# kai422/DAS3R

Hardware: AMD Instinct MI355X
Metric: render fwd+bwd Msplats/s at 1080p (higher is better)
Workload: dtype f32; 1 GPU; 1M random splats, 1920x1080, SH degree 3, forward+backward (BASELINE.json configs[3], constant P); splats_per_gpu=1000000, splats_per_gpu_final=1000000, init_steps=30, sh_degree=3, num_rendered=2614506, api=GaussianRasterizer.forward + autograd backward (drop-in surface), parallelism=1 independent scenes, one per GPU

## Files before the change

### das3r_amd/_lib.py

```python
import ctypes as C
import os

_HERE = os.path.dirname(os.path.abspath(__file__))
LIB_PATH = os.path.join(_HERE, "libdas3r_hip.so")
ABI_VERSION = 16
NO_BACKWARD_IN_FLAG = 8
ANTIALIAS_FLAG = 16
AUX_MAX_CHANNELS = 8

ALLOC_FN = C.CFUNCTYPE(C.c_void_p, C.c_void_p, C.c_size_t)


class RasterArgs(C.Structure):
    _fields_ = [("P", C.c_int32), ("sh_degree", C.c_int32), ("M", C.c_int32), ("image_width", C.c_int32),
                ("image_height", C.c_int32), ("tanfovx", C.c_float), ("tanfovy", C.c_float), ("scale_modifier", C.c_float),
                ("bg", C.c_void_p), ("viewmatrix", C.c_void_p), ("projmatrix", C.c_void_p), ("campos", C.c_void_p),
                ("prefiltered", C.c_int32), ("debug", C.c_int32), ("capacity_hint", C.c_int64)]


class PreTransform(C.Structure):
    _fields_ = [("xyz", C.c_void_p), ("rot", C.c_void_p), ("scaling", C.c_void_p), ("opacity_raw", C.c_void_p), ("conf_flat", C.c_void_p),
                ("mask_index", C.c_void_p), ("R", C.c_void_p), ("t", C.c_void_p), ("Lq", C.c_void_p)]


class RasterIn(C.Structure):
    _fields_ = [("means3D", C.c_void_p), ("opacities", C.c_void_p), ("shs", C.c_void_p), ("colors_precomp", C.c_void_p),
                ("scales", C.c_void_p), ("rotations", C.c_void_p), ("cov3D_precomp", C.c_void_p), ("pre", C.POINTER(PreTransform))]


class RasterOut(C.Structure):
    _fields_ = [("out_color", C.c_void_p), ("radii", C.c_void_p), ("out_invdepth", C.c_void_p)]


class RasterSaved(C.Structure):
    _fields_ = [("geom", C.c_void_p), ("binning", C.c_void_p), ("img", C.c_void_p), ("num_rendered", C.c_int64), ("capacity", C.c_int64),
                ("check_word", C.c_void_p), ("check_tag", C.c_uint32), ("flags", C.c_uint32)]


class AdamSlot(C.Structure):
    _fields_ = [("param", C.c_void_p), ("exp_avg", C.c_void_p), ("exp_avg_sq", C.c_void_p), ("step_size", C.c_float), ("bc2_sqrt", C.c_float)]


class Chain(C.Structure):
    _fields_ = [("g_conf_flat", C.c_void_p), ("g_small", C.c_void_p), ("slots", C.POINTER(AdamSlot)), ("beta1", C.c_float), ("beta2", C.c_float),
                ("eps", C.c_float)]


class RasterGrads(C.Structure):
    _fields_ = [("dL_dmeans2D", C.c_void_p), ("dL_dopacities", C.c_void_p), ("dL_dmeans3D", C.c_void_p),
                ("dL_dshs", C.c_void_p), ("dL_dcolors_precomp", C.c_void_p), ("dL_dscales", C.c_void_p),
                ("dL_drotations", C.c_void_p), ("dL_dcov3D", C.c_void_p), ("scratch", C.c_void_p), ("chain", C.POINTER(Chain))]


class PruneTensor(C.Structure):
    _fields_ = [("src", C.c_void_p), ("dst", C.c_void_p), ("row_bytes", C.c_int64)]


class PathPolicyState(C.Structure):
    _fields_ = [("P", C.c_int32), ("W", C.c_int32), ("H", C.c_int32), ("last_I", C.c_int64), ("peak_I", C.c_int64), ("radix_left", C.c_int32),
                ("backoff", C.c_int32), ("gen", C.c_uint32), ("seg_extra", C.c_int32), ("last_seg", C.c_int32), ("fine", C.c_int32),
                ("forwards", C.c_uint32), ("clean", C.c_uint32), ("longest", C.c_uint32), ("resume_valid", C.c_int32), ("resume_fine", C.c_int32),
                ("resume_forwards", C.c_uint32)]


class PathPolicyInputs(C.Structure):
    _fields_ = [("P", C.c_int32), ("W", C.c_int32), ("H", C.c_int32), ("ntiles", C.c_int32), ("tbits", C.c_int32), ("tile_passes", C.c_int32),
                ("too_long", C.c_uint32), ("want_bits", C.c_uint32), ("forced", C.c_int32), ("onesweep", C.c_int32), ("capacity_hint", C.c_int64),
                ("capacity_exact", C.c_int32)]


class PathPolicyPlan(C.Structure):
    _fields_ = [("local", C.c_int32), ("seg", C.c_int32), ("seg_bits", C.c_int32), ("seg_passes", C.c_int32), ("speculate", C.c_int32),
                ("decide_fine", C.c_int32), ("gen", C.c_uint32), ("cap", C.c_int64)]


class Switches(C.Structure):
    _fields_ = [(n, C.c_int32) for n in
                ("sort_ipl", "sort_classic", "rect_upstream", "verbose", "binning", "capacity_exact", "fused_emit_off", "no_sh_stage", "render_fwd",
                 "render_bwd", "render_bwd_mb", "render_bwd_atomic", "render_bwd_pix", "render_bwd_occ", "render_bwd_strips", "tile_chunk",
                 "scan_items", "deterministic", "tile_lpt_off", "bwd_reduce_set", "bwd_reduce_shfl", "ablate_set", "ablate", "tickets",
                 "bwd_pad_lds", "fwd_pad_lds", "bwd_buckets", "fwd_no_prefetch", "split_colour", "tile_strip")]


class BwdChoice(C.Structure):
    _fields_ = [(n, C.c_int32) for n in ("kernel", "mb", "slices", "pix", "occ", "strips", "atomic_flush")]


class FwdChoice(C.Structure):
    _fields_ = [(n, C.c_int32) for n in ("kernel", "quad_lanes", "row_private", "tile_lpt")]


class PreprocessBackwardInputs(C.Structure):
    _fields_ = [(n, C.c_int32) for n in ("has_sh", "has_cov", "M", "sh_degree", "shs_aligned16", "dL_dshs_aligned16", "no_sh_stage", "jac_saved",
                                         "chained", "quad_rows", "depth", "aa")]


class PreprocessForm(C.Structure):
    _fields_ = [(n, C.c_int32) for n in ("has_sh", "has_cov", "stage_in", "stage_out", "deg0", "chain", "depth", "jac", "aa", "base_index",
                                         "sh_rows_staged")]


PRUNE_GROUP_ROWS = 1024


def prune_count_words(P):
    return 1 + (int(P) + PRUNE_GROUP_ROWS - 1) // PRUNE_GROUP_ROWS


class RasterLayout(C.Structure):
    _fields_ = [(n, C.c_size_t) for n in
                ("geom_bytes", "binning_bytes", "img_bytes", "depth_key", "xy", "conic_opacity", "rgbd", "splat_stride", "clamped",
                 "tiles_touched", "sorted_idx", "offsets", "point_list", "final_T", "n_contrib", "ranges")]


EXPORTS = ("das3r_raster_forward", "das3r_raster_backward", "das3r_raster_backward_depth", "das3r_raster_backward_depth_scratch_bytes", "das3r_raster_check", "das3r_raster_backward_scratch_bytes", "das3r_mark_visible", "das3r_knn3_workspace_bytes",
           "das3r_knn3_mean_dist2", "das3r_raster_get_layout", "das3r_abi_version", "das3r_last_error", "das3r_reload_switches", "das3r_get_stats",
           "das3r_raster_forget_shapes", "das3r_raster_learning",
           "das3r_profile_enable", "das3r_profile_report", "das3r_pretransform_forward", "das3r_pretransform_backward", "das3r_pose_matrices", "das3r_pose_chain",
           "das3r_adam_step", "das3r_adam_step_gated", "das3r_photometric_blocks", "das3r_photometric_forward", "das3r_photometric_backward",
           "das3r_has_experiments", "das3r_pair_counters", "das3r_debug_poison_lds", "das3r_debug_inject_fault", "das3r_debug_mutate",
           "das3r_pose_matrices_qt", "das3r_pose_chain_qt", "das3r_photometric_finish", "das3r_pretransform_backward_adam", "das3r_pretransform_pose_sums",
           "das3r_raster_count_live_pairs", "das3r_photometric_backward_finish", "das3r_pose_chain_qt_rearm", "das3r_ssim_map_forward", "das3r_ssim_map_backward",
           "das3r_split_colour_rule", "das3r_split_colour_switch", "das3r_depth_l1_blocks", "das3r_depth_l1", "das3r_prune_select", "das3r_prune_compact",
           "das3r_photometric_forward_exposure", "das3r_photometric_backward_finish_exposure", "das3r_exposure_grad_finish",
           "das3r_raster_aux_forward", "das3r_raster_aux_scratch_bytes", "das3r_raster_aux_adjoint",
           "das3r_raster_aux_backward_scratch_bytes", "das3r_raster_aux_backward",
           "das3r_raster_distortion_forward", "das3r_raster_distortion_backward_scratch_bytes", "das3r_raster_distortion_backward",
           "das3r_thin_workspace_bytes", "das3r_thin_voxels", "das3r_raster_focal_workspace_bytes", "das3r_raster_backward_focal",
           "das3r_debug_path_policy_fresh", "das3r_debug_path_policy_plan", "das3r_debug_path_policy_count", "das3r_debug_path_policy_skew",
           "das3r_debug_path_policy_hint", "das3r_debug_path_policy_forget", "das3r_debug_path_policy_resume", "das3r_debug_seg_dbits",
           "das3r_debug_parse_switches", "das3r_debug_choose_backward", "das3r_debug_choose_forward", "das3r_debug_has_invdepth_form",
           "das3r_debug_kernel_name", "das3r_debug_choose_preprocess_backward", "das3r_debug_preprocess_backward_name")

_lib = None


def load():
    global _lib
    if _lib is not None:
        return _lib
    if not os.path.exists(LIB_PATH):
        raise RuntimeError(
            f"das3r_amd: HIP library not found at {LIB_PATH}. Build it with `python -c 'import __graft_entry__ as g; "
            f"g.build()'` or `make -C das3r_amd/csrc`. There is no CPU fallback.")
    L = C.CDLL(LIB_PATH)
    for name in EXPORTS:
        if not hasattr(L, name):
            raise RuntimeError(f"das3r_amd: {LIB_PATH} does not export {name}; rebuild it")
    L.das3r_abi_version.restype = C.c_int
    if L.das3r_abi_version() != ABI_VERSION:
        raise RuntimeError("das3r_amd: ABI version mismatch between the Python host layer and libdas3r_hip.so; rebuild")
    L.das3r_last_error.restype = C.c_char_p
    L.das3r_raster_forward.restype = C.c_int64
    L.das3r_raster_forward.argtypes = [C.POINTER(RasterArgs), C.POINTER(RasterIn), C.POINTER(RasterOut), ALLOC_FN, ALLOC_FN,
                                       ALLOC_FN, C.c_void_p, C.POINTER(RasterSaved), C.c_void_p]
    L.das3r_raster_backward.restype = C.c_int
    L.das3r_raster_backward.argtypes = [C.POINTER(RasterArgs), C.POINTER(RasterIn), C.POINTER(RasterSaved), C.c_void_p,
                                        C.POINTER(RasterGrads), C.c_void_p]
    L.das3r_raster_backward_scratch_bytes.restype = C.c_size_t
    L.das3r_raster_backward_depth.restype = C.c_int
    L.das3r_raster_backward_depth.argtypes = [C.POINTER(RasterArgs), C.POINTER(RasterIn), C.POINTER(RasterSaved), C.c_void_p, C.c_void_p,
                                              C.POINTER(RasterGrads), C.c_void_p]
    L.das3r_raster_backward_depth_scratch_bytes.restype = C.c_size_t
    L.das3r_raster_backward_depth_scratch_bytes.argtypes = [C.c_int64]
    L.das3r_raster_backward_scratch_bytes.argtypes = [C.c_int64]
    L.das3r_raster_check.restype = C.c_int
    L.das3r_raster_check.argtypes = [C.POINTER(RasterSaved), C.c_void_p]
    L.das3r_raster_count_live_pairs.restype = C.c_int
    L.das3r_raster_count_live_pairs.argtypes = [C.POINTER(RasterArgs), C.POINTER(RasterSaved), C.POINTER(C.c_uint64), C.c_void_p]
    L.das3r_mark_visible.restype = C.c_int
    L.das3r_mark_visible.argtypes = [C.c_int32, C.c_void_p, C.c_void_p, C.c_void_p, C.c_void_p, C.c_void_p]
    L.das3r_knn3_workspace_bytes.restype = C.c_size_t
    L.das3r_knn3_workspace_bytes.argtypes = [C.c_int32]
    L.das3r_knn3_mean_dist2.restype = C.c_int
    L.das3r_knn3_mean_dist2.argtypes = [C.c_int32, C.c_void_p, C.c_void_p, C.c_void_p, C.c_void_p]
    L.das3r_pose_matrices.restype = C.c_int
    L.das3r_pose_matrices.argtypes = [C.c_void_p, C.c_void_p, C.c_void_p]
    L.das3r_pose_chain.restype = C.c_int
    L.das3r_pose_chain.argtypes = [C.c_void_p, C.c_void_p, C.c_void_p, C.c_void_p]
    L.das3r_pretransform_forward.restype = C.c_int
    L.das3r_pretransform_forward.argtypes = [C.c_int32] + [C.c_void_p] * 13 + [C.c_void_p]
    L.das3r_pretransform_backward.restype = C.c_int
    L.das3r_pretransform_backward.argtypes = [C.c_int32] + [C.c_void_p] * 18 + [C.c_void_p]
    L.das3r_pretransform_backward_adam.restype = C.c_int
    L.das3r_pretransform_backward_adam.argtypes = [C.c_int32] + [C.c_void_p] * 10 + [C.POINTER(AdamSlot), C.c_float, C.c_float, C.c_float, C.c_void_p]
    L.das3r_pretransform_pose_sums.restype = C.c_int
    L.das3r_pretransform_pose_sums.argtypes = [C.c_int32] + [C.c_void_p] * 7 + [C.c_void_p]
    L.das3r_photometric_blocks.restype = C.c_int64
    L.das3r_photometric_blocks.argtypes = [C.c_int32, C.c_int32]
    L.das3r_photometric_forward.restype = C.c_int
    L.das3r_photometric_forward.argtypes = [C.c_int32, C.c_int32, C.c_void_p, C.c_void_p, C.c_void_p, C.c_float, C.c_void_p, C.c_void_p, C.c_void_p]
    L.das3r_photometric_backward.restype = C.c_int
    L.das3r_photometric_backward.argtypes = [C.c_int32, C.c_int32, C.c_void_p, C.c_void_p, C.c_void_p, C.c_float, C.c_void_p, C.c_void_p,
                                             C.c_void_p, C.c_void_p, C.c_void_p]
    L.das3r_pose_matrices_qt.restype = C.c_int
    L.das3r_pose_matrices_qt.argtypes = [C.c_void_p, C.c_void_p, C.c_void_p, C.c_void_p]
    L.das3r_pose_chain_qt.restype = C.c_int
    L.das3r_pose_chain_qt.argtypes = [C.c_void_p, C.c_void_p, C.c_void_p, C.c_void_p, C.c_void_p]
    L.das3r_pose_chain_qt_rearm.restype = C.c_int
    L.das3r_pose_chain_qt_rearm.argtypes = [C.c_void_p, C.c_void_p, C.c_void_p, C.c_void_p, C.c_void_p, C.c_void_p, C.c_void_p]
    L.das3r_ssim_map_forward.restype = C.c_int
    L.das3r_ssim_map_forward.argtypes = [C.c_int32, C.c_int32, C.c_void_p, C.c_void_p, C.c_void_p, C.c_void_p, C.c_void_p, C.c_void_p]
    L.das3r_ssim_map_backward.restype = C.c_int
    L.das3r_ssim_map_backward.argtypes = [C.c_int32, C.c_int32, C.c_void_p, C.c_void_p, C.c_void_p, C.c_void_p, C.c_void_p, C.c_void_p, C.c_void_p]
    L.das3r_photometric_backward_finish.restype = C.c_int
    L.das3r_photometric_backward_finish.argtypes = [C.c_int32, C.c_int32, C.c_void_p, C.c_void_p, C.c_void_p, C.c_float, C.c_void_p, C.c_void_p,
                                                    C.c_void_p, C.c_void_p, C.c_void_p, C.c_void_p, C.c_void_p]
    L.das3r_photometric_forward_exposure.restype = C.c_int
    L.das3r_photometric_forward_exposure.argtypes = [C.c_int32, C.c_int32, C.c_void_p, C.c_void_p, C.c_void_p, C.c_float, C.c_void_p, C.c_void_p,
                                                     C.c_void_p, C.c_void_p]
    L.das3r_photometric_backward_finish_exposure.restype = C.c_int
    L.das3r_photometric_backward_finish_exposure.argtypes = [C.c_int32, C.c_int32, C.c_void_p, C.c_void_p, C.c_void_p, C.c_float] + [C.c_void_p] * 9
    L.das3r_exposure_grad_finish.restype = C.c_int
    L.das3r_exposure_grad_finish.argtypes = [C.c_int32, C.c_int32, C.c_void_p, C.c_void_p, C.c_void_p, C.c_void_p]
    L.das3r_depth_l1_blocks.restype = C.c_int64
    L.das3r_depth_l1_blocks.argtypes = [C.c_int32, C.c_int32]
    L.das3r_depth_l1.restype = C.c_int
    L.das3r_depth_l1.argtypes = [C.c_int32, C.c_int32, C.c_void_p, C.c_void_p, C.c_void_p, C.c_void_p, C.c_float, C.c_void_p, C.c_void_p, C.c_void_p,
                                 C.c_void_p, C.c_void_p]
    L.das3r_prune_select.restype = C.c_int
    L.das3r_prune_select.argtypes = [C.c_int32, C.c_void_p, C.c_void_p, C.c_void_p, C.c_float, C.c_void_p, C.c_float, C.c_void_p, C.c_void_p, C.c_void_p,
                                     C.c_void_p]
    L.das3r_prune_compact.restype = C.c_int
    L.das3r_prune_compact.argtypes = [C.c_int32, C.c_int32, C.c_void_p, C.c_int32, C.POINTER(PruneTensor), C.c_void_p]
    L.das3r_thin_workspace_bytes.restype = C.c_size_t
    L.das3r_thin_workspace_bytes.argtypes = [C.c_int32]
    L.das3r_thin_voxels.restype = C.c_int
    L.das3r_thin_voxels.argtypes = [C.c_int32, C.c_void_p, C.c_void_p, C.c_float, C.c_void_p, C.c_void_p, C.c_void_p, C.c_void_p, C.c_void_p]
    L.das3r_raster_focal_workspace_bytes.restype = C.c_size_t
    L.das3r_raster_focal_workspace_bytes.argtypes = [C.c_int32]
    L.das3r_raster_backward_focal.restype = C.c_int
    L.das3r_raster_backward_focal.argtypes = [C.POINTER(RasterArgs), C.POINTER(RasterIn), C.POINTER(RasterSaved), C.c_void_p, C.c_void_p,
                                              C.POINTER(RasterGrads), C.c_void_p, C.c_void_p, C.c_void_p, C.c_void_p]
    L.das3r_raster_aux_forward.restype = C.c_int
    L.das3r_raster_aux_forward.argtypes = [C.POINTER(RasterArgs), C.POINTER(RasterSaved), C.c_int32, C.c_void_p, C.c_void_p, C.c_void_p]
    L.das3r_raster_aux_scratch_bytes.restype = C.c_size_t
    L.das3r_raster_aux_scratch_bytes.argtypes = [C.c_int64, C.c_int32]
    L.das3r_raster_aux_adjoint.restype = C.c_int
    L.das3r_raster_aux_adjoint.argtypes = [C.POINTER(RasterArgs), C.POINTER(RasterSaved), C.c_int32, C.c_void_p, C.c_void_p, C.c_int32, C.c_void_p,
                                           C.c_void_p]
    L.das3r_raster_aux_backward_scratch_bytes.restype = C.c_size_t
    L.das3r_raster_aux_backward_scratch_bytes.argtypes = [C.c_int64, C.c_int32]
    L.das3r_raster_aux_backward.restype = C.c_int
    L.das3r_raster_aux_backward.argtypes = [C.POINTER(RasterArgs), C.POINTER(RasterIn), C.POINTER(RasterSaved), C.c_int32, C.c_void_p, C.c_void_p,
                                            C.c_void_p, C.c_void_p, C.POINTER(RasterGrads), C.c_void_p]
    L.das3r_raster_distortion_forward.restype = C.c_int
    L.das3r_raster_distortion_forward.argtypes = [C.POINTER(RasterArgs), C.POINTER(RasterSaved), C.c_void_p, C.c_void_p, C.c_void_p]
    L.das3r_raster_distortion_backward_scratch_bytes.restype = C.c_size_t
    L.das3r_raster_distortion_backward_scratch_bytes.argtypes = [C.c_int64, C.c_int32]
    L.das3r_raster_distortion_backward.restype = C.c_int
    L.das3r_raster_distortion_backward.argtypes = [C.POINTER(RasterArgs), C.POINTER(RasterIn), C.POINTER(RasterSaved), C.c_void_p, C.c_void_p,
                                                   C.POINTER(RasterGrads), C.c_void_p]
    L.das3r_photometric_finish.restype = C.c_int
    L.das3r_photometric_finish.argtypes = [C.c_int32, C.c_int32, C.c_void_p, C.c_float, C.c_void_p, C.c_void_p]
    L.das3r_adam_step_gated.restype = C.c_int
    L.das3r_adam_step_gated.argtypes = [C.c_int32, C.c_void_p, C.c_float, C.c_float, C.c_float, C.c_void_p, C.c_float, C.c_void_p, C.c_void_p]
    L.das3r_adam_step.restype = C.c_int
    L.das3r_adam_step.argtypes = [C.c_int32, C.c_void_p, C.c_float, C.c_float, C.c_float, C.c_void_p]
    ps = C.POINTER(PathPolicyState)
    L.das3r_debug_path_policy_fresh.restype = None
    L.das3r_debug_path_policy_fresh.argtypes = [ps, C.c_uint32]
    L.das3r_debug_path_policy_plan.restype = None
    L.das3r_debug_path_policy_plan.argtypes = [ps, C.POINTER(PathPolicyInputs), C.POINTER(PathPolicyPlan)]
    L.das3r_debug_path_policy_count.restype = C.c_int
    L.das3r_debug_path_policy_count.argtypes = [ps, C.POINTER(PathPolicyInputs), C.POINTER(PathPolicyPlan), C.c_int64]
    L.das3r_debug_path_policy_skew.restype = C.c_int
    L.das3r_debug_path_policy_skew.argtypes = [ps, C.c_uint32, C.c_uint32, C.c_int64, C.c_int32]
    L.das3r_debug_path_policy_hint.restype = C.c_uint32
    L.das3r_debug_path_policy_hint.argtypes = [ps]
    L.das3r_debug_path_policy_forget.restype = None
    L.das3r_debug_path_policy_forget.argtypes = [ps]
    L.das3r_debug_path_policy_resume.restype = None
    L.das3r_debug_path_policy_resume.argtypes = [ps, C.c_uint32, C.c_uint32]
    L.das3r_debug_seg_dbits.restype = C.c_int
    L.das3r_debug_seg_dbits.argtypes = [C.c_int32, C.c_int32]
    sw = C.POINTER(Switches)
    L.das3r_debug_parse_switches.restype = None
    L.das3r_debug_parse_switches.argtypes = [C.POINTER(C.c_char_p), C.POINTER(C.c_char_p), C.c_int32, C.c_int32, sw]
    L.das3r_debug_choose_backward.restype = None
    L.das3r_debug_choose_backward.argtypes = [sw, C.c_int64, C.c_int32, C.c_uint32, C.POINTER(BwdChoice)]
    L.das3r_debug_choose_forward.restype = None
    L.das3r_debug_choose_forward.argtypes = [sw, C.c_int32, C.c_int64, C.c_int32, C.c_int32, C.POINTER(FwdChoice)]
    L.das3r_debug_has_invdepth_form.restype = C.c_int
    L.das3r_debug_has_invdepth_form.argtypes = [C.c_int32, C.c_int32]
    L.das3r_debug_kernel_name.restype = C.c_char_p
    L.das3r_debug_kernel_name.argtypes = [C.c_int32, C.c_int32]
    L.das3r_debug_choose_preprocess_backward.restype = C.c_int
    L.das3r_debug_choose_preprocess_backward.argtypes = [C.POINTER(PreprocessBackwardInputs), C.POINTER(PreprocessForm)]
    L.das3r_debug_preprocess_backward_name.restype = C.c_char_p
    L.das3r_debug_preprocess_backward_name.argtypes = [C.POINTER(PreprocessForm)]
    L.das3r_raster_get_layout.restype = C.c_int
    L.das3r_raster_get_layout.argtypes = [C.c_int32, C.c_int64, C.c_int32, C.c_int32, C.POINTER(RasterLayout)]
    _lib = L
    return L


def reload_switches():
    L = load()
    L.das3r_reload_switches.restype = None
    L.das3r_reload_switches.argtypes = []
    L.das3r_reload_switches()


def split_colour_rule(has_sh, sh_degree, P, binning_path, forced=None, no_backward=False):
    L = load()
    L.das3r_split_colour_rule.restype = C.c_int
    L.das3r_split_colour_rule.argtypes = [C.c_int32] * 6
    L.das3r_split_colour_switch.restype = C.c_int
    L.das3r_split_colour_switch.argtypes = []
    if forced is None:
        forced = L.das3r_split_colour_switch()
    return bool(L.das3r_split_colour_rule(int(bool(has_sh)), int(sh_degree), int(P), int(binning_path), int(bool(no_backward)), int(forced)))


def split_colour_switch():
    L = load()
    L.das3r_split_colour_switch.restype = C.c_int
    L.das3r_split_colour_switch.argtypes = []
    return int(L.das3r_split_colour_switch())


def has_experiments():
    L = load()
    L.das3r_has_experiments.restype = C.c_int
    L.das3r_has_experiments.argtypes = []
    return bool(L.das3r_has_experiments())


def inject_fault(bits):
    L = load()
    L.das3r_debug_inject_fault.restype = None
    L.das3r_debug_inject_fault.argtypes = [C.c_uint32]
    L.das3r_debug_inject_fault(int(bits))


def forget_shapes():
    L = load()
    L.das3r_raster_forget_shapes.restype = C.c_int
    L.das3r_raster_forget_shapes.argtypes = []
    check(L.das3r_raster_forget_shapes(), "das3r_raster_forget_shapes")


def learning(state=None):
    L = load()
    L.das3r_raster_learning.restype = C.c_int
    L.das3r_raster_learning.argtypes = [C.c_int32, C.POINTER(C.c_uint32)]
    buf = (C.c_uint32 * 2)(*(state if state is not None else (0, 0)))
    check(L.das3r_raster_learning(0 if state is None else 1, buf), "das3r_raster_learning")
    return int(buf[0]), int(buf[1])


def mutate(what):
    L = load()
    L.das3r_debug_mutate.restype = None
    L.das3r_debug_mutate.argtypes = [C.c_uint32]
    L.das3r_debug_mutate(int(what))


def poison_lds(pattern=0x7FC00000):
    import torch
    L = load()
    L.das3r_debug_poison_lds.restype = C.c_int
    L.das3r_debug_poison_lds.argtypes = [C.c_uint32, C.c_void_p]
    check(L.das3r_debug_poison_lds(int(pattern), C.c_void_p(torch.cuda.current_stream().cuda_stream)), "das3r_debug_poison_lds")


def pair_counters(enable):
    L = load()
    L.das3r_pair_counters.restype = C.c_int
    L.das3r_pair_counters.argtypes = [C.c_int, C.POINTER(C.c_uint64)]
    if enable:
        check(L.das3r_pair_counters(1, None), "das3r_pair_counters")
        return None
    out = (C.c_uint64 * 4)()
    check(L.das3r_pair_counters(0, out), "das3r_pair_counters")
    return dict(fwd_pairs=int(out[0]), bwd_pairs=int(out[1]), fwd_wave_iterations=int(out[2]), bwd_wave_iterations=int(out[3]))
# ... 57 lines not shown
```

### das3r_amd/csrc/api.hip

```cpp
#include <stdarg.h>
#include <string.h>

#include <vector>

#include "host_state.h"
#include "preprocess_choice.h"
#include <algorithm>

namespace das3r {

static thread_local char g_err[512] = "";

void set_error(const char *fmt, ...) {
    va_list ap;
    va_start(ap, fmt);
    vsnprintf(g_err, sizeof(g_err), fmt, ap);
    va_end(ap);
}

struct ProfRec {
    const char *name;
    hipEvent_t start, stop;
};
static bool g_prof_on = false;
static std::vector<ProfRec> g_prof;
bool profile_enabled() { return g_prof_on; }
static std::vector<hipEvent_t> g_event_pool;
static hipEvent_t pooled_event() {
    if (!g_event_pool.empty()) { hipEvent_t e = g_event_pool.back(); g_event_pool.pop_back(); return e; }
    hipEvent_t e = nullptr;
    return hipEventCreate(&e) == hipSuccess ? e : nullptr;
}
void profile_begin(const char *name, hipStream_t s) {
    ProfRec r;
    r.name = name;
    r.start = pooled_event();
    r.stop = pooled_event();
    if (!r.start || !r.stop) return;
    (void)hipEventRecord(r.start, s);
    g_prof.push_back(r);
}
void profile_end(hipStream_t s) {
    if (!g_prof.empty()) (void)hipEventRecord(g_prof.back().stop, s);
}

static Switches g_sw;
static bool g_sw_loaded = false;
static int g_inject_fault = 0;
static int g_mutate = 0;
static void load_switches() {
#ifdef DAS3R_EXPERIMENTS
    const bool experiments = true;
#else
    const bool experiments = false;
#endif
    Switches w = parse_switches(getenv, experiments);
    w.inject_fault = g_inject_fault;
    w.mutate = g_mutate;
    g_sw = w;
    __atomic_store_n(&g_sw_loaded, true, __ATOMIC_RELEASE);
}
const Switches &switches() {
    if (!__atomic_load_n(&g_sw_loaded, __ATOMIC_ACQUIRE)) load_switches();
    return g_sw;
}

static int g_threads_on_device[MAX_DEVICES] = {};
struct ThreadRegistrar {
    bool on[MAX_DEVICES] = {};
    void add(int dev) {
        if (!on[dev]) { on[dev] = true; __atomic_fetch_add(&g_threads_on_device[dev], 1, __ATOMIC_RELAXED); }
    }
    ~ThreadRegistrar() {
        for (int d = 0; d < MAX_DEVICES; d++)
            if (on[d]) __atomic_fetch_sub(&g_threads_on_device[d], 1, __ATOMIC_RELAXED);
    }
};
static thread_local ThreadRegistrar g_registrar;
void register_rendering_thread(int dev) { g_registrar.add(dev); }
bool grid_is_resident(int nblocks) {
    const int forced = switches().tickets;
    int dev = 0;
    if (hipGetDevice(&dev) != hipSuccess || dev < 0 || dev >= MAX_DEVICES) return false;
    const bool shared = __atomic_load_n(&g_threads_on_device[dev], __ATOMIC_RELAXED) > 1;
    if (forced >= 0) {
        static bool warned = false;
        if (shared && forced > 0 && !__atomic_exchange_n(&warned, true, __ATOMIC_RELAXED))
            fprintf(stderr, "[das3r] DAS3R_TICKETS is set to a bound while several host threads render on device %d: ticket-free chained "
                            "kernels are only safe when a grid has the device to itself\n", dev);
        return nblocks <= forced;
    }
    if (shared) return false;
    static thread_local int cached_dev = -1, cached_limit = 0;
    if (dev != cached_dev) {
        int cus = 0;
        if (hipDeviceGetAttribute(&cus, hipDeviceAttributeMultiprocessorCount, dev) != hipSuccess) return false;
        cached_dev = dev;
        cached_limit = cus * 2;
    }
    return nblocks <= cached_limit;
}

int sort_ipl_override() { return switches().sort_ipl; }
#ifdef DAS3R_EXPERIMENTS
bool use_onesweep() { return !switches().sort_classic; }
#else
bool use_onesweep() { return true; }
#endif
bool use_tight_rect() { return !switches().rect_upstream; }

void compute_layout(int P, int64_t I, int W, int H, Layout *L, bool shjac) {
    memset(L, 0, sizeof(*L));
    const size_t Pn = P > 0 ? (size_t)P : 1, In = I > 0 ? (size_t)I : 1;
    L->capacity = I;
    L->tiles_x = (W + TILE_X - 1) / TILE_X;
    L->tiles_y = (H + TILE_Y - 1) / TILE_Y;
    L->ntiles = L->tiles_x * L->tiles_y;
    L->tbits = tile_bits(L->ntiles);
    L->tile_passes = (L->tbits + 7) / 8;
    L->dbits = 0;
    L->kbits = L->tbits;
    L->kshift = 0;
    L->part_passes = L->tile_passes;
    L->chunksP = sort_num_chunks(P);
    L->chunksI = sort_num_chunks(I);
    size_t o = 0;
    auto take = [&](size_t b) { size_t r = o; o += align_up(b); return r; };
    L->g_keyA = take(4 * Pn);
    L->g_keyB = take(4 * Pn);
    L->g_valA = take(4 * Pn);
    L->g_valB = take(4 * Pn);
    L->pub.sorted_idx = L->g_valA;
    L->pub.depth_key = L->g_keyA;
    L->pub.xy = take(16 * SPLAT_REC * Pn);
    L->pub.conic_opacity = L->pub.xy + 16;
    L->pub.rgbd = L->pub.xy + 32;
    L->pub.splat_stride = 16 * SPLAT_REC;
    L->pub.clamped = take(Pn);
    L->pub.tiles_touched = take(4 * Pn);
    L->pub.offsets = take(4 * Pn);
    L->g_hist = take(4 * (size_t)RADIX_SIZE * (size_t)(L->chunksP > 0 ? L->chunksP : 1));
    L->g_totals = take(4 * RADIX_SIZE);
    L->g_blocksums = take(4 * (size_t)div_up((int64_t)Pn, 4096));
    L->g_count = take(256);
    L->g_off_by_gid = take(4 * Pn);
    L->g_rect = take(4 * Pn);
    L->g_dhist = take(4 * 256);
    L->g_ghist = take(4 * 4 * RADIX_SIZE);
    L->g_ticket = take(256);
    L->g_status = take(onesweep_status_bytes((int64_t)Pn, 4));
    L->g_scan_status = take(scan_status_bytes((int)Pn));
    L->g_ctrl_bytes = o - L->g_ghist;
    if (shjac) L->g_shjac = take(4 * 9 * Pn);
    L->pub.geom_bytes = o;
    o = 0;
    L->b_keyA = take(4 * In);
    L->b_keyB = take(4 * In);
    L->b_valA = take(4 * In);
    L->b_valB = take(4 * In);
    L->b_hist = take(4 * (size_t)RADIX_SIZE * (size_t)(L->chunksI > 0 ? L->chunksI : 1));
    L->b_totals = take(4 * RADIX_SIZE);
    L->b_gid_of = take(4 * In);
    L->b_slot = take(4 * In);
    L->b_e2 = take(4 * In);
    L->b_ghist = take(4 * 4 * RADIX_SIZE);
    L->b_ticket = take(256);
    L->b_status = take(onesweep_status_bytes((int64_t)In, L->tile_passes + 1));
    L->b_ctrl_bytes = o - L->b_ghist;
    L->b_ckpt = take(((size_t)In / BUCKET + (size_t)(L->ntiles > 0 ? L->ntiles : 1) + 2) * 256 * 16);
    L->pub.binning_bytes = o;
    const size_t npix_d = (size_t)W * (size_t)H;
    L->d_ckpt = take(((size_t)In / BUCKET + (size_t)(L->ntiles > 0 ? L->ntiles : 1) + 2) * 256 * 16);
    L->d_recs = take(16 * SPLAT_REC * Pn);
    L->d_dpix = take(4 * 3 * (npix_d > 0 ? npix_d : 1));
    L->d_bg = take(16);
    L->d_dz = take(4 * Pn);
    L->d_bytes = o;
    L->pub.point_list = (L->tile_passes & 1) ? L->b_valB : L->b_valA;
    o = 0;
    const size_t npix = (size_t)W * (size_t)H;
    L->pub.final_T = take(4 * (npix > 0 ? npix : 1));
    L->pub.n_contrib = take(4 * (npix > 0 ? npix : 1));
    L->pub.ranges = take(8 * (size_t)(L->ntiles > 0 ? L->ntiles : 1));
    L->i_order = take(4 * (size_t)(L->ntiles > 0 ? L->ntiles : 1));
    L->pub.img_bytes = o;
}

}

using namespace das3r;

extern "C" int das3r_abi_version(void) { return DAS3R_ABI_VERSION; }
extern "C" void das3r_reload_switches(void) { load_switches(); }
extern "C" void das3r_debug_inject_fault(uint32_t bits) {
    g_inject_fault = (int)bits;
    load_switches();
}
extern "C" void das3r_debug_mutate(uint32_t what) {
    g_mutate = (int)what;
    load_switches();
}
extern "C" const char *das3r_last_error(void) { return g_err; }
extern "C" int das3r_split_colour_switch(void) { return switches().split_colour; }
extern "C" int das3r_split_colour_rule(int32_t has_sh, int32_t sh_degree, int32_t P, int32_t binning_path, int32_t no_backward, int32_t forced) {
    return split_colour_rule(has_sh != 0, sh_degree, P, binning_path, no_backward != 0, forced) ? 1 : 0;
}

namespace {
struct PolicyOnState {
    Verdict v;
    Resume r;
    das3r_path_policy_state *s;
    explicit PolicyOnState(das3r_path_policy_state *state) : s(state) { policy_state_from(*s, &v, &r); }
    ~PolicyOnState() { policy_state_to(v, r, s); }
    PolicyInputs inputs(const das3r_path_policy_inputs *in) {
        return PolicyInputs{in->P, in->W, in->H, in->ntiles, in->tbits, in->tile_passes, in->too_long, in->want_bits, in->forced, in->onesweep != 0,
                            in->capacity_hint, in->capacity_exact != 0, &r};
    }
};
ForwardPlan plan_of(const das3r_path_policy_plan *p) {
    return ForwardPlan{p->local != 0, p->seg != 0, p->seg == 2, p->seg_bits, p->seg_passes, p->speculate != 0, p->cap, p->decide_fine != 0, p->gen};
}
}
extern "C" void das3r_debug_path_policy_fresh(das3r_path_policy_state *state, uint32_t gen) { policy_state_to(Verdict::fresh(gen), Resume(), state); }
extern "C" void das3r_debug_path_policy_plan(das3r_path_policy_state *state, const das3r_path_policy_inputs *in, das3r_path_policy_plan *out) {
    PolicyOnState on(state);
    const ForwardPlan p = plan_forward(on.v, on.inputs(in));
    *out = das3r_path_policy_plan{p.local, p.bucket_local ? 2 : (p.seg ? 1 : 0), p.seg_bits, p.seg_passes, p.speculate, p.decide_fine, p.gen, p.cap};
}
extern "C" int das3r_debug_path_policy_count(das3r_path_policy_state *state, const das3r_path_policy_inputs *in, const das3r_path_policy_plan *plan, int64_t I) {
    PolicyOnState on(state);
    return learn_count(on.v, I, on.inputs(in), plan_of(plan)) ? 1 : 0;
}
extern "C" int das3r_debug_path_policy_skew(das3r_path_policy_state *state, uint32_t longest, uint32_t crowd16, int64_t cap, int32_t ntiles) {
    PolicyOnState on(state);
    return learn_skew(on.v, longest, crowd16, cap, ntiles) ? 1 : 0;
}
extern "C" uint32_t das3r_debug_path_policy_hint(const das3r_path_policy_state *state) {
    Verdict v;
    Resume r;
    policy_state_from(*state, &v, &r);
    return backward_hint(v, (uint32_t)BUCKET);
}
extern "C" void das3r_debug_path_policy_forget(das3r_path_policy_state *state) {
    PolicyOnState on(state);
    forget(on.v);
}
extern "C" void das3r_debug_path_policy_resume(das3r_path_policy_state *state, uint32_t fine, uint32_t forwards) {
    PolicyOnState on(state);
    resume(on.v, on.r, fine != 0u, forwards);
}
extern "C" int das3r_debug_seg_dbits(int32_t tbits, int32_t passes) { return seg_dbits((int)tbits, (int)passes); }

extern "C" void das3r_debug_parse_switches(const char *const *names, const char *const *values, int32_t n, int32_t experiments, das3r_switches *out) {
    auto lookup = [&](const char *name) -> const char * {
        for (int32_t i = 0; i < n; i++)
            if (strcmp(names[i], name) == 0) return values[i];
        return nullptr;
    };
    switches_to(parse_switches(lookup, experiments != 0), out);
}
extern "C" void das3r_debug_choose_backward(const das3r_switches *sw, int64_t num_rendered, int32_t ntiles, uint32_t fwd_flags, das3r_bwd_choice *out) {
    const BwdChoice c = choose_backward(switches_from(*sw), num_rendered, ntiles, fwd_flags);
    *out = das3r_bwd_choice{c.kernel, c.mb, c.slices, c.pix, c.occ, c.strips, c.atomic_flush};
}
extern "C" void das3r_debug_choose_forward(const das3r_switches *sw, int32_t ntiles, int64_t capacity, int32_t local_lists, int32_t prefer_regions,
                                           das3r_fwd_choice *out) {
    const Switches w = switches_from(*sw);
    const bool local = local_lists != 0, regions = prefer_regions != 0;
    *out = das3r_fwd_choice{choose_forward(w, ntiles, capacity, local, regions), quad_lanes(w, ntiles, capacity, local), row_private(w, capacity, ntiles),
                            tile_lpt_wanted(w, ntiles, capacity, local, regions)};
}
extern "C" int das3r_debug_has_invdepth_form(int32_t backward, int32_t kernel) {
    return (backward ? bwd_has_invdepth_form((BwdKernel)kernel) : fwd_has_invdepth_form((FwdKernel)kernel)) ? 1 : 0;
}
extern "C" const char *das3r_debug_kernel_name(int32_t backward, int32_t kernel) {
    return backward ? bwd_kernel_name((BwdKernel)kernel) : fwd_kernel_name((FwdKernel)kernel);
}

static PreprocessForm form_from(const das3r_preprocess_form *f) {
    return PreprocessForm{f->has_sh != 0, f->has_cov != 0, f->stage_in != 0, f->stage_out != 0, f->deg0 != 0, f->chain != 0, f->depth != 0, f->jac != 0, f->aa != 0};
}
extern "C" int das3r_debug_choose_preprocess_backward(const das3r_preprocess_backward_inputs *in, das3r_preprocess_form *out) {
    const PreprocessBackwardInputs ci = {in->has_sh != 0, in->has_cov != 0, in->M, in->sh_degree, in->shs_aligned16 != 0, in->dL_dshs_aligned16 != 0,
                                         in->no_sh_stage != 0, in->jac_saved != 0, in->chained != 0, in->quad_rows != 0, in->depth != 0, in->aa != 0};
    const PreprocessForm f = choose_preprocess_backward(ci);
    *out = das3r_preprocess_form{f.has_sh, f.has_cov, f.stage_in, f.stage_out, f.deg0, f.chain, f.depth, f.jac, f.aa, preprocess_backward_base_index(f),
                                 sh_rows_staged(ci.has_sh, ci.M, ci.sh_degree, ci.shs_aligned16, ci.no_sh_stage)};
    return chain_refusal(ci);
}
extern "C" const char *das3r_debug_preprocess_backward_name(const das3r_preprocess_form *form) { return preprocess_backward_name(form_from(form)); }

extern "C" int das3r_raster_get_layout(int32_t P, int64_t num_rendered, int32_t W, int32_t H, das3r_raster_layout *out) {
    if (!out || P < 0 || num_rendered < 0 || W <= 0 || H <= 0) { set_error("das3r_raster_get_layout: invalid argument"); return DAS3R_ERR_INVALID_ARG; }
    Layout L;
    compute_layout(P, num_rendered, W, H, &L);
    *out = L.pub;
    return DAS3R_OK;
}

extern "C" int das3r_raster_forget_shapes(void) {
    PerDevice *T = nullptr;
    int r = per_device(&T);
    if (r) return r;
    forget(T->verdict);
    return DAS3R_OK;
}

extern "C" int das3r_raster_learning(int32_t set, uint32_t state[2]) {
    if (!state) { set_error("das3r_raster_learning: invalid argument"); return DAS3R_ERR_INVALID_ARG; }
    PerDevice *T = nullptr;
    int r = per_device(&T);
    if (r) return r;
    if (!set) {
        state[0] = prefers_regions(T->verdict) ? 1u : 0u;
        state[1] = forwards_seen(T->verdict);
        return DAS3R_OK;
    }
    resume(T->verdict, T->resume, state[0] != 0u, state[1]);
    return DAS3R_OK;
}

static Layout saved_layout(const das3r_raster_args *a, const das3r_raster_saved *saved, bool shjac = false) {
    Layout L;
    compute_layout(a->P, saved->capacity > 0 ? saved->capacity : saved->num_rendered, a->image_width, a->image_height, &L, shjac);
    return L;
}

static bool shjac_saved(const das3r_raster_args *a, const das3r_raster_in *in, const das3r_raster_saved *saved) {
    return (saved->flags & SHJAC_SAVED_FLAG) != 0 && in->shs != nullptr && a->sh_degree >= 2;
}

static int backward_validate(const char *who, const das3r_raster_in *in, const das3r_raster_saved *saved, const float *dL_dpix, bool depth_pass,
                             const float *dL_dinvdepth, const das3r_raster_grads *g) {
    const bool chained = g && g->chain;
    if (!saved || !saved->geom || !saved->img || !dL_dpix || (depth_pass && !dL_dinvdepth) || !g || !g->dL_dmeans2D ||
        (!chained && (!g->dL_dopacities || !g->dL_dmeans3D)) || (saved->num_rendered > 0 && !g->scratch)) {
        set_error("%s: null saved state / %sgradient buffer", who, depth_pass ? "upstream gradient / " : "");
        return DAS3R_ERR_INVALID_ARG;
    }
    if (depth_pass && !(saved->flags & DEPTH_SAVED_FLAG)) {
        set_error("%s: the saved state is not that of a forward with out_invdepth (das3r_raster_saved.flags bit 1 is clear)", who);
        return DAS3R_ERR_INVALID_ARG;
    }
    const bool has_sh = in->shs != nullptr, has_cov = in->cov3D_precomp != nullptr;
    if ((has_sh && !g->dL_dshs) || (!has_sh && !g->dL_dcolors_precomp) || (has_cov && !g->dL_dcov3D) ||
        (!has_cov && !chained && (!g->dL_dscales || !g->dL_drotations))) {
        set_error("%s: gradient buffer missing for a provided input", who);
        return DAS3R_ERR_INVALID_ARG;
    }
    return DAS3R_OK;
}

struct FocalOut {
    float *sums, *per_splat, *workspace;
};

static int refuse_bwd_without_invdepth(const char *who) {
    const BwdKernel k = switches().render_bwd;
    if (bwd_has_invdepth_form(k)) return DAS3R_OK;
    set_error("%s: DAS3R_RENDER_BWD=%s has no inverse-depth form", who, bwd_kernel_name(k));
    return DAS3R_ERR_INVALID_ARG;
}

static int backward_body(const char *who, const das3r_raster_args *a, const das3r_raster_in *in, const das3r_raster_saved *saved, const float *dL_dpix,
                         bool depth_pass, const float *dL_dinvdepth, const das3r_raster_grads *g, const FocalOut *focal, das3r_stream_t stream) {
    hipStream_t s = (hipStream_t)stream;
    int rc = validate(a, in);
    if (rc) return rc;
    const int P = a->P;
    if (P == 0) {
        if (focal) HIP_TRY(hipMemsetAsync(focal->sums, 0, 2 * sizeof(float), s));
        return DAS3R_OK;
    }
    if ((rc = backward_validate(who, in, saved, dL_dpix, depth_pass, dL_dinvdepth, g))) return rc;
    if (depth_pass && (rc = refuse_bwd_without_invdepth(who))) return rc;
    if ((rc = das3r_raster_check(saved, stream))) return rc;
    const Layout L = saved_layout(a, saved, shjac_saved(a, in, saved));
    float *partial = g->scratch;
    const float *dz = nullptr;
    bool quad_rows = false;
    if (saved->num_rendered > 0) {
        if (!saved->binning) { set_error("%s: binning buffer missing", who); return DAS3R_ERR_INVALID_ARG; }
        if ((rc = launch_render_backward(a, dL_dpix, saved->geom, saved->binning, saved->img, L, partial, s, &quad_rows, saved->num_rendered, saved->flags))) return rc;
        if (depth_pass) {
            const size_t c = L.capacity > 0 ? (size_t)L.capacity : 1;
            float *partial_depth = (float *)((char *)g->scratch + align_up(c * 9 * sizeof(float) + 16));
            if ((rc = launch_depth_pass_inputs(P, a->image_width * a->image_height, saved->geom, L, saved->binning, dL_dinvdepth, s, a->debug != 0))) return rc;
            Layout Ld = L;
            Ld.pub.xy = L.d_recs;
            Ld.pub.conic_opacity = L.d_recs + 16;
            Ld.pub.rgbd = L.d_recs + 32;
            Ld.b_ckpt = L.d_ckpt;
            das3r_raster_args ad = *a;
            ad.bg = (const float *)(saved->binning + L.d_bg);
            bool quad_rows_d = false;
            if ((rc = launch_render_backward(&ad, (const float *)(saved->binning + L.d_dpix), saved->binning, saved->binning, saved->img, Ld, partial_depth, s,
                                             &quad_rows_d, saved->num_rendered, saved->flags))) return rc;
            float *dzw = (float *)(saved->binning + L.d_dz);
            if ((rc = launch_depth_fold(P, saved->geom, L, partial, partial_depth, dzw, s, a->debug != 0))) return rc;
            dz = dzw;
        }
    }
    const bool aa = (saved->flags & ANTIALIAS_FLAG) != 0;
    if (focal && (rc = launch_focal_grad(a, in, saved->geom, L, partial, quad_rows, aa, focal->sums, focal->per_splat, focal->workspace, s))) return rc;
    return launch_preprocess_backward(a, in, saved->geom, saved->binning, L, g, partial, s, quad_rows, dz, aa);
}

extern "C" int das3r_raster_backward(const das3r_raster_args *a, const das3r_raster_in *in, const das3r_raster_saved *saved,
                                     const float *dL_dpix, const das3r_raster_grads *g, das3r_stream_t stream) {
    return backward_body("das3r_raster_backward", a, in, saved, dL_dpix, false, nullptr, g, nullptr, stream);
}

extern "C" int das3r_raster_backward_depth(const das3r_raster_args *a, const das3r_raster_in *in, const das3r_raster_saved *saved,
                                           const float *dL_dpix, const float *dL_dinvdepth, const das3r_raster_grads *g, das3r_stream_t stream) {
    return backward_body("das3r_raster_backward_depth", a, in, saved, dL_dpix, true, dL_dinvdepth, g, nullptr, stream);
}

extern "C" size_t das3r_raster_focal_workspace_bytes(int32_t P) { return focal_workspace_bytes(P); }
extern "C" int das3r_raster_backward_focal(const das3r_raster_args *a, const das3r_raster_in *in, const das3r_raster_saved *saved, const float *dL_dpix,
                                           const float *dL_dinvdepth, const das3r_raster_grads *g, float *sums, float *per_splat, float *workspace,
                                           das3r_stream_t stream) {
    if (!sums || !workspace) {
        set_error("das3r_raster_backward_focal: null sums / workspace");
        return DAS3R_ERR_INVALID_ARG;
    }
    const bool depth_pass = dL_dinvdepth != nullptr;
    if (depth_pass) {
        const int rc = refuse_bwd_without_invdepth("das3r_raster_backward_focal");
        if (rc) return rc;
    }
    const FocalOut focal = {sums, per_splat, workspace};
    return backward_body("das3r_raster_backward_focal", a, in, saved, dL_dpix, depth_pass, dL_dinvdepth, g, &focal, stream);
}

extern "C" size_t das3r_raster_backward_depth_scratch_bytes(int64_t capacity) {
    const size_t c = capacity > 0 ? (size_t)capacity : 1;
    return align_up(c * 9 * sizeof(float) + 16) + c * 9 * sizeof(float) + 16;
}

extern "C" size_t das3r_raster_backward_scratch_bytes(int64_t capacity) {
    const size_t c = capacity > 0 ? (size_t)capacity : 1;
#ifdef DAS3R_EXPERIMENTS
    if (switches().render_bwd == BWD_STREAM) return std::max(c * 9 * sizeof(float) + 16, stream_scratch_bytes(capacity));
#endif
    return c * 9 * sizeof(float) + 16;
}

static int aux_validate(const char *who, const das3r_raster_args *a, const das3r_raster_saved *saved, int32_t C, const void *p0, const void *p1) {
    if (!a || !saved) { set_error("%s: null args / saved state", who); return DAS3R_ERR_INVALID_ARG; }
    if (C < 1 || C > DAS3R_AUX_MAX_CHANNELS) { set_error("%s: C = %d channels (1 .. %d per call)", who, C, DAS3R_AUX_MAX_CHANNELS); return DAS3R_ERR_INVALID_ARG; }
    if (a->P < 0 || a->image_width <= 0 || a->image_height <= 0) { set_error("%s: bad extents P=%d W=%d H=%d", who, a->P, a->image_width, a->image_height); return DAS3R_ERR_INVALID_ARG; }
    if (!p1 || (a->P > 0 && !p0)) { set_error("%s: null feature / image / gradient pointer", who); return DAS3R_ERR_INVALID_ARG; }
    if (a->P > 0 && saved->num_rendered > 0 && (!saved->geom || !saved->binning || !saved->img)) { set_error("%s: saved buffers missing", who); return DAS3R_ERR_INVALID_ARG; }
    return DAS3R_OK;
}

extern "C" int das3r_raster_aux_forward(const das3r_raster_args *a, const das3r_raster_saved *saved, int32_t C, const float *features, float *out,
                                        das3r_stream_t stream) {
    hipStream_t s = (hipStream_t)stream;
    int rc = aux_validate("das3r_raster_aux_forward", a, saved, C, features, out);
    if (rc) return rc;
    const int P = a->P, W = a->image_width, H = a->image_height;
    if (P == 0 || saved->num_rendered <= 0) {
        HIP_TRY(hipMemsetAsync(out, 0, sizeof(float) * (size_t)C * (size_t)W * (size_t)H, s));
        return DAS3R_OK;
    }
    if ((rc = das3r_raster_check(saved, stream))) return rc;
    const Layout L = saved_layout(a, saved);
    return launch_render_aux_forward(P, W, H, C, features, out, saved->geom, saved->binning, saved->img, L, saved->num_rendered, a->debug != 0, s);
}

extern "C" size_t das3r_raster_aux_scratch_bytes(int64_t capacity, int32_t C) {
    const size_t c = capacity > 0 ? (size_t)capacity : 1, ch = C > 0 ? (size_t)C : 1;
    return c * ch * sizeof(float) + 16;
}

extern "C" int das3r_raster_aux_adjoint(const das3r_raster_args *a, const das3r_raster_saved *saved, int32_t C, const float *dL_dout, float *dL_dfeat,
                                        int32_t accumulate, float *scratch, das3r_stream_t stream) {
    hipStream_t s = (hipStream_t)stream;
    int rc = aux_validate("das3r_raster_aux_adjoint", a, saved, C, dL_dfeat, dL_dout);
    if (rc) return rc;
    const int P = a->P, W = a->image_width, H = a->image_height;
    if (P == 0) return DAS3R_OK;
    if (saved->num_rendered <= 0) {
        if (!accumulate) HIP_TRY(hipMemsetAsync(dL_dfeat, 0, sizeof(float) * (size_t)P * (size_t)C, s));
        return DAS3R_OK;
    }
    if (!scratch) { set_error("das3r_raster_aux_adjoint: null scratch (das3r_raster_aux_scratch_bytes)"); return DAS3R_ERR_INVALID_ARG; }
    if ((rc = das3r_raster_check(saved, stream))) return rc;
    const Layout L = saved_layout(a, saved);
    return launch_render_aux_adjoint(P, W, H, C, dL_dout, dL_dfeat, accumulate != 0, scratch, saved->geom, saved->binning, saved->img, L, saved->num_rendered, a->debug != 0, s);
}

extern "C" size_t das3r_raster_aux_backward_scratch_bytes(int64_t capacity, int32_t C) {
    const size_t c = capacity > 0 ? (size_t)capacity : 1, ch = C > 0 ? (size_t)C : 0;
    return align_up(c * 9 * sizeof(float) + 16) + c * ch * sizeof(float) + 16;
}

extern "C" int das3r_raster_aux_backward(const das3r_raster_args *a, const das3r_raster_in *in, const das3r_raster_saved *saved, int32_t C,
                                         const float *features, const float *dL_dout, const float *dL_dalpha, float *dL_dfeatures,
                                         const das3r_raster_grads *g, das3r_stream_t stream) {
    static const char who[] = "das3r_raster_aux_backward";
    hipStream_t s = (hipStream_t)stream;
    if (!a || !in || !saved || !g) { set_error("%s: null args / inputs / saved state / grads", who); return DAS3R_ERR_INVALID_ARG; }
    if (C < 0 || C > DAS3R_AUX_MAX_CHANNELS) { set_error("%s: C = %d channels (0 .. %d per call)", who, C, DAS3R_AUX_MAX_CHANNELS); return DAS3R_ERR_INVALID_ARG; }
    if (C == 0 && !dL_dalpha) { set_error("%s: C = 0 channels and null dL_dalpha: no loss term", who); return DAS3R_ERR_INVALID_ARG; }
    if (C == 0 && dL_dfeatures) { set_error("%s: dL_dfeatures with C = 0 channels", who); return DAS3R_ERR_INVALID_ARG; }
    if (C > 0 && (!dL_dout || (a->P > 0 && !features))) { set_error("%s: null features / dL_dout with C = %d channels", who, C); return DAS3R_ERR_INVALID_ARG; }
    if (g->chain) { set_error("%s: grads->chain is not supported here (the chained backward belongs to the colour loss)", who); return DAS3R_ERR_INVALID_ARG; }
    if (!g->scratch) { set_error("%s: null scratch (das3r_raster_aux_backward_scratch_bytes)", who); return DAS3R_ERR_INVALID_ARG; }
    int rc = validate(a, in);
    if (rc) return rc;
    const int P = a->P, W = a->image_width, H = a->image_height;
    if (P == 0) return DAS3R_OK;
    if ((rc = backward_validate(who, in, saved,  reinterpret_cast<const float *>(g->scratch), false, nullptr, g))) return rc;
    if (saved->num_rendered > 0 && !saved->binning) { set_error("%s: binning buffer missing", who); return DAS3R_ERR_INVALID_ARG; }
    if ((rc = das3r_raster_check(saved, stream))) return rc;
    const Layout L = saved_layout(a, saved, shjac_saved(a, in, saved));
    float *partial = g->scratch;
    if (saved->num_rendered > 0) {
        const size_t c = L.capacity > 0 ? (size_t)L.capacity : 1;
        float *partial_f = dL_dfeatures ? (float *)((char *)g->scratch + align_up(c * 9 * sizeof(float) + 16)) : nullptr;
        if ((rc = launch_render_aux_backward(P, W, H, C, features, dL_dout, dL_dalpha, partial, partial_f, saved->geom, saved->binning, saved->img, L,
                                             a->debug != 0, s))) return rc;
        if (dL_dfeatures && (rc = launch_aux_gather(P, C, partial_f, dL_dfeatures, saved->geom, L, a->debug != 0, s))) return rc;
    } else if (dL_dfeatures) {
        HIP_TRY(hipMemsetAsync(dL_dfeatures, 0, sizeof(float) * (size_t)P * (size_t)C, s));
    }
    return launch_preprocess_backward(a, in, saved->geom, saved->binning, L, g, partial, s, false, nullptr, (saved->flags & ANTIALIAS_FLAG) != 0);
}
// ... 198 lines not shown
```

### das3r_amd/csrc/common.h

```cpp
#pragma once
#include <hip/hip_runtime.h>
#include <stdint.h>
#include <stdio.h>

#include "../../include/das3r_raster.h"
#include "kernel_choice.h"
#include "path_policy.h"
#include "pretransform_math.h"

#define TILE_X 16
#define TILE_Y 16
#define TILE_PIX 256
#define WAVE 64
#define NEAR_PLANE 0.001f

namespace das3r {

void set_error(const char *fmt, ...);

const Switches &switches();

#define HIP_TRY(expr)                                                                          \
    do {                                                                                       \
        hipError_t _e = (expr);                                                                \
        if (_e != hipSuccess) {                                                                \
            das3r::set_error("%s failed: %s (%s:%d)", #expr, hipGetErrorString(_e), __FILE__, __LINE__); \
            return DAS3R_ERR_HIP;                                                              \
        }                                                                                      \
    } while (0)

#define KERNEL_CHECK(stream, debug, name)                                                      \
    do {                                                                                       \
        hipError_t _e = hipGetLastError();                                                     \
        if (_e == hipSuccess && (debug)) _e = hipStreamSynchronize(stream);                    \
        if (_e != hipSuccess) {                                                                \
            das3r::set_error("kernel %s failed: %s", name, hipGetErrorString(_e));             \
            return DAS3R_ERR_HIP;                                                              \
        }                                                                                      \
    } while (0)

bool profile_enabled();
void profile_begin(const char *name, hipStream_t s);
void profile_end(hipStream_t s);
struct ProfTimer {
    hipStream_t s;
    bool on;
    ProfTimer(const char *name, hipStream_t stream) : s(stream), on(profile_enabled()) {
        if (on) profile_begin(name, s);
    }
    ~ProfTimer() {
        if (on) profile_end(s);
    }
};

unsigned long long *pair_counters();
constexpr int PHASE_WORDS = 16, PHASE_COPIES = 64;
#ifdef DAS3R_EXPERIMENTS
#define PHASE_BEGIN()                                                                      \
    __shared__ unsigned long long phase_w_[8];                                             \
    unsigned long long phase_t_ = 0ull;                                                    \
    if (pairs != nullptr && threadIdx.x == 0) {                                            \
        for (int k_ = 0; k_ < 8; k_++) phase_w_[k_] = 0ull;                                \
        phase_t_ = clock64();                                                              \
    }
#define PHASE_MARK(k)                                                                      \
    if (pairs != nullptr && threadIdx.x == 0) {                                            \
        const unsigned long long now_ = clock64();                                         \
        phase_w_[(k) & 7] += now_ - phase_t_;                                              \
        phase_t_ = now_;                                                                   \
    }
#define PHASE_END(base)                                                                    \
    if (pairs != nullptr && threadIdx.x == 0)                                              \
        for (int k_ = 0; k_ < 8; k_++) atomicAdd(pairs + 4 + (blockIdx.x % PHASE_COPIES) * PHASE_WORDS + (base) + k_, phase_w_[k_]);
constexpr int TRACE_WGS = 16384, TRACE_PASSES = 8, TRACE_STAMPS = 8;
unsigned long long *wg_trace();
static inline unsigned long long *pairs_or_trace() {
    unsigned long long *p = pair_counters();
    if (p == nullptr && wg_trace() != nullptr) p = reinterpret_cast<unsigned long long *>(reinterpret_cast<uintptr_t>(wg_trace()) | 1u);
    return p;
}
#define DECODE_PAIRS_OR_TRACE(arg)                                                                                         \
    unsigned long long *const trace = (reinterpret_cast<uintptr_t>(arg) & 1u)                                              \
                                          ? reinterpret_cast<unsigned long long *>(reinterpret_cast<uintptr_t>(arg) & ~(uintptr_t)1) \
                                          : nullptr;                                                                       \
    unsigned long long *const pairs = trace ? nullptr : (arg);
#define WG_STAMP(k)                                                                                   \
    if (trace != nullptr && threadIdx.x == 0 && s_block < (uint32_t)TRACE_WGS)                        \
        trace[((size_t)(shift >> 3) * TRACE_WGS + s_block) * TRACE_STAMPS + (k)] = wall_clock64();
#define SCAN_STAMP(k)                                                                                 \
    if (wg_trace_ptr != nullptr && threadIdx.x == 0 && s_block < (uint32_t)TRACE_WGS)                 \
        wg_trace_ptr[((size_t)(TRACE_PASSES - 1) * TRACE_WGS + s_block) * TRACE_STAMPS + (k)] = wall_clock64();
#define BLK_STAMP(ptr, r, k)                                                                          \
    if ((ptr) != nullptr && threadIdx.x == 0 && blockIdx.x < (uint32_t)TRACE_WGS)                      \
        (ptr)[((size_t)(r) * TRACE_WGS + blockIdx.x) * TRACE_STAMPS + (k)] = wall_clock64();
#define PAIRS_ARG pairs_or_trace()
#else
#define PAIRS_ARG pair_counters()
#define PHASE_MARK(k)
#define PHASE_BEGIN()
#define PHASE_END(base)
#define WG_STAMP(k)
#define SCAN_STAMP(k)
#define BLK_STAMP(ptr, r, k)
#endif

#define DAS3R_LAUNCH(kernel, grid, block, shmem, stream, ...)                \
    do {                                                                     \
        das3r::ProfTimer _pt(#kernel, stream);                               \
        hipLaunchKernelGGL(kernel, grid, block, shmem, stream, __VA_ARGS__); \
    } while (0)

static inline size_t align_up(size_t x, size_t a = 256) { return (x + a - 1) / a * a; }
static inline int div_up(int64_t a, int64_t b) { return (int)((a + b - 1) / b); }

constexpr int RADIX_BITS = 8;
constexpr int RADIX_SIZE = 1 << RADIX_BITS;
constexpr int SORT_WAVES_PER_BLOCK = 4;
int sort_ipl_override();
static inline int sort_items_per_lane(int64_t n) {
    const int o = sort_ipl_override();
    return o ? o : (n >= (int64_t)(1 << 21) ? 16 : (n >= (1 << 17) ? 8 : 4));
}
static inline int sort_num_chunks(int64_t n) { return n == 0 ? 0 : div_up(n, (int64_t)WAVE * sort_items_per_lane(n)); }
__host__ __device__ static inline int tile_digit_width(int tbits) {
    const int passes = (tbits + 7) / 8;
    return passes > 0 ? (tbits + passes - 1) / passes : 8;
}
static inline int tile_bits(int ntiles) {
    int b = 0;
    while ((1 << b) < ntiles) b++;
    return b < 1 ? 1 : b;
}

constexpr int SPLAT_REC = 4;

constexpr uint32_t DEPTH_SAVED_FLAG = 2u;
constexpr uint32_t SHJAC_SAVED_FLAG = 4u;
constexpr uint32_t NO_BACKWARD_IN_FLAG = 8u;
constexpr uint32_t ANTIALIAS_FLAG = 16u;
struct Layout {
    das3r_raster_layout pub;
    size_t g_keyA, g_keyB, g_valA, g_valB, g_hist, g_totals, g_blocksums, g_count, g_off_by_gid, g_rect;
    size_t b_keyA, b_keyB, b_valA, b_valB, b_hist, b_totals, b_gid_of, b_slot;
    size_t b_e2;
    size_t b_ckpt;
    size_t d_ckpt, d_recs, d_dpix, d_bg, d_dz, d_bytes;
    size_t g_ghist, g_ticket, g_status, g_scan_status, g_ctrl_bytes;
    int64_t capacity;
    size_t b_ghist, b_ticket, b_status, b_ctrl_bytes;
    int tiles_x, tiles_y, ntiles, tbits, tile_passes;
    int chunksP, chunksI;
    int dbits, kbits, kshift;
    int part_passes;
    size_t g_dhist;
    size_t g_shjac;
    const uint32_t *dhist_ptr;
    size_t i_order;
};
static inline int seg_dbits(const Layout &L, int passes) { return seg_dbits(L.tbits, passes); }

struct LocalBin {
    float4 *ckpt;
    uint32_t *point_list, *slot_list;
    uint32_t *keys;
    uint32_t *host_flag;
    uint32_t flag_value;
    uint32_t last_g, cap;
    bool prefer_regions;
    const uint32_t *tile_order;
    int dbits, fbits;
};
void compute_layout(int P, int64_t I, int W, int H, Layout *L, bool shjac = false);

struct EmitArgs {
    unsigned long long *status;
    uint32_t tag;
    uint32_t *ghist;
    uint32_t *err;
    uint32_t *tile_keys, *gids, *off_by_gid;
    uint32_t cap;
    int tbits;
    uint32_t *count;
    uint32_t *count_out;
};
constexpr int EMIT_SLOT_WORDS = 64 + 4 * 256;
constexpr int EMIT_STATUS_GRANULES = 1024;

constexpr int COLOUR_WGS_PER_CU = 4;
struct SideStream {
    hipStream_t stream;
    hipEvent_t fork, join;
    int colour_blocks;
};
int launch_preprocess(const das3r_raster_args *a, const das3r_raster_in *in, int32_t *radii, char *geom, char *img, char *binning_ctrl,
                      size_t binning_ctrl_bytes, const Layout &L, unsigned long long *arrive, uint32_t *host_out, uint32_t tag,
                      hipStream_t s, const EmitArgs *emit, uint32_t *dhist, uint32_t *dhist_next, bool aa ,
                      const SideStream *side = nullptr);
int launch_sh_colour(const das3r_raster_args *a, const das3r_raster_in *in, char *geom, const Layout &L, const SideStream *side);
int launch_mark_visible(int P, const float *means3D, const float *viewmatrix, uint8_t *present, hipStream_t s);
int launch_depth_sort(int P, char *geom, const Layout &L, int part, char *binning_ctrl, size_t binning_ctrl_bytes, bool debug, hipStream_t s);
int launch_scan(int P, char *geom, const Layout &L, uint32_t *host_out, uint32_t tag, bool debug, hipStream_t s, bool index_order = false);
int launch_scan_emit(int P, int64_t cap, const int32_t *radii, char *geom, char *binning, const Layout &L, uint32_t *host_out, uint32_t tag,
                     bool debug, hipStream_t s, bool index_order = false);
size_t scan_status_bytes(int P);
int launch_binning_scan_emit(int P, int64_t I, const int32_t *radii, char *geom, char *binning, const Layout &L, bool ctrl_zeroed,
                             uint32_t *host_out, uint32_t tag, bool debug, hipStream_t s, bool index_order = false);
size_t onesweep_status_bytes(int64_t n, int passes);
int launch_onesweep_depth_sort(int P, char *geom, const Layout &L, int part, uint32_t *zero_ptr, uint32_t zero_words, bool debug,
                               hipStream_t s);
int launch_onesweep_partition(int64_t cap, char *geom, char *binning, const Layout &L, uint32_t **keys_final, bool debug, hipStream_t s,
                              uint32_t *ghist_override = nullptr, uint32_t *err_override = nullptr);
inline PreXform pre_xform(const das3r_raster_in *in) {
    PreXform x = {nullptr, nullptr, nullptr, nullptr, nullptr, nullptr, nullptr, nullptr, nullptr};
    if (in && in->pre) {
        const das3r_pretransform *p = in->pre;
        x = PreXform{p->xyz, p->rot, p->scaling, p->opacity_raw, p->conf_flat, p->mask_index, p->R, p->t, p->Lq};
    }
    return x;
}
int launch_render_forward_regions(const das3r_raster_args *a, float *out_color, char *geom, char *binning, char *img, const Layout &L, const LocalBin &lb,
                                  hipStream_t s, float *out_invdepth, float4 *dckpt);
int launch_tile_lpt(char *img, const Layout &L, uint32_t cap, bool debug, hipStream_t s);
int launch_list_skew(const char *img, const char *binning, const char *geom, const Layout &L, uint32_t cap, uint32_t last_g, uint32_t *mailbox_words, uint32_t tag,
                     bool debug, hipStream_t s);
int launch_render_forward_slices(const das3r_raster_args *a, float *out_color, char *geom, char *binning, char *img, const Layout &L, const LocalBin &lb,
                                 hipStream_t s);
int launch_render_forward_lanes(const das3r_raster_args *a, float *out_color, char *geom, char *binning, char *img, const Layout &L,
                                const LocalBin &lb, hipStream_t s, float *out_invdepth, float4 *dckpt);
int launch_render_forward_rows(const das3r_raster_args *a, float *out_color, char *geom, char *binning, char *img, const Layout &L,
                               const LocalBin &lb, hipStream_t s, float *out_invdepth, float4 *dckpt);
int launch_render_backward_mfma(const das3r_raster_args *a, const float *dL_dpix, char *geom, char *binning, char *img, const Layout &L,
                                float *partial, hipStream_t s);
size_t stream_scratch_bytes(int64_t capacity);
int launch_render_backward_stream(const das3r_raster_args *a, const float *dL_dpix, char *geom, char *binning, char *img, const Layout &L,
                                  float *scratch, hipStream_t s);
int launch_render_backward_scan(const das3r_raster_args *a, const float *dL_dpix, char *geom, char *binning, char *img, const Layout &L,
                                float *partial, const BwdChoice &c, hipStream_t s);
int launch_render_backward_blk(const das3r_raster_args *a, const float *dL_dpix, char *geom, char *binning, char *img, const Layout &L,
                               float *partial, const BwdChoice &c, hipStream_t s);
int launch_render_backward_regions(const das3r_raster_args *a, const float *dL_dpix, char *geom, char *binning, char *img, const Layout &L,
                               float *partial, const BwdChoice &c, hipStream_t s);
constexpr int LOCAL_MAX = 1024;
bool grid_is_resident(int nblocks);
bool use_onesweep();
bool use_tight_rect();
int launch_binning(int P, int64_t I, int W, int H, const int32_t *radii, char *geom, char *binning, char *img, const Layout &L,
                   bool fused_scan, uint32_t *host_late, uint32_t tag, bool debug, hipStream_t s, uint32_t **dead_keys = nullptr,
                   uint32_t *emit_slot = nullptr ,
                   uint32_t *seg_host_flag = nullptr, uint32_t seg_flag_value = 0 ,
                   bool local_finish = false );
int launch_segment_sort(int64_t cap, const uint32_t *n_ptr, const uint32_t *keys_final, int fbits, uint32_t *point_list, uint32_t *slot_list,
                        const uint32_t *depth_key, uint32_t last_g, uint32_t *scratch_keys, uint32_t *host_flag, uint32_t flag_value, bool debug,
                        hipStream_t s, int dbits, uint2 *ranges, const uint32_t *err, uint32_t *host_late, uint32_t tag, uint32_t inject);
int launch_render_forward(const das3r_raster_args *a, const float *colors_precomp, float *out_color, char *geom, char *binning,
                          char *img, const Layout &L, const LocalBin &lb, hipStream_t s, float *out_invdepth ,
                          float4 *dckpt );
int launch_depth_pass_inputs(int P, int npix, const char *geom, const Layout &L, char *binning, const float *dL_dinvdepth, hipStream_t s, bool debug);
int launch_depth_fold(int P, const char *geom, const Layout &L, float *partial, const float *partial_depth, float *dz, hipStream_t s, bool debug);
size_t focal_workspace_bytes(int P);
int launch_focal_grad(const das3r_raster_args *a, const das3r_raster_in *in, const char *geom, const Layout &L, const float *partial, bool quad_rows,
                      bool aa , float *sums , float *per_splat , float *workspace, hipStream_t s);
static inline const uint8_t *quad_rows_exist(const float *partial, const Layout &L, bool quad_rows) {
    const size_t cap_rows = L.capacity > 0 ? (size_t)L.capacity : 1;
    return quad_rows ? reinterpret_cast<const uint8_t *>(partial) + align_up(cap_rows * 4 * 12 * sizeof(float)) : nullptr;
}
int launch_render_backward(const das3r_raster_args *a, const float *dL_dpix, char *geom, char *binning, char *img, const Layout &L,
                           float *partial, hipStream_t s, bool *quad_rows, int64_t num_rendered, uint32_t fwd_flags );
int launch_render_aux_forward(int P, int W, int H, int C, const float *feat, float *out, const char *geom, const char *binning, const char *img,
                              const Layout &L, int64_t num_rendered, bool debug, hipStream_t s);
int launch_render_aux_adjoint(int P, int W, int H, int C, const float *dL_dout, float *dL_dfeat, int accumulate, float *partial, const char *geom,
                              const char *binning, const char *img, const Layout &L, int64_t num_rendered, bool debug, hipStream_t s);
int launch_aux_gather(int P, int C, const float *partial, float *dL_dfeat, const char *geom, const Layout &L, bool debug, hipStream_t s);
int launch_render_aux_backward(int P, int W, int H, int C, const float *feat, const float *dL_dout, const float *dL_dalpha, float *partial,
                               float *partial_f, const char *geom, const char *binning, const char *img, const Layout &L, bool debug, hipStream_t s);
int launch_render_distortion_forward(int P, int W, int H, float *out, float *totals, const char *geom, const char *binning, const char *img,
                                     const Layout &L, bool debug, hipStream_t s);
int launch_render_distortion_backward(int P, int W, int H, const float *dL_ddist, const float *totals, float *partial, const char *geom,
                                      const char *binning, const char *img, const Layout &L, bool debug, hipStream_t s);
int launch_distortion_fold(int P, const char *geom, const Layout &L, float *partial, float *dz, bool debug, hipStream_t s);
int launch_count_live_pairs(const das3r_raster_args *a, char *geom, char *binning, char *img, const Layout &L, unsigned long long *out, hipStream_t s);
int launch_preprocess_backward(const das3r_raster_args *a, const das3r_raster_in *in, char *geom, char *binning, const Layout &L,
                               const das3r_raster_grads *g, const float *partial, hipStream_t s, bool quad_rows, const float *dz ,
                               bool aa );

#ifdef __HIPCC__
__device__ __forceinline__ int lane_id() { return __lane_id(); }

template <int CTRL, int ROW_MASK>
__device__ __forceinline__ float dpp_step(float v) {
    int moved = __builtin_amdgcn_update_dpp(0, __float_as_int(v), CTRL, ROW_MASK, 0xf, true);
    return v + __int_as_float(moved);
}
__device__ __forceinline__ float wave_sum_to_lane63(float v) {
    v = dpp_step<0x111, 0xf>(v);
    v = dpp_step<0x112, 0xf>(v);
    v = dpp_step<0x114, 0xf>(v);
    v = dpp_step<0x118, 0xf>(v);
    v = dpp_step<0x142, 0xa>(v);
    v = dpp_step<0x143, 0xc>(v);
    return v;
}
__device__ __forceinline__ float row_sum_to_lane15(float v) {
    v = dpp_step<0x111, 0xf>(v);
    v = dpp_step<0x112, 0xf>(v);
    v = dpp_step<0x114, 0xf>(v);
    v = dpp_step<0x118, 0xf>(v);
    return v;
}
__device__ __forceinline__ float wave_sum_shfl(float v) {
#pragma unroll
    for (int o = 32; o >= 1; o >>= 1) v += __shfl_xor(v, o, 64);
    return v;
}
#endif

}
```

### das3r_amd/csrc/forward.hip

```cpp
#include <string.h>

#include <algorithm>
#include <vector>

#include "host_state.h"

namespace das3r {

constexpr int SPLIT_MIN_P = 1 << 18;
bool split_colour_rule(bool has_sh, int sh_degree, int P, int binning_path, bool no_backward, int forced) {
    if (!has_sh || sh_degree < 1 || binning_path != 1 || forced < 0 || P <= 0) return false;
    if (forced > 0) return true;
    return sh_degree >= 2 && P >= SPLIT_MIN_P && !no_backward;
}

struct PerStream {
    int dev;
    hipStream_t caller;
    SideStream side = {nullptr, nullptr, nullptr, 0};
    uint32_t *dhist = nullptr;
    uint32_t turn = 0;
};
struct PerStreams {
    std::vector<PerStream> all;
// ... 73 lines not shown
    if ((in->shs != nullptr) == (in->colors_precomp != nullptr)) { set_error("Please provide excatly one of either SHs or precomputed colors!"); return DAS3R_ERR_INVALID_ARG; }
    const bool sr = in->pre != nullptr || (in->scales != nullptr && in->rotations != nullptr);
    if ((!in->pre && (in->scales != nullptr) != (in->rotations != nullptr)) || sr == (in->cov3D_precomp != nullptr)) {
        set_error("Please provide exactly one of either scale/rotation pair or precomputed 3D covariance!");
        return DAS3R_ERR_INVALID_ARG;
    }
    if (in->shs) {
        if (a->sh_degree < 0 || a->sh_degree > 3) { set_error("sh_degree must be 0..3 (got %d)", a->sh_degree); return DAS3R_ERR_INVALID_ARG; }
        if (a->M < (a->sh_degree + 1) * (a->sh_degree + 1) || a->M > 16) { set_error("M=%d incompatible with sh_degree=%d (need (D+1)^2 <= M <= 16)", a->M, a->sh_degree); return DAS3R_ERR_INVALID_ARG; }
    }
    if (a->tanfovx <= 0.f || a->tanfovy <= 0.f) { set_error("tanfov must be positive"); return DAS3R_ERR_INVALID_ARG; }
    return DAS3R_OK;
}

int per_device(PerDevice **out) {
    static thread_local PerDevice state[MAX_DEVICES];
    int dev = 0;
    HIP_TRY(hipGetDevice(&dev));
    if (dev < 0 || dev >= MAX_DEVICES) { set_error("device ordinal %d not supported", dev); return DAS3R_ERR_INVALID_ARG; }
    PerDevice &T = state[dev];
    register_rendering_thread(dev);
    if (!T.mb.host) {
        uint32_t *h = nullptr;
        HIP_TRY(hipHostMalloc((void **)&h, MAILBOX_BYTES, hipHostMallocMapped));
        memset(h, 0, MAILBOX_BYTES);
        HIP_TRY(hipHostGetDevicePointer((void **)&T.mb.dev, h, 0));
        T.mb.host = h;
    }
    *out = &T;
    return DAS3R_OK;
}
static int await_tag(volatile uint32_t *word, uint32_t tag, hipStream_t s, uint32_t *seen) {
    for (long spins = 0; spins < 200000000L; spins++) {
        if ((*seen = __atomic_load_n(word, __ATOMIC_ACQUIRE)) == tag) return DAS3R_OK;
        __builtin_ia32_pause();
        if ((spins & 0xFFFFF) == 0xFFFFF && hipStreamQuery(s) != hipErrorNotReady) break;
    }
    HIP_TRY(hipStreamSynchronize(s));
    *seen = __atomic_load_n(word, __ATOMIC_ACQUIRE);
    return DAS3R_OK;
}
static int mailbox_wait(Mailbox *mb, int idx, uint32_t tag, hipStream_t s) {
    uint32_t seen = 0;
    const int r = await_tag(&mb->host[idx], tag, s, &seen);
    if (r) return r;
    if (seen == tag) return DAS3R_OK;
    set_error("the device never delivered the result of this forward to the host mailbox");
    return DAS3R_ERR_HIP;
}

static unsigned long long g_stats[4] = {0, 0, 0, 0};
static void stat_add(int i) { __atomic_fetch_add(&g_stats[i], 1ull, __ATOMIC_RELAXED); }
int examine_check_slot(volatile uint32_t *slot, uint32_t tag, bool wait, hipStream_t s) {
    const CheckResult c = examine_check_word(slot, tag, wait, [s](volatile uint32_t *word, uint32_t t, uint32_t *seen) { return await_tag(word, t, s, seen); });
    if (c.error) return c.error;
    if (c.state == CHECK_NOT_THERE) return 1;
    for (int i = 1; i < 4; i++)
        if (c.stats >> i & 1u) stat_add(i);
    if (c.rescued && switches().verbose) fprintf(stderr, "das3r: a look-back poll needed the read-modify-write path\n");
    if (c.state != CHECK_FAILED) return DAS3R_OK;
    set_error("a forward's binning failed its self-check (flags 0x%x); its output is invalid", c.flags);
    return DAS3R_ERR_HIP;
}
struct SlotExaminer {
    Mailbox *mb;
    hipStream_t s;
    int operator()(uint32_t i, uint32_t tag, bool wait) const { return examine_check_slot(mb->host + check_word_index(i), tag, wait, s); }
};

constexpr uint32_t ARRIVE_SLOTS = 16, ARRIVE_WORDS = 8 + 64 * 8;
constexpr size_t EMIT_SLOT_BYTES = sizeof(uint32_t) * EMIT_SLOT_WORDS + sizeof(unsigned long long) * EMIT_STATUS_GRANULES;

struct Join {
    hipStream_t s;
    SideStream side = {nullptr, nullptr, nullptr, 0};
    bool forked = false, pending = false;
    ~Join() {
        if (pending) (void)hipStreamWaitEvent(s, side.join, 0);
    }
};

struct ForwardCall {
    const das3r_raster_args *a;
    const das3r_raster_in *in;
    const das3r_raster_out *out;
    das3r_alloc_fn alloc_geom, alloc_binning, alloc_img;
    void *user;
    das3r_raster_saved *saved;
    hipStream_t s;
    Join join;
    PerDevice *T = nullptr;
    Mailbox *mb = nullptr;
    Layout L;
    PolicyInputs policy_in;
    ForwardPlan plan;
    bool local = false;
    bool shjac = false, depth = false, no_backward = false, aa = false;
    uint32_t count_tag = 0, late_tag = 0;
    const uint32_t *seg_dhist = nullptr;
    unsigned long long *arrive = nullptr;

    int64_t run();
    int check_arguments();
    int empty_scene();
    int arrival_ring();
    int layout_and_alloc(int64_t cap);
    int preprocess(int binning_path, const EmitArgs *emit);
    int colour_launch();
    int colour_join();
    int claim_check_slot(uint32_t **host_late);
    int look_at_lists(LocalBin *lb);
    int bin_and_render(bool local_order, bool ctrl_zeroed, uint32_t *count_out = nullptr, uint32_t count_out_tag = 0, uint32_t *emit_slot = nullptr);
    int read_count(int64_t *I);
    int flow_fused_emit(int64_t *I);
    int flow_speculative(int64_t *I);
    int after_speculation(int64_t *I);
    int flow_exact(int64_t *I);
    int redo_exact(int64_t I);
};

int ForwardCall::check_arguments() {
    const int rc = validate(a, in);
    if (rc) return rc;
    if (!out || !out->out_color || (a->P > 0 && !out->radii) || !alloc_geom || !alloc_binning || !alloc_img || !saved) {
        set_error("das3r_raster_forward: null output/allocator");
        return DAS3R_ERR_INVALID_ARG;
    }
    if (out->out_invdepth && !fwd_has_invdepth_form(switches().render_fwd)) {
        set_error("das3r_raster_forward: DAS3R_RENDER=%s has no inverse-depth form (das3r_raster_out.out_invdepth)", fwd_kernel_name(switches().render_fwd));
        return DAS3R_ERR_INVALID_ARG;
    }
    return DAS3R_OK;
}

int64_t ForwardCall::run() {
    stat_add(0);
    int rc = check_arguments();
    if (rc) return rc;
    const int P = a->P, W = a->image_width, H = a->image_height;
    depth = out->out_invdepth != nullptr;
    shjac = in->shs != nullptr && a->sh_degree >= 2 && !(saved->flags & NO_BACKWARD_IN_FLAG);
    no_backward = (saved->flags & NO_BACKWARD_IN_FLAG) != 0;
    aa = (saved->flags & ANTIALIAS_FLAG) != 0;
    compute_layout(P, 0, W, H, &L, shjac);
    saved->geom = alloc_geom(user, L.pub.geom_bytes);
    saved->img = alloc_img(user, L.pub.img_bytes);
    saved->binning = nullptr;
    saved->num_rendered = 0;
    saved->capacity = 0;
    saved->check_word = nullptr;
    saved->check_tag = 0;
    saved->flags = aa ? ANTIALIAS_FLAG : 0u;
    if (!saved->geom || !saved->img) { set_error("scratch allocation failed (geom %zu B, img %zu B)", L.pub.geom_bytes, L.pub.img_bytes); return DAS3R_ERR_ALLOC; }
    if (P == 0) return empty_scene();
    if ((rc = per_device(&T))) return rc;
    mb = &T->mb;
    if ((rc = T->checks.settle_all(SlotExaminer{mb, s}))) return rc;
    if ((rc = arrival_ring())) return rc;
    const uint32_t too_long = mb->host[MB_TOO_LONG];
    if (too_long) mb->host[MB_TOO_LONG] = 0;
    const uint32_t want_bits = mb->host[MB_WANT_BITS];
    if (want_bits) mb->host[MB_WANT_BITS] = 0;
    policy_in = PolicyInputs{P, W, H, L.ntiles, L.tbits, L.tile_passes, too_long, want_bits, switches().binning , use_onesweep(),
                             a->capacity_hint, switches().capacity_exact, &T->resume};
    plan = plan_forward(T->verdict, policy_in);
    local = plan.local;
    count_tag = next_tag(mb);
    arrive = T->arrive_ring + (size_t)(count_tag % ARRIVE_SLOTS) * ARRIVE_WORDS;
    int64_t I = 0;
    if (plan.speculate) {
        if ((rc = layout_and_alloc(plan.cap))) return rc;
        const bool fused_emit = local && grid_is_resident(div_up(P, 256)) && !switches().fused_emit_off;
        rc = fused_emit ? flow_fused_emit(&I) : flow_speculative(&I);
    } else {
        rc = flow_exact(&I);
    }
    if (rc) return rc;
    if (a->debug && late_tag && (rc = T->checks.settle(check_slot_of(late_tag), true, SlotExaminer{mb, s}))) return rc;
    saved->num_rendered = I;
    saved->capacity = L.capacity;
    if (depth) saved->flags |= DEPTH_SAVED_FLAG;
    if (shjac) saved->flags |= SHJAC_SAVED_FLAG;
    return I;
}

int ForwardCall::empty_scene() {
    const int W = a->image_width, H = a->image_height;
    HIP_TRY(hipMemsetAsync(out->out_color, 0, sizeof(float) * 3 * (size_t)W * H, s));
    if (out->out_invdepth) HIP_TRY(hipMemsetAsync(out->out_invdepth, 0, sizeof(float) * (size_t)W * H, s));
    HIP_TRY(hipMemsetAsync(saved->img + L.pub.ranges, 0, 8 * (size_t)L.ntiles, s));
    saved->binning = alloc_binning(user, 256);
    return 0;
}

int ForwardCall::arrival_ring() {
    if (T->arrive_ring) return DAS3R_OK;
    HIP_TRY(hipMalloc((void **)&T->arrive_ring, ARRIVE_SLOTS * ARRIVE_WORDS * sizeof(unsigned long long)));
    HIP_TRY(hipMemsetAsync(T->arrive_ring, 0, ARRIVE_SLOTS * ARRIVE_WORDS * sizeof(unsigned long long), s));
    HIP_TRY(hipStreamSynchronize(s));
    return DAS3R_OK;
}

int ForwardCall::layout_and_alloc(int64_t cap) {
    compute_layout(a->P, cap, a->image_width, a->image_height, &L, shjac);
    L.dhist_ptr = seg_dhist;
    if (plan.seg) {
        L.dbits = plan.seg_bits;
        L.kbits = L.tbits + plan.seg_bits;
        L.kshift = std::min(16, 32 - L.kbits);
        L.part_passes = plan.seg_passes;
    }
    saved->binning = alloc_binning(user, depth ? L.d_bytes : L.pub.binning_bytes);
    if (saved->binning) return DAS3R_OK;
    set_error("scratch allocation failed (binning %zu B)", L.pub.binning_bytes);
    return DAS3R_ERR_ALLOC;
}

int ForwardCall::preprocess(int binning_path, const EmitArgs *emit) {
    int rc;
    uint32_t *dhist = nullptr, *dhist_next = nullptr;
    if (!emit && (rc = seg_dhist_for(plan.seg, s, saved->geom, L, &dhist, &dhist_next))) return rc;
    L.dhist_ptr = seg_dhist = dhist;
    const SideStream *side = nullptr;
    if (split_colour_rule(in->shs != nullptr, a->sh_degree, a->P, binning_path, no_backward, switches().split_colour)) {
        if ((rc = side_stream_for(s, &join.side))) return rc;
        side = &join.side;
    }
    char *ctrl = plan.speculate ? saved->binning + L.b_ghist : nullptr;
    if ((rc = launch_preprocess(a, in, out->radii, saved->geom, saved->img, ctrl, ctrl ? L.b_ctrl_bytes : 0, L, plan.speculate ? nullptr : arrive, mb->dev,
                                count_tag, s, emit, dhist, dhist_next, aa, side))) return rc;
    join.forked = side != nullptr;
    return DAS3R_OK;
}

int ForwardCall::colour_launch() {
    if (!join.forked) return DAS3R_OK;
    join.forked = false;
    join.pending = true;
    return launch_sh_colour(a, in, saved->geom, L, &join.side);
}
int ForwardCall::colour_join() {
    const int r = colour_launch();
    if (r) return r;
    if (!join.pending) return DAS3R_OK;
    join.pending = false;
    HIP_TRY(hipStreamWaitEvent(s, join.side.join, 0));
    return DAS3R_OK;
}

int ForwardCall::claim_check_slot(uint32_t **host_late) {
    late_tag = next_tag(mb);
    uint32_t slot = 0;
    const int r = T->checks.claim(late_tag, &slot, SlotExaminer{mb, s});
    if (r) return r;
    *host_late = mb->dev + check_word_index(slot);
    saved->check_word = (void *)(mb->host + check_word_index(slot));
    saved->check_tag = late_tag;
    return DAS3R_OK;
}

int ForwardCall::look_at_lists(LocalBin *lb) {
    int r;
    const int P = a->P;
    const int64_t cap = L.capacity;
    const bool by_shape = cap > 0 && quad_lanes(switches(), L.ntiles, L.capacity, false);
    if (plan.decide_fine && by_shape) {
        const uint32_t tag = next_tag(mb);
        if ((r = launch_list_skew(saved->img, saved->binning, saved->geom, L, (uint32_t)cap, (uint32_t)(P - 1), mb->dev + MB_LONGEST, tag, a->debug != 0, s))) return r;
        if ((r = mailbox_wait(mb, MB_SKEW_TAG, tag, s))) return r;
        const uint32_t longest = mb->host[MB_LONGEST], crowd16 = mb->host[MB_CROWD16];
        const int64_t mean = skew_mean(T->verdict, cap, L.ntiles);
        const bool now_fine = learn_skew(T->verdict, longest, crowd16, cap, L.ntiles);
        if (switches().verbose) fprintf(stderr, "[das3r] tile lists: longest %lld, mean %lld, %.1f of 64 consecutive entries in one quadrant -> %s kernels\n", (long long)longest,
                                        (long long)mean, crowd16 / 16.0, now_fine ? "2x2-region" : "block");
    }
    const bool fine = prefers_regions(T->verdict);
    lb->prefer_regions = fine;
    lb->tile_order = nullptr;
    if (tile_lpt_wanted(switches(), L.ntiles, L.capacity, false, fine)) {
        if ((r = launch_tile_lpt(saved->img, L, (uint32_t)cap, a->debug != 0, s))) return r;
        lb->tile_order = (const uint32_t *)(saved->img + L.i_order);
    }
    if (fine && by_shape) saved->flags |= backward_hint(T->verdict, (uint32_t)BUCKET);
    return DAS3R_OK;
}

int ForwardCall::bin_and_render(bool local_order, bool ctrl_zeroed, uint32_t *count_out, uint32_t count_out_tag, uint32_t *emit_slot) {
    int r;
    const int P = a->P;
    const int64_t cap = L.capacity;
    const bool fused_scan = use_onesweep();
    const bool seg = L.dbits > 0;
    const bool finish = seg && plan.bucket_local;
    if (!emit_slot) {
        if (fused_scan) {
            if ((r = launch_binning_scan_emit(P, cap, out->radii, saved->geom, saved->binning, L, ctrl_zeroed, count_out, count_out_tag, a->debug != 0,
                                              s, local_order || seg))) return r;
        } else if ((r = launch_scan(P, saved->geom, L, nullptr, 0, a->debug != 0, s))) return r;
    }
    uint32_t *host_late = nullptr;
    if (cap > 0 && (r = claim_check_slot(&host_late))) return r;
    uint32_t *dead_keys = nullptr;
    if ((r = launch_binning(P, cap, a->image_width, a->image_height, out->radii, saved->geom, saved->binning, saved->img, L, fused_scan, host_late, late_tag,
                            a->debug != 0, s, &dead_keys, emit_slot, mb->dev + MB_TOO_LONG, plan.gen, finish))) return r;
    if ((r = colour_launch())) return r;
    LocalBin lb = {(float4 *)(saved->binning + L.b_ckpt), nullptr, nullptr, nullptr, nullptr, plan.gen, (uint32_t)(P - 1), (uint32_t)cap};
    if ((r = look_at_lists(&lb))) return r;
    if ((local_order || finish) && cap > 0) {
        lb.point_list = (uint32_t *)(saved->binning + L.pub.point_list);
        lb.slot_list = (uint32_t *)(saved->binning + L.b_slot);
        lb.keys = dead_keys;
        lb.host_flag = mb->dev + MB_TOO_LONG;
        if (finish) lb.dbits = L.dbits, lb.fbits = L.kshift;
    }
    if ((r = colour_join())) return r;
    return launch_render_forward(a, in->colors_precomp, out->out_color, saved->geom, saved->binning, saved->img, L, lb, s, out->out_invdepth,
                                 depth ? (float4 *)(saved->binning + L.d_ckpt) : nullptr);
}

int ForwardCall::read_count(int64_t *I) {
    const int rc = mailbox_wait(mb, MB_COUNT_TAG, count_tag, s);
    if (rc) return rc;
    if (a->prefiltered && mb->host[MB_FILTERED] == count_tag) {
        set_error("Point is filtered although prefiltered is set. This shouldn't happen!");
        return DAS3R_ERR_INVALID_ARG;
    }
    *I = (int64_t)mb->host[MB_COUNT];
    if (*I > CAPACITY_MAX) { set_error("num_rendered %lld exceeds 2^31", (long long)*I); return DAS3R_ERR_OVERFLOW; }
    return DAS3R_OK;
}

int ForwardCall::flow_fused_emit(int64_t *I) {
    int rc;
    if (!T->emit_ring) HIP_TRY(hipMalloc((void **)&T->emit_ring, ARRIVE_SLOTS * EMIT_SLOT_BYTES));
    if (T->emit.wants_zeroing(count_tag)) {
        HIP_TRY(hipMemsetAsync(T->emit_ring, 0, ARRIVE_SLOTS * EMIT_SLOT_BYTES, s));
        T->emit.zeroed();
    }
    uint32_t *emit_slot = (uint32_t *)(T->emit_ring + (size_t)(count_tag % ARRIVE_SLOTS) * EMIT_SLOT_BYTES);
    const EmitArgs em = {(unsigned long long *)(emit_slot + EMIT_SLOT_WORDS), count_tag, emit_slot + 64, emit_slot,
                         (uint32_t *)(saved->binning + L.b_keyA), (uint32_t *)(saved->binning + L.b_gid_of),
                         (uint32_t *)(saved->geom + L.g_off_by_gid), (uint32_t)L.capacity, L.tbits, (uint32_t *)(saved->geom + L.g_count), mb->dev};
    T->emit.taken_by(count_tag);
    if ((rc = preprocess(2, &em))) return rc;
    if ((rc = bin_and_render(true, true, nullptr, 0, emit_slot))) return rc;
    T->emit.rearmed();
    return after_speculation(I);
}

int ForwardCall::flow_speculative(int64_t *I) {
    int rc;
    if ((rc = preprocess(1, nullptr))) return rc;
    if ((rc = bin_and_render(local, true, mb->dev, count_tag))) return rc;
    return after_speculation(I);
}

int ForwardCall::after_speculation(int64_t *I) {
    const int rc = read_count(I);
    if (rc) return rc;
    (void)learn_count(T->verdict, *I, policy_in, plan);
    return *I > L.capacity ? redo_exact(*I) : DAS3R_OK;
}

int ForwardCall::redo_exact(int64_t I) {
    const int rc = layout_and_alloc(I);
    if (rc) return rc;
    HIP_TRY(hipMemsetAsync(saved->geom + L.g_ghist, 0, L.g_ctrl_bytes, s));
    HIP_TRY(hipMemsetAsync(saved->img + L.pub.ranges, 0, 8 * (size_t)L.ntiles, s));
    return bin_and_render(local, false);
}

int ForwardCall::flow_exact(int64_t *I) {
    int rc;
    const int P = a->P;
    const bool seg = plan.seg, debug = a->debug != 0;
    if ((rc = preprocess((local || seg) ? 1 : 0, nullptr))) return rc;
    if (!local && !seg && (rc = launch_depth_sort(P, saved->geom, L, 0, nullptr, 0, debug, s))) return rc;
    if ((rc = read_count(I))) return rc;
    if (learn_count(T->verdict, *I, policy_in, plan)) {
        local = false;
        if ((rc = colour_join())) return rc;
        if ((rc = launch_depth_sort(P, saved->geom, L, 0, nullptr, 0, debug, s))) return rc;
    }
    if ((rc = layout_and_alloc(*I))) return rc;
    if (!local && !seg && (rc = launch_depth_sort(P, saved->geom, L, 1, saved->binning + L.b_ghist, L.b_ctrl_bytes, debug, s))) return rc;
    return bin_and_render(local, !local && !seg);
}

}

using namespace das3r;

extern "C" int das3r_raster_check(const das3r_raster_saved *saved, das3r_stream_t stream) {
    if (!saved) { set_error("das3r_raster_check: null saved state"); return DAS3R_ERR_INVALID_ARG; }
    if (!saved->check_word || !saved->check_tag) return DAS3R_OK;
    const int r = examine_check_slot((volatile uint32_t *)saved->check_word, saved->check_tag, true, (hipStream_t)stream);
    return r < 0 ? r : DAS3R_OK;
}

extern "C" void das3r_get_stats(uint64_t out[4]) {
    for (int i = 0; i < 4; i++) out[i] = (uint64_t)__atomic_load_n(&g_stats[i], __ATOMIC_RELAXED);
}

extern "C" int64_t das3r_raster_forward(const das3r_raster_args *a, const das3r_raster_in *in, const das3r_raster_out *out,
                                        das3r_alloc_fn alloc_geom, das3r_alloc_fn alloc_binning, das3r_alloc_fn alloc_img,
                                        void *user, das3r_raster_saved *saved, das3r_stream_t stream) {
    ForwardCall call = {a, in, out, alloc_geom, alloc_binning, alloc_img, user, saved, (hipStream_t)stream, Join{(hipStream_t)stream}};
    return call.run();
}
```

### das3r_amd/csrc/kernel_choice.h

```cpp
#pragma once
#include <stdint.h>
#include <stdlib.h>
#include <string.h>

#include <algorithm>

namespace das3r {

enum FwdKernel : int {
    FWD_AUTO = 0,
    FWD_QUAD = 1,
    FWD_ROWS = 2,
    FWD_LANES = 3,
    FWD_SLICES = 4,
    FWD_REGIONS = 5,
};
enum BwdKernel : int {
    BWD_AUTO = 0,
    BWD_DPP = 1,
    BWD_MFMA = 2,
    BWD_SCAN = 3,
    BWD_STREAM = 5,
    BWD_BLK = 6,
    BWD_REGIONS = 7,
};
enum RegionStrips : int {
    STRIPS_NONE = 0,
    STRIPS_QUADRANT = 1,
    STRIPS_INTERLEAVED = 2,
};

static inline const char *fwd_kernel_name(FwdKernel k) {
    switch (k) {
        case FWD_QUAD: return "quad";
        case FWD_ROWS: return "rows";
        case FWD_LANES: return "lanes";
        case FWD_SLICES: return "slices";
        case FWD_REGIONS: return "fine";
        default: return "auto";
    }
}
static inline const char *bwd_kernel_name(BwdKernel k) {
    switch (k) {
        case BWD_DPP: return "dpp";
        case BWD_MFMA: return "mfma";
        case BWD_SCAN: return "scan";
        case BWD_STREAM: return "stream";
        case BWD_BLK: return "blk";
        case BWD_REGIONS: return "fine";
        default: return "auto";
    }
}
static inline bool fwd_has_invdepth_form(FwdKernel k) { return k != FWD_SLICES; }
static inline bool bwd_has_invdepth_form(BwdKernel k) { return k != BWD_MFMA && k != BWD_SCAN && k != BWD_STREAM; }

struct Switches {
    int sort_ipl;
    bool sort_classic;
    bool rect_upstream;
    bool verbose;
    int binning;
    bool capacity_exact;
    bool fused_emit_off;
    bool no_sh_stage;
    FwdKernel render_fwd;
    BwdKernel render_bwd;
    int render_bwd_mb;
    bool render_bwd_atomic;
    int tile_chunk;
    int scan_items;
    bool deterministic;
    int render_bwd_occ;
    bool tile_lpt_off;
    int render_bwd_pix;
    RegionStrips render_bwd_strips;
    bool bwd_reduce_set, bwd_reduce_shfl;
    bool ablate_set;
    int ablate;
    int tickets;
    int bwd_pad_lds, fwd_pad_lds;
    int bwd_buckets;
    int inject_fault;
    int mutate;
    bool fwd_no_prefetch;
    int split_colour;
    int tile_strip;
};

template <class Lookup>
static inline Switches parse_switches(Lookup &&lookup, bool experiments) {
    Switches w;
    memset(&w, 0, sizeof(w));
    auto env = [&](const char *k) -> const char * { const char *e = lookup(k); return (e && e[0]) ? e : nullptr; };
    auto number_in = [](const char *e, int none) {
        while (*e && (*e < '0' || *e > '9')) e++;
        return *e ? atoi(e) : none;
    };
    const char *e;
    if (experiments) {
        if ((e = env("DAS3R_SORT_IPL"))) { const int v = atoi(e); w.sort_ipl = (v == 4 || v == 8 || v == 16) ? v : 0; }
        w.sort_classic = (e = env("DAS3R_SORT")) && e[0] == 'c';
        w.no_sh_stage = lookup("DAS3R_NO_SH_STAGE") != nullptr;
        if ((e = env("DAS3R_ABLATE"))) { w.ablate_set = true; w.ablate = atoi(e); }
        if ((e = env("DAS3R_BWD_PAD_LDS"))) w.bwd_pad_lds = atoi(e);
        if ((e = env("DAS3R_FWD_PAD_LDS"))) w.fwd_pad_lds = atoi(e);
        if ((e = env("DAS3R_SCAN_ITEMS"))) { const int v = atoi(e); w.scan_items = (v == 1 || v == 2 || v == 4 || v == 8 || v == 16) ? v : 0; }
        w.fwd_no_prefetch = (e = env("DAS3R_FWD_PREFETCH")) && e[0] == '0';
    }
    w.rect_upstream = (e = env("DAS3R_RECT")) && e[0] == 'u';
    w.verbose = env("DAS3R_VERBOSE") != nullptr;
    if ((e = env("DAS3R_BINNING"))) w.binning = e[0] == 'l' ? 1 : (e[0] == 'r' ? -1 : (e[0] == 's' ? (strchr(e, '3') ? 3 : 2) : (e[0] == 'b' ? 4 : 0)));
    w.capacity_exact = (e = env("DAS3R_CAPACITY")) && e[0] == 'e';
    w.fused_emit_off = (e = env("DAS3R_FUSED_EMIT")) && e[0] == '0';
    if ((e = env("DAS3R_SPLIT_COLOUR"))) w.split_colour = e[0] == '0' ? -1 : (e[0] == '1' ? 1 : 0);
    w.tile_lpt_off = (e = env("DAS3R_TILE_LPT")) && e[0] == '0';
    if ((e = env("DAS3R_RENDER")))
        w.render_fwd = e[0] == 'q' ? FWD_QUAD : (e[0] == 'r' ? FWD_ROWS : (e[0] == 'l' ? FWD_LANES : (e[0] == 's' ? FWD_SLICES : (e[0] == 'f' ? FWD_REGIONS : FWD_AUTO))));
    if ((e = env("DAS3R_RENDER_BWD"))) {
        w.render_bwd = e[0] == 'd' ? BWD_DPP
                     : e[0] == 'm' ? BWD_MFMA
                     : strncmp(e, "stream", 6) == 0 ? BWD_STREAM
                     : e[0] == 's' ? BWD_SCAN
                     : e[0] == 'b' ? BWD_BLK
                     : e[0] == 'f' ? BWD_REGIONS : BWD_AUTO;
        if (w.render_bwd == BWD_BLK) {
            w.render_bwd_mb = number_in(e, 128);
            const char *pp = strchr(e, 'p');
            w.render_bwd_pix = pp ? atoi(pp + 1) : 0;
            const char *po = strchr(e, 'o');
            w.render_bwd_occ = po ? atoi(po + 1) : 5;
        }
        if (w.render_bwd == BWD_REGIONS) {
            w.render_bwd_mb = number_in(e, 128);
            w.render_bwd_strips = strchr(e, 'q') ? STRIPS_QUADRANT : (strchr(e, 's') ? STRIPS_INTERLEAVED : STRIPS_NONE);
        }
        if (w.render_bwd == BWD_SCAN) {
            w.render_bwd_mb = number_in(e, 256);
            w.render_bwd_atomic = strncmp(e, "scana", 5) == 0 || w.render_bwd_mb >= 1000;
        }
    }
    if ((e = env("DAS3R_BWD_REDUCE"))) { w.bwd_reduce_set = true; w.bwd_reduce_shfl = e[0] == 's'; }
    w.tickets = -1;
    if ((e = env("DAS3R_TICKETS"))) w.tickets = e[0] == 'a' ? 0 : (e[0] == 'n' ? 1 << 30 : ((e[0] >= '1' && e[0] <= '9') ? atoi(e) : -1));
    w.deterministic = (e = env("DAS3R_DETERMINISTIC")) && e[0] != '0';
    w.bwd_buckets = -1;
    if ((e = env("DAS3R_BWD_BUCKETS"))) w.bwd_buckets = atoi(e);
    w.tile_strip = 8;
    w.tile_chunk = -1;
    if ((e = env("DAS3R_TILE_CHUNK"))) { const int v = atoi(e); w.tile_chunk = (v >= 0 && v <= 64 && (v & (v - 1)) == 0) ? v : -1; }
    if ((e = env("DAS3R_TILE_STRIP"))) w.tile_strip = std::max(0, std::min(63, atoi(e)));
    return w;
}

constexpr int64_t ROWS_MEAN_LIST = 128;
constexpr int64_t LANES_MEAN_LIST = 1024;
constexpr int FEW_TILES = 1024;

static inline bool quad_lanes(const Switches &sw, int ntiles, int64_t capacity, bool local_lists) {
    if (local_lists) return false;
    if (sw.render_fwd != FWD_AUTO) return sw.render_fwd >= FWD_LANES;
    return ntiles <= FEW_TILES && capacity >= LANES_MEAN_LIST * ntiles;
}
static inline bool row_private(const Switches &sw, int64_t instances, int ntiles) {
    if (sw.render_fwd == FWD_QUAD || sw.render_fwd == FWD_ROWS) return sw.render_fwd == FWD_ROWS;
    return instances >= ROWS_MEAN_LIST * ntiles;
}
static inline FwdKernel choose_forward(const Switches &sw, int ntiles, int64_t capacity, bool local_lists, bool prefer_regions) {
    if (quad_lanes(sw, ntiles, capacity, local_lists)) {
        if (sw.render_fwd == FWD_SLICES) return FWD_SLICES;
        if (sw.render_fwd == FWD_REGIONS || (sw.render_fwd == FWD_AUTO && prefer_regions)) return FWD_REGIONS;
        return FWD_LANES;
    }
    return row_private(sw, capacity, ntiles) ? FWD_ROWS : FWD_QUAD;
}
static inline bool tile_lpt_wanted(const Switches &sw, int ntiles, int64_t capacity, bool local_lists, bool prefer_regions) {
    return prefer_regions && capacity > 0 && quad_lanes(sw, ntiles, capacity, local_lists) && ntiles <= FEW_TILES && !sw.tile_lpt_off &&
           (sw.render_fwd == FWD_AUTO || sw.render_fwd == FWD_REGIONS);
}

constexpr int BUCKET = 1024;
constexpr int64_t BLK_MEAN_LIST = 96;
constexpr int64_t LONG_MEAN_LIST = 1024;
constexpr int MAX_SLICES = 32, MAX_HINT_SLICES = 64;
constexpr int MAX_BUCKET_MB = 256;

struct BwdChoice {
    BwdKernel kernel;
    int mb;
    int slices;
    int pix, occ;
    RegionStrips strips;
    bool atomic_flush;
};

static inline BwdChoice choose_backward(const Switches &sw, int64_t num_rendered, int ntiles, uint32_t fwd_flags) {
    BwdKernel kind = sw.render_bwd;
    int mb = sw.render_bwd_mb ? sw.render_bwd_mb : 256;
    const int64_t tiles = std::max(ntiles, 1);
    if (kind == BWD_AUTO) {
        const int64_t mean_list = num_rendered / tiles;
        const bool long_lists = mean_list >= BLK_MEAN_LIST;
        kind = (sw.bwd_reduce_set || sw.ablate_set || !long_lists) ? BWD_DPP : BWD_BLK;
        mb = mean_list >= LONG_MEAN_LIST ? 192 : 128;
        if (kind == BWD_BLK && mean_list >= LONG_MEAN_LIST && ntiles <= FEW_TILES && (fwd_flags & 1u) && !sw.ablate_set) {
            kind = BWD_REGIONS;
            mb = 128;
        }
        if (sw.deterministic && kind == BWD_DPP) {
            kind = BWD_BLK;
            mb = 64;
        }
    }
    BwdChoice c = {kind, mb, 1, 0, 5, STRIPS_NONE, false};
    if (kind == BWD_SCAN || kind == BWD_BLK || kind == BWD_REGIONS) {
        int slices = sw.bwd_buckets;
        if (slices < 0) slices = (int)std::min<int64_t>(MAX_SLICES, std::max<int64_t>(1, num_rendered / ((int64_t)BUCKET * tiles)));
        c.atomic_flush = kind == BWD_SCAN && sw.render_bwd_atomic;
        if (slices > 1 && (mb > MAX_BUCKET_MB || c.atomic_flush)) slices = 1;
        const int hint = (int)((fwd_flags >> 8) & 0xFFu);
        if (sw.bwd_buckets < 0 && kind == BWD_REGIONS && slices > 1 && hint > slices) slices = std::min(hint, MAX_HINT_SLICES);
        c.slices = slices;
    }
    c.pix = sw.render_bwd == BWD_BLK ? sw.render_bwd_pix : (mb == 128 ? 1 : 0);
    c.occ = sw.render_bwd_occ == 4 ? 4 : 5;
    if (sw.render_bwd == BWD_REGIONS) c.strips = sw.render_bwd_strips;
    return c;
}

#define DAS3R_SWITCH_FIELDS(X)                                                                                                              \
    X(sort_ipl) X(sort_classic) X(rect_upstream) X(verbose) X(binning) X(capacity_exact) X(fused_emit_off) X(no_sh_stage) X(render_bwd_mb) \
    X(render_bwd_atomic) X(tile_chunk) X(scan_items) X(deterministic) X(render_bwd_occ) X(tile_lpt_off) X(render_bwd_pix) X(bwd_reduce_set) \
    X(bwd_reduce_shfl) X(ablate_set) X(ablate) X(tickets) X(bwd_pad_lds) X(fwd_pad_lds) X(bwd_buckets) X(fwd_no_prefetch) X(split_colour)   \
    X(tile_strip)
template <class S>
static inline Switches switches_from(const S &s) {
    Switches w;
    memset(&w, 0, sizeof(w));
#define X(f) w.f = static_cast<decltype(w.f)>(s.f);
    DAS3R_SWITCH_FIELDS(X)
#undef X
    w.render_fwd = static_cast<FwdKernel>(s.render_fwd);
    w.render_bwd = static_cast<BwdKernel>(s.render_bwd);
    w.render_bwd_strips = static_cast<RegionStrips>(s.render_bwd_strips);
    return w;
}
template <class S>
static inline void switches_to(const Switches &w, S *s) {
#define X(f) s->f = static_cast<int32_t>(w.f);
    DAS3R_SWITCH_FIELDS(X)
#undef X
    s->render_fwd = w.render_fwd;
    s->render_bwd = w.render_bwd;
    s->render_bwd_strips = w.render_bwd_strips;
}
#undef DAS3R_SWITCH_FIELDS

}
```

### das3r_amd/csrc/path_policy.h

```cpp
#pragma once
#include <stdint.h>

#include <algorithm>

namespace das3r {

constexpr int64_t LOCAL_AVG = 384;
constexpr int64_t SEG_AVG = 384;
constexpr int64_t BUCKET_LOCAL_AVG = 256;
constexpr int BUCKET_LOCAL_TILES = 1024;
constexpr int BUCKET_LOCAL_DBITS = 2;
constexpr uint32_t CROWDED16 = 23u * 16u;
constexpr uint32_t FINE_PERIOD = 512;
constexpr int BACKOFF_MIN = 64, BACKOFF_MAX = 4096;
constexpr uint32_t CLEAN_RESET = 256;
constexpr int64_t CAPACITY_MAX = 0x7FFFFF00;

static inline int seg_dbits(int tbits, int passes) { return 8 * (passes < 3 ? passes : 3) - tbits; }

static inline uint32_t next_gen(uint32_t gen) { return gen + 1u ? gen + 1u : 1u; }

static inline bool bucket_local_rule(int forced, bool onesweep, int tbits, int tile_passes, int ntiles, int64_t last_I, int radix_left) {
    if (!onesweep || seg_dbits(tbits, tile_passes) < BUCKET_LOCAL_DBITS) return false;
    if (forced == 4) return true;
    return forced == 0 && radix_left == 0 && ntiles > BUCKET_LOCAL_TILES && last_I > BUCKET_LOCAL_AVG * ntiles && last_I <= LOCAL_AVG * ntiles;
}

struct Verdict {
    int P = 0, W = 0, H = 0;
    int64_t last_I = -1;
    int64_t peak_I = 0;
    int radix_left = 0;
    int backoff = BACKOFF_MIN;
    uint32_t gen = 0;
    int seg_extra = 0;
    bool last_seg = false;
    bool fine = false;
    uint32_t forwards = 0;
    uint32_t clean = 0;
    uint32_t longest = 0;
    static Verdict fresh(uint32_t gen) {
        Verdict v;
        v.gen = gen;
        return v;
    }
};

struct Resume {
    bool valid = false, fine = false;
    uint32_t forwards = 0;
};

struct PolicyInputs {
    int P, W, H;
    int ntiles, tbits, tile_passes;
    uint32_t too_long;
    uint32_t want_bits;
    int forced;
    bool onesweep;
    int64_t capacity_hint;
    bool capacity_exact;
    Resume *resume;
};

struct ForwardPlan {
    bool local, seg;
    bool bucket_local;
    int seg_bits, seg_passes;
    bool speculate;
    int64_t cap;
    bool decide_fine;
    uint32_t gen;
};

static inline ForwardPlan plan_forward(Verdict &v, const PolicyInputs &in) {
    if (v.P != in.P || v.W != in.W || v.H != in.H) {
        v = Verdict::fresh(next_gen(v.gen));
        v.P = in.P;
        v.W = in.W;
        v.H = in.H;
        if (in.resume && in.resume->valid) {
            v.fine = in.resume->fine;
            v.forwards = in.resume->forwards;
            in.resume->valid = false;
        }
    }
    ForwardPlan p;
    p.decide_fine = (v.forwards++ & (FINE_PERIOD - 1u)) == 0u;
    if (v.last_I < 0) {
    } else if (in.too_long == v.gen && !(v.last_seg && v.seg_extra == 0 && in.tile_passes < 3 && seg_dbits(in.tbits, in.tile_passes + 1) > 0)) {
        if (v.clean >= CLEAN_RESET) v.backoff = BACKOFF_MIN;
        v.radix_left = v.backoff;
        if (v.backoff < BACKOFF_MAX) v.backoff *= 2;
        v.clean = 0;
        v.gen = next_gen(v.gen);
    } else if (in.too_long == v.gen || in.want_bits == v.gen) {
        v.seg_extra = 1;
        v.gen = next_gen(v.gen);
    }
    const int forced = in.forced;
    p.bucket_local = bucket_local_rule(forced, in.onesweep, in.tbits, in.tile_passes, in.ntiles, v.last_I, v.radix_left);
    p.local = !p.bucket_local && in.onesweep && (forced == 1 || forced == 4 || (forced == 0 && v.radix_left == 0 && v.last_I <= LOCAL_AVG * in.ntiles));
    p.seg_passes = in.tile_passes + ((!p.bucket_local && (forced == 3 || (forced == 0 && v.seg_extra))) ? 1 : 0);
    p.seg_bits = (in.onesweep && p.seg_passes <= 3) ? seg_dbits(in.tbits, p.seg_passes) : 0;
    p.seg = p.bucket_local || (!p.local && p.seg_bits > 0 && (forced == 2 || forced == 3 || (forced == 0 && v.radix_left == 0 && v.last_I >= 0 &&
                                                                                              (v.last_I >> std::min(p.seg_bits, 20)) <= SEG_AVG * in.ntiles)));
    v.last_seg = p.seg && !p.bucket_local;
    if (p.local || p.seg) v.clean++;
    if (forced == 0 && v.radix_left > 0) v.radix_left--;
    p.speculate = (p.local || p.seg) && v.last_I >= 0 && in.capacity_hint != -1 && !in.capacity_exact;
    p.cap = p.speculate ? std::min(std::max(v.last_I + v.last_I / 4, v.peak_I + v.peak_I / 20) + 4096, CAPACITY_MAX) : 0;
    p.gen = v.gen;
    return p;
}

static inline bool learn_count(Verdict &v, int64_t I, const PolicyInputs &in, const ForwardPlan &p) {
    v.last_I = I;
    v.peak_I = std::max(I, v.peak_I - v.peak_I / 1024);
    return p.local && in.forced == 0 && I > LOCAL_AVG * in.ntiles;
}

static inline int64_t skew_mean(const Verdict &v, int64_t cap, int ntiles) { return (v.last_I > 0 ? v.last_I : cap) / std::max(ntiles, 1); }

static inline bool learn_skew(Verdict &v, uint32_t longest32, uint32_t crowd16, int64_t cap, int ntiles) {
    const int64_t longest = (int64_t)longest32, mean = skew_mean(v, cap, ntiles);
    v.longest = longest32;
    v.fine = (longest > mean + (mean * 4) / 5 && longest >= 4096) || crowd16 >= CROWDED16;
    return v.fine;
}

static inline uint32_t backward_hint(const Verdict &v, uint32_t bucket) { return 1u | (std::min<uint32_t>(63u, v.longest / bucket + 2u) << 8); }

static inline bool prefers_regions(const Verdict &v) { return v.fine; }
static inline uint32_t forwards_seen(const Verdict &v) { return v.forwards; }

static inline void forget(Verdict &v) { v = Verdict::fresh(v.gen); }

static inline void resume(Verdict &v, Resume &r, bool fine, uint32_t forwards) {
    forget(v);
    r.valid = true;
    r.fine = fine;
    r.forwards = forwards;
}

template <class S>
static inline void policy_state_from(const S &s, Verdict *v, Resume *r) {
    v->P = s.P, v->W = s.W, v->H = s.H;
    v->last_I = s.last_I, v->peak_I = s.peak_I;
    v->radix_left = s.radix_left, v->backoff = s.backoff;
    v->gen = s.gen;
    v->seg_extra = s.seg_extra;
    v->last_seg = s.last_seg != 0, v->fine = s.fine != 0;
    v->forwards = s.forwards, v->clean = s.clean, v->longest = s.longest;
    r->valid = s.resume_valid != 0, r->fine = s.resume_fine != 0, r->forwards = s.resume_forwards;
}
template <class S>
static inline void policy_state_to(const Verdict &v, const Resume &r, S *s) {
    s->P = v.P, s->W = v.W, s->H = v.H;
    s->last_I = v.last_I, s->peak_I = v.peak_I;
    s->radix_left = v.radix_left, s->backoff = v.backoff;
    s->gen = v.gen;
    s->seg_extra = v.seg_extra;
    s->last_seg = v.last_seg, s->fine = v.fine;
    s->forwards = v.forwards, s->clean = v.clean, s->longest = v.longest;
    s->resume_valid = r.valid, s->resume_fine = r.fine, s->resume_forwards = r.forwards;
}

}
```

### das3r_amd/csrc/render_common.h

```cpp
#pragma once
#include "common.h"

namespace das3r {

struct StagedSplat {
    float4 xyh;
    float4 co;
    float4 rgbd;
};

__device__ __forceinline__ float4 lds_read4(const float4 *p) {
    const float4 v = *p;
    asm volatile("" ::"v"(v.w));
    return v;
}

__device__ __forceinline__ StagedSplat null_splat() {
    StagedSplat z;
    z.xyh = make_float4(0.f, 0.f, -1e30f, -1e30f);
    z.co = make_float4(0.f, 0.f, 0.f, 0.f);
    z.rgbd = make_float4(0.f, 0.f, 0.f, 0.f);
    return z;
}

__device__ __forceinline__ void lds_barrier() {
    __builtin_amdgcn_fence(__ATOMIC_RELEASE, "workgroup", "local");
    __builtin_amdgcn_s_barrier();
    __builtin_amdgcn_fence(__ATOMIC_ACQUIRE, "workgroup", "local");
}

__device__ __forceinline__ int packed_ntiles(const int packed) { return packed & 0x3FFFFF; }
__device__ __forceinline__ int xcd_tile(const int block, const int packed, const int tiles_x) {
    const int ntiles = packed & 0x3FFFFF, code = (packed >> 22) & 7, SH = (int)((unsigned)packed >> 25);
    int k;
    if (code == 0) {
        const int per = (ntiles + 7) >> 3;
        k = (block & 7) * per + (block >> 3);
    } else {
        const int lg = code - 1, j = block >> 3;
        k = ((((j >> lg) << 3) + (block & 7)) << lg) + (j & ((1 << lg) - 1));
    }
    if (k >= ntiles) return -1;
    if (SH == 0) return k;
    const int tiles_y = ntiles / tiles_x;
    const int strip = k / (SH * tiles_x);
    const int rem = k - strip * SH * tiles_x;
    const int h = min(SH, tiles_y - SH * strip);
    const int bx = rem / h, by = SH * strip + (rem - bx * h);
    return by * tiles_x + bx;
}
static inline int tile_chunk_code(const int ntiles) {
    const int forced = switches().tile_chunk;
    if (forced == 0) return 0;
    int c = 64;
    if (forced > 0) c = forced;
    else while (c > 1 && ntiles / c < 64) c >>= 1;
    int lg = 0;
    while ((1 << lg) < c) lg++;
    return lg + 1;
}
static inline int pack_tiles(const Layout &L) {
    const uint32_t sh = (L.capacity >= (int64_t)128 * L.ntiles) ? (uint32_t)std::min(switches().tile_strip, 63) : 0u;
    return (int)(((uint32_t)L.ntiles & 0x3FFFFFu) | ((uint32_t)tile_chunk_code(L.ntiles) << 22) | (sh << 25));
}
static inline int xcd_grid(const Layout &L) {
    const int code = tile_chunk_code(L.ntiles);
    if (code == 0) return ((L.ntiles + 7) / 8) * 8;
    const int ch = 1 << (code - 1), nchunks = (L.ntiles + ch - 1) / ch;
    return ((nchunks + 7) / 8) * 8 * ch;
}

__device__ __forceinline__ void quadrant_pixel(const int bx, const int by, const int wave, const int lane, int &px, int &py) {
    px = bx * TILE_X + ((wave & 1) << 3) + (lane & 7);
    py = by * TILE_Y + ((wave >> 1) << 3) + (lane >> 3);
}

__device__ __forceinline__ bool pair_alpha(const float x, const float y, const float4 co, const float px, const float py, float &dx,
                                           float &dy, float &G, float &alpha) {
    dx = x - px;
    dy = y - py;
    const float q = __fmaf_rn(__fmul_rn(co.x, dx), dx, __fmul_rn(__fmul_rn(co.z, dy), dy));
    const float power = __fmaf_rn(-0.5f, q, -__fmul_rn(__fmul_rn(co.y, dx), dy));
    G = __expf(power);
    alpha = fminf(0.99f, __fmul_rn(co.w, G));
    return (!(power > 0.0f)) & (alpha >= (1.0f / 255.0f));
}


__device__ __forceinline__ float min_clamp01(const float a, const float b) {
    float r;
    asm("v_min_f32_e64 %0, %1, %2 clamp" : "=v"(r) : "v"(a), "v"(b));
    return r;
}
__device__ __forceinline__ float fma_clamp01(const float a, const float b, const float c) {
    float r;
    asm("v_fma_f32 %0, %1, %2, %3 clamp" : "=v"(r) : "v"(a), "v"(b), "v"(c));
    return r;
}
__device__ __forceinline__ float alpha_if_visible(const float a1, const float power) {
    const float m = fminf(a1 - (1.0f / 255.0f), -power);
    return min_clamp01(a1, __fmaf_rn(1e30f, m, a1));
}
struct PixelBlend {
    float T, C0, C1, C2, live, lastf;
    float D;
};
__device__ __forceinline__ float4 staged_invz(const float4 r) {
    return make_float4(r.x, r.y, r.z, 1.0f / r.w);
}
template <bool DEPTH = false>
__device__ __forceinline__ void blend_pair(PixelBlend &px, const float alpha, const float4 c, const float jf) {
    const float a = alpha * px.live;
    const float test_T = px.T * (1.0f - a);
    const float s = fma_clamp01(test_T, 0x1p100f, -__uint_as_float(0x6AD1B716u) );
    const float w = a * s;
    const float wT = w * px.T;
    px.C0 = __fmaf_rn(c.x, wT, px.C0);
    px.C1 = __fmaf_rn(c.y, wT, px.C1);
    px.C2 = __fmaf_rn(c.z, wT, px.C2);
    if constexpr (DEPTH) px.D = __fmaf_rn(c.w, wT, px.D);
    px.T = px.T * (1.0f - w);
    px.live *= s;
    px.lastf = fmaxf(px.lastf, fminf(jf, __fmaf_rn(w, 1e30f, -1.0f)));
}
__device__ __forceinline__ void blend_batch_begin(PixelBlend &px) { px.lastf = -1.0f; }
__device__ __forceinline__ uint32_t blend_batch_end(const PixelBlend &px, const uint32_t last_contributor, const uint32_t batch_first) {
    return px.lastf >= 0.0f ? batch_first + (uint32_t)px.lastf + 1u : last_contributor;
}

__device__ __forceinline__ uint2 safe_range(uint2 r, const uint32_t cap) {
    r.y = min(r.y, cap);
    r.x = min(r.x, r.y);
    return r;
}

__device__ __forceinline__ bool quadrant_hit(const float4 xyh, const float cx, const float cy) {
    return fabsf(xyh.x - cx) <= xyh.z + 3.5f && fabsf(xyh.y - cy) <= xyh.w + 3.5f;
}

__device__ __forceinline__ void diagonal_extents(const float4 xyh, const float4 co, float &hd1, float &hd2) {
    const float ex = (xyh.z - 0.02f) * (1.0f / 1.0005f), ey = (xyh.w - 0.02f) * (1.0f / 1.0005f);
    const float ex2 = ex * ex, ey2 = ey * ey, txy = -co.y * ex2 * __builtin_amdgcn_rcpf(co.z);
    const float half = 0.5f * (ex2 + ey2), slack = 2e-6f * (ex2 + ey2) + 1e-3f;
    hd1 = __builtin_amdgcn_sqrtf(fmaxf(half + txy, 0.f) + slack) * 1.0005f + 0.05f;
    hd2 = __builtin_amdgcn_sqrtf(fmaxf(half - txy, 0.f) + slack) * 1.0005f + 0.05f;
}
__device__ __forceinline__ bool block_hit_oct(const float x, const float y, const float hx, const float hy, const float hd1, const float hd2,
                                              const float cx, const float cy) {
    const float ddx = x - cx, ddy = y - cy;
    constexpr float RS2 = 0.70710678f, HALF_DIAG = 2.1213204f + 1e-3f;
    return (fabsf(ddx) <= hx + 1.5f) & (fabsf(ddy) <= hy + 1.5f) & (fabsf(ddx + ddy) * RS2 <= hd1 + HALF_DIAG) &
           (fabsf(ddx - ddy) * RS2 <= hd2 + HALF_DIAG);
}

__device__ __forceinline__ uint32_t region_mask(const float4 p, const float qcx0, const float qcy0) {
    uint32_t xb = 0, yb = 0;
    const float hx = p.z + 0.5f, hy = p.w + 0.5f;
#pragma unroll
    for (int k = 0; k < 4; k++) {
        xb |= (fabsf(p.x - (qcx0 + (float)(2 * k))) <= hx ? 1u : 0u) << k;
        yb |= (fabsf(p.y - (qcy0 + (float)(2 * k))) <= hy ? 1u : 0u) << k;
    }
    return ((yb & 1u) ? xb : 0u) | ((yb & 2u) ? xb << 4 : 0u) | ((yb & 4u) ? xb << 8 : 0u) | ((yb & 8u) ? xb << 12 : 0u);
}

__device__ __forceinline__ float4 *ckpt_slot(float4 *ckpt, const uint2 range, const int tile, const int s) {
    return ckpt + ((size_t)(range.x / BUCKET) + (size_t)tile + (size_t)s) * TILE_PIX;
}
__device__ __forceinline__ int ckpt_buckets(const uint2 range) { return (int)((range.y - range.x + BUCKET - 1) / BUCKET); }

__device__ __forceinline__ void ce64(double &lo, double &hi) {
    double a, b;
    asm("v_min_f64 %0, %2, %3\n\tv_max_f64 %1, %2, %3" : "=&v"(a), "=&v"(b) : "v"(lo), "v"(hi));
    lo = a;
    hi = b;
}
constexpr unsigned long long SORT_PAD = 0x7FEFFFFFFFFFFFFFull;

template <int g, int E>
__device__ __forceinline__ void butterfly_group(double *key, const int lane, const int R) {
    const int s = R - g;
#pragma unroll
    for (int c = 0; c < (E >> g); c++) {
        const int gid = c * 64 + lane;
        const int base = ((gid >> s) << R) | (gid & ((1 << s) - 1));
        double e[1 << g];
#pragma unroll
        for (int m = 0; m < (1 << g); m++) e[m] = key[base + (m << s)];
#pragma unroll
        for (int t = g - 1; t >= 0; t--)
#pragma unroll
            for (int m = 0; m < (1 << g); m++)
                if (!((m >> t) & 1)) ce64(e[m], e[m | (1 << t)]);
#pragma unroll
        for (int m = 0; m < (1 << g); m++) key[base + (m << s)] = e[m];
    }
}

template <int G>
__device__ __forceinline__ void wave_bitonic_sort(double *key, const int lane) {
    constexpr int E = 1 << G, H = E / 2, LOGN = 6 + G;
    {
        double v[E];
#pragma unroll
        for (int m = 0; m < E; m++) v[m] = key[lane * E + m];
#pragma unroll
        for (int lk = 1; lk <= G; lk++) {
#pragma unroll
            for (int i = 0; i < E; i++)
                if (!(i & (1 << (lk - 1)))) ce64(v[i], v[i ^ ((1 << lk) - 1)]);
#pragma unroll
            for (int lj = lk - 2; lj >= 0; lj--)
#pragma unroll
                for (int i = 0; i < E; i++)
                    if (!((i >> lj) & 1)) ce64(v[i], v[i | (1 << lj)]);
        }
#pragma unroll
        for (int m = 0; m < E; m++) key[lane * E + m] = v[m];
    }
    __builtin_amdgcn_fence(__ATOMIC_ACQ_REL, "wavefront");
    for (int lk = G + 1; lk <= LOGN; lk++) {
        {
            const int sh = lk - G;
            const int block = lane >> sh, hbase = lane & ((1 << sh) - 1);
            const int lo0 = (block << lk) + hbase, hi0 = (block << lk) + ((1 << lk) - 1) - hbase;
            double a[H], b[H];
#pragma unroll
            for (int m = 0; m < H; m++) {
                a[m] = key[lo0 + (m << sh)];
                b[m] = key[hi0 - (m << sh)];
            }
#pragma unroll
            for (int m = 0; m < H; m++) ce64(a[m], b[m]);
#pragma unroll
            for (int t = G - 2; t >= 0; t--)
#pragma unroll
                for (int m = 0; m < H; m++)
                    if (!((m >> t) & 1)) {
                        ce64(a[m], a[m | (1 << t)]);
                        ce64(b[m | (1 << t)], b[m]);
                    }
#pragma unroll
            for (int m = 0; m < H; m++) {
                key[lo0 + (m << sh)] = a[m];
                key[hi0 - (m << sh)] = b[m];
            }
        }
        __builtin_amdgcn_fence(__ATOMIC_ACQ_REL, "wavefront");
        for (int R = lk - G; R > 0;) {
            const int g = R < G ? R : G;
            if (g == 1) butterfly_group<1, E>(key, lane, R);
            else if (g == 2) butterfly_group<2, E>(key, lane, R);
            else if (g == 3) butterfly_group<3, E>(key, lane, R);
            __builtin_amdgcn_fence(__ATOMIC_ACQ_REL, "wavefront");
            R -= g;
        }
    }
}

__device__ __forceinline__ void rank_below(uint32_t &rank, const uint32_t kj, const uint32_t ki) {
    uint32_t tmp;
    asm("v_sub_co_u32 %1, vcc, %2, %3\n\tv_addc_co_u32 %0, vcc, 0, %0, vcc" : "+v"(rank), "=&v"(tmp) : "v"(kj), "v"(ki) : "vcc");
}
struct NoMark {
    __device__ __forceinline__ void operator()(int) const {}
};
template <bool DEPTH = false, class Mark = NoMark>
__device__ __forceinline__ bool local_order_tile(const LocalBin &lb, const uint2 range, const float4 *__restrict__ xyh,
                                                 const float4 *__restrict__ conic_opacity, const float4 *__restrict__ rgbd,
                                                 StagedSplat *stage , uint32_t *s_gid , const int tid,
                                                 const Mark mark = Mark()) {
    const int n = (int)(range.y - range.x);
    uint32_t *pl = lb.point_list + range.x, *sl = lb.slot_list + range.x;
    if (n <= TILE_PIX) {
        unsigned long long *s_key = reinterpret_cast<unsigned long long *>(s_gid);
        unsigned long long key = 0;
        uint32_t g = 0, slot = 0;
        float4 r0 = make_float4(0.f, 0.f, 0.f, 0.f), r1 = r0, r2 = r0;
        if (tid < n) {
            g = min(pl[tid], lb.last_g);
            slot = sl[tid];
            r0 = xyh[(size_t)g * SPLAT_REC];
            r1 = conic_opacity[(size_t)g * SPLAT_REC];
            r2 = rgbd[(size_t)g * SPLAT_REC];
            key = ((unsigned long long)__float_as_uint(r2.w) << 32) | (unsigned long long)g;
        }
        if (tid < ((n + 7) & ~7)) s_key[tid] = tid < n ? key : ~0ull;
        __syncthreads();
        if (tid < n) {
            int rank = 0;
            for (int j = 0; j < n; j += 8) {
                unsigned long long o[8];
#pragma unroll
                for (int u = 0; u < 8; u++) o[u] = s_key[j + u];
#pragma unroll
                for (int u = 0; u < 8; u++) rank += o[u] < key ? 1 : 0;
            }
            stage[rank].xyh = r0;
            stage[rank].co = r1;
            if constexpr (DEPTH) stage[rank].rgbd = staged_invz(r2);
            else stage[rank].rgbd = r2;
            pl[rank] = g;
            sl[rank] = slot;
        } else {
            stage[tid] = null_splat();
        }
        return true;
    }
    if (lb.dbits > 0 && n <= 2 * TILE_PIX) {
        uint32_t *s_word = reinterpret_cast<uint32_t *>(stage), *s_byrank = s_word + 2 * TILE_PIX + 8, *s_depth = s_byrank + 2 * TILE_PIX + 8;
        uint32_t *s_lo = s_depth + 2 * TILE_PIX, *s_hi = s_lo + 128;
        const uint32_t *kk = lb.keys + range.x;
        const int wsh = lb.fbits + 9;
        const uint32_t kmask = (1u << (lb.dbits + lb.fbits)) - 1u;
        uint32_t g[2], slot[2], w[2], rank[2];
#pragma unroll
        for (int u = 0; u < 2; u++) {
            const int i = u * TILE_PIX + tid;
            g[u] = slot[u] = 0u;
            rank[u] = 0xFFFFFFFFu;
            w[u] = 0xFFFFFFFFu;
            if (i < n) {
                g[u] = min(pl[i], lb.last_g);
                slot[u] = sl[i];
                w[u] = ((kk[i] & kmask) << 9) | (uint32_t)i;
            }
            s_word[i] = w[u];
        }
        if (tid < 8) s_word[2 * TILE_PIX + tid] = 0xFFFFFFFFu;
        __syncthreads();
#pragma unroll
        for (int u = 0; u < 2; u++) {
            const int i = u * TILE_PIX + tid;
            if (i < n) {
                const uint32_t b = w[u] >> wsh, before = i ? s_word[i - 1] >> wsh : 0xFFFFFFFFu;
                if (before != b) {
                    s_lo[b] = (uint32_t)i;
                    if (i) s_hi[before] = (uint32_t)i;
                }
                if (i == n - 1) s_hi[b] = (uint32_t)n;
            }
        }
        __syncthreads();
#pragma unroll
        for (int u = 0; u < 2; u++) {
            const int i = u * TILE_PIX + tid;
            if (i < n) {
                const uint32_t b = w[u] >> wsh, lo = min(s_lo[b], (uint32_t)n) & ~3u, hi = min(s_hi[b], (uint32_t)n);
                uint32_t r = lo;
                for (uint32_t j = lo; j < hi; j += 8u) {
                    const uint4 o = *reinterpret_cast<const uint4 *>(s_word + j), q = *reinterpret_cast<const uint4 *>(s_word + j + 4u);
                    rank_below(r, o.x, w[u]);
                    rank_below(r, o.y, w[u]);
                    rank_below(r, o.z, w[u]);
                    rank_below(r, o.w, w[u]);
                    rank_below(r, q.x, w[u]);
                    rank_below(r, q.y, w[u]);
                    rank_below(r, q.z, w[u]);
                    rank_below(r, q.w, w[u]);
                }
                rank[u] = min(r, (uint32_t)(n - 1));
                s_byrank[rank[u]] = w[u];
            }
        }
        __syncthreads();
        bool tied[2];
#pragma unroll
        for (int u = 0; u < 2; u++) {
            const uint32_t r = rank[u], f = w[u] >> 9;
            tied[u] = r != 0xFFFFFFFFu && ((r > 0u && (s_byrank[r - 1u] >> 9) == f) || (r + 1u < (uint32_t)n && (s_byrank[r + 1u] >> 9) == f));
            if (tied[u]) s_depth[r] = __float_as_uint(rgbd[(size_t)g[u] * SPLAT_REC].w);
        }
        __syncthreads();
#pragma unroll
        for (int u = 0; u < 2; u++)
            if (tied[u]) {
                const uint32_t r = rank[u], f = w[u] >> 9, mine = s_depth[r], at = w[u] & 0x1FFu;
                uint32_t a = r, b = r + 1u, below = 0u;
                while (a > 0u && (s_byrank[a - 1u] >> 9) == f) a--;
                while (b < (uint32_t)n && (s_byrank[b] >> 9) == f) b++;
                for (uint32_t k = a; k < b; k++) {
                    const uint32_t dk = s_depth[k], pk = s_byrank[k] & 0x1FFu;
                    below += (dk < mine || (dk == mine && pk < at)) ? 1u : 0u;
                }
                rank[u] = a + below;
            }
#pragma unroll
        for (int u = 0; u < 2; u++)
            if (rank[u] != 0xFFFFFFFFu) s_gid[rank[u]] = g[u];
        __syncthreads();
#pragma unroll
        for (int u = 0; u < 2; u++)
            if (rank[u] != 0xFFFFFFFFu) {
                pl[rank[u]] = g[u];
                sl[rank[u]] = slot[u];
            }
        return false;
    }
    if (n <= LOCAL_MAX) {
        unsigned long long *s_key = reinterpret_cast<unsigned long long *>(stage);
        uint32_t *s_slot = reinterpret_cast<uint32_t *>(stage) + 2 * LOCAL_MAX;
        const int N = n <= 2 * TILE_PIX ? 2 * TILE_PIX : LOCAL_MAX;
        for (int i = tid; i < N; i += TILE_PIX) {
            unsigned long long k = SORT_PAD;
            if (i < n) {
                const uint32_t g = min(pl[i], lb.last_g);
                s_gid[i] = g;
                s_slot[i] = sl[i];
                k = ((unsigned long long)__float_as_uint(rgbd[(size_t)g * SPLAT_REC].w) << 32) | (unsigned long long)i;
            }
            s_key[i] = k;
        }
        __syncthreads();
        mark(6);
        if (N == 2 * TILE_PIX) {
            if (tid < 64) wave_bitonic_sort<3>(reinterpret_cast<double *>(stage), tid);
        } else {
            bool wide_before = false;
            for (int lk = 1; (1 << (lk - 1)) < n; lk++)
                for (int lj = lk - 1; lj >= 0; lj--) {
                    const bool wide = lj > 6;
                    if (wide || wide_before) __syncthreads();
                    else __builtin_amdgcn_fence(__ATOMIC_ACQ_REL, "wavefront");
                    wide_before = wide;
                    for (int pr = tid; pr < (N >> 1); pr += TILE_PIX) {
                        const int i = ((pr >> lj) << (lj + 1)) | (pr & ((1 << lj) - 1));
                        const int q = (lj == lk - 1) ? (i ^ ((2 << lj) - 1)) : (i | (1 << lj));
                        if (q < n) {
                            const unsigned long long a = s_key[i], b = s_key[q];
                            if (a > b) {
                                s_key[i] = b;
                                s_key[q] = a;
                            }
                        }
                    }
                }
        }
        __syncthreads();
        mark(7);
        uint32_t g[LOCAL_MAX / TILE_PIX], slot[LOCAL_MAX / TILE_PIX];
#pragma unroll
        for (int u = 0; u < LOCAL_MAX / TILE_PIX; u++) {
            const int i = u * TILE_PIX + tid;
            const int from = i < n ? (int)((uint32_t)s_key[i] & (uint32_t)(LOCAL_MAX - 1)) : 0;
            g[u] = s_gid[from];
            slot[u] = s_slot[from];
        }
        __syncthreads();
#pragma unroll
        for (int u = 0; u < LOCAL_MAX / TILE_PIX; u++) {
            const int i = u * TILE_PIX + tid;
            if (i < n) {
                s_gid[i] = g[u];
                pl[i] = g[u];
                sl[i] = slot[u];
            }
        }
        __syncthreads();
        return false;
    }
    uint32_t *dk = lb.keys + range.x;
    if (tid == 0) __hip_atomic_store(lb.host_flag, lb.flag_value, __ATOMIC_RELAXED, __HIP_MEMORY_SCOPE_SYSTEM);
    for (int i = tid; i < n; i += TILE_PIX) dk[i] = __float_as_uint(rgbd[(size_t)min(pl[i], lb.last_g) * SPLAT_REC].w);
    __syncthreads();
    for (int k = 2; (k >> 1) < n; k <<= 1)
        for (int j = k >> 1; j > 0; j >>= 1) {
            const int flip = (j == (k >> 1)) ? k - 1 : j;
            for (int i = tid; i < n; i += TILE_PIX) {
                const int q = i ^ flip;
                if (q > i && q < n) {
                    const uint32_t da = dk[i], db = dk[q], ga = pl[i], gb = pl[q];
                    if (da > db || (da == db && ga > gb)) {
                        dk[i] = db; dk[q] = da;
                        pl[i] = gb; pl[q] = ga;
                        const uint32_t t = sl[i];
                        sl[i] = sl[q];
                        sl[q] = t;
                    }
                }
            }
            __syncthreads();
        }
    return false;
}

template <int CTRL>
__device__ __forceinline__ float dpp_add_full(float v) {
    return v + __int_as_float(__builtin_amdgcn_update_dpp(0, __float_as_int(v), CTRL, 0xf, 0xf, true));
}
__device__ __forceinline__ float swap32_add(const float a, const float b) {
    const auto r = __builtin_amdgcn_permlane32_swap(__float_as_uint(a), __float_as_uint(b), false, false);
    return __uint_as_float(r[0]) + __uint_as_float(r[1]);
}
__device__ __forceinline__ float swap16_add(const float a, const float b) {
    const auto r = __builtin_amdgcn_permlane16_swap(__float_as_uint(a), __float_as_uint(b), false, false);
    return __uint_as_float(r[0]) + __uint_as_float(r[1]);
}
__device__ __forceinline__ float wave_reduce8_transposed(const float v[8], const int lane) {
    const float r0 = swap32_add(v[0], v[4]), r1 = swap32_add(v[1], v[5]);
    const float r2 = swap32_add(v[2], v[6]), r3 = swap32_add(v[3], v[7]);
    const float s02 = swap16_add(r0, r2);
    const float s13 = swap16_add(r1, r3);
    const float t0 = dpp_add_full<0x128>(s02);
    const float t1 = dpp_add_full<0x128>(s13);
    float m = (lane & 8) ? t1 : t0;
    m = dpp_add_full<0x141>(m);
    m = dpp_add_full<0x1B>(m);
    m = dpp_add_full<0xB1>(m);
    return m;
}

struct ReplayState {
    float T, R;
};
__device__ __forceinline__ void replay_pair(const bool active, const float alpha, const float G, const float dx, const float dy,
                                            const float4 co, const float4 c, const float dLp0, const float dLp1, const float dLp2,
                                            const float tfbg, const float ddelx_dx, const float ddely_dy, ReplayState &st, float v[9]) {
    const float am = active ? alpha : 0.f, Gm = active ? G : 0.f;
    const float rinv = __builtin_amdgcn_rcpf(1.f - am);
    st.T = st.T * rinv;
    const float w = am * st.T;
    const float cd = c.x * dLp0 + c.y * dLp1 + c.z * dLp2;
    const float dL_dalpha = st.T * cd - (st.R + tfbg) * rinv;
    st.R = st.R + cd * w;
    const float gdl = Gm * dL_dalpha;
    const float hd = -0.5f * co.w * gdl;
    const float gx = hd * dx, gy = hd * dy;
    v[0] = w * dLp0;
    v[1] = w * dLp1;
    v[2] = w * dLp2;
    v[3] = (gx * co.x + gy * co.y) * (2.0f * ddelx_dx);
    v[4] = (gy * co.z + gx * co.y) * (2.0f * ddely_dy);
    v[5] = gx * dx;
    v[6] = gx * dy;
    v[7] = gy * dy;
    v[8] = gdl;
}

__device__ __forceinline__ void replay_pair_moments(const bool active, const float alpha, const float G, const float dx, const float dy,
                                                    const float4 c, const float dLp0, const float dLp1, const float dLp2, const float tfbg,
                                                    ReplayState &st, float v[9]) {
    const float am = active ? alpha : 0.f, Gm = active ? G : 0.f;
    const float rinv = __builtin_amdgcn_rcpf(1.f - am);
    st.T = st.T * rinv;
    const float w = am * st.T;
    const float cd = c.x * dLp0 + c.y * dLp1 + c.z * dLp2;
    const float dL_dalpha = st.T * cd - (st.R + tfbg) * rinv;
    st.R = st.R + cd * w;
    const float g = Gm * dL_dalpha;
    const float gx = g * dx, gy = g * dy;
    v[0] = w * dLp0;
    v[1] = w * dLp1;
    v[2] = w * dLp2;
    v[3] = gx;
    v[4] = gy;
    v[5] = gx * dx;
    v[6] = gx * dy;
    v[7] = gy * dy;
    v[8] = g;
}
__device__ __forceinline__ void moments_to_sums(float *a , const float4 co, const float ddelx_dx, const float ddely_dy) {
    const float hd = -0.5f * co.w;
    const float m1 = a[3], m2 = a[4];
    a[3] = hd * (co.x * m1 + co.y * m2) * (2.0f * ddelx_dx);
    a[4] = hd * (co.z * m2 + co.y * m1) * (2.0f * ddely_dy);
    a[5] = hd * a[5];
    a[6] = hd * a[6];
    a[7] = hd * a[7];
}

}
```

### das3r_amd/csrc/sort.hip

```cpp
#include "granule.h"
#include "segkey.h"
#include <algorithm>
#include "splat_math.h"

namespace das3r {

template <int IPL>
__global__ void __launch_bounds__(256) radix_hist_kernel(const uint32_t *__restrict__ keys, uint32_t cap, const uint32_t *__restrict__ n_ptr,
                                                         int shift, uint32_t mask, int nchunks, uint32_t *__restrict__ hist) {
    const uint32_t n = n_ptr ? min(*n_ptr, cap) : cap;
    __shared__ uint32_t cnt[SORT_WAVES_PER_BLOCK][RADIX_SIZE];
    const int lane = __lane_id(), wave = threadIdx.x >> 6;
    const int chunk = blockIdx.x * SORT_WAVES_PER_BLOCK + wave;
    const uint32_t base = (uint32_t)chunk * 64u * (uint32_t)IPL;
    uint32_t k[IPL];
#pragma unroll
    for (int s = 0; s < IPL; s++) {
        const uint32_t i = base + s * 64 + lane;
        k[s] = (chunk < nchunks && i < n) ? keys[i] : 0u;
    }
#pragma unroll
    for (int d = lane; d < RADIX_SIZE; d += 64) cnt[wave][d] = 0;
    __builtin_amdgcn_wave_barrier();
    if (chunk >= nchunks) return;
#pragma unroll
    for (int s = 0; s < IPL; s++) {
        const uint32_t i = base + s * 64 + lane;
        if (i < n) atomicAdd(&cnt[wave][(k[s] >> shift) & mask], 1u);
    }
    __builtin_amdgcn_wave_barrier();
#pragma unroll
    for (int d = lane; d < RADIX_SIZE; d += 64) hist[(size_t)d * nchunks + chunk] = cnt[wave][d];
}

__global__ void __launch_bounds__(256) radix_rowscan_kernel(uint32_t *__restrict__ hist, int nchunks, uint32_t *__restrict__ totals) {
    __shared__ uint32_t ws[4];
    uint32_t *row = hist + (size_t)blockIdx.x * nchunks;
    uint32_t carry = 0;
    for (int base = 0; base < nchunks; base += 256) {
        const int i = base + threadIdx.x;
        const uint32_t v = i < nchunks ? row[i] : 0;
        uint32_t tot;
        const uint32_t ex = block_exclusive_scan_256(v, ws, &tot);
        if (i < nchunks) row[i] = carry + ex;
        carry += tot;
    }
    if (threadIdx.x == 0) totals[blockIdx.x] = carry;
}

template <int IPL>
__global__ void __launch_bounds__(256) radix_scatter_kernel(const uint32_t *__restrict__ keys_in, const uint32_t *__restrict__ vals_in,
                                                            uint32_t *__restrict__ keys_out, uint32_t *__restrict__ vals_out,
                                                            uint32_t cap, const uint32_t *__restrict__ n_ptr, int shift, int bits,
                                                            int nchunks, const uint32_t *__restrict__ hist,
                                                            const uint32_t *__restrict__ totals, const uint32_t *__restrict__ gather_src,
                                                            uint32_t *__restrict__ inv_out) {
    const uint32_t n = n_ptr ? min(*n_ptr, cap) : cap;
    __shared__ uint32_t off_s[SORT_WAVES_PER_BLOCK][RADIX_SIZE];
    const int lane = __lane_id(), wave = threadIdx.x >> 6;
    const int chunk = blockIdx.x * SORT_WAVES_PER_BLOCK + wave;
    if (chunk >= nchunks) return;
    volatile uint32_t *off = off_s[wave];
    const uint32_t mask = (1u << bits) - 1u;
    const uint32_t base = (uint32_t)chunk * 64u * (uint32_t)IPL;

    uint32_t k[IPL], v[IPL], out[IPL];
#pragma unroll
    for (int s = 0; s < IPL; s++) {
        const uint32_t i = base + s * 64 + lane;
        k[s] = i < n ? keys_in[i] : 0u;
        v[s] = (vals_in && i < n) ? vals_in[i] : i;
    }
#pragma unroll
    for (int s = 0; s < IPL; s++) {
        const uint32_t i = base + s * 64 + lane;
        out[s] = (gather_src && i < n) ? gather_src[v[s]] : v[s];
    }
    {
        uint32_t t[4], h[4], sum = 0;
#pragma unroll
        for (int q = 0; q < 4; q++) {
            t[q] = totals[4 * lane + q];
            h[q] = hist[(size_t)(4 * lane + q) * nchunks + chunk];
            sum += t[q];
        }
        uint32_t ex = wave_incl_scan_u32(sum) - sum;
#pragma unroll
        for (int q = 0; q < 4; q++) {
            off[4 * lane + q] = ex + h[q];
            ex += t[q];
        }
    }
    __builtin_amdgcn_wave_barrier();

#pragma unroll
    for (int s = 0; s < IPL; s++) {
        const uint32_t i = base + s * 64 + lane;
        const bool valid = i < n;
        const uint32_t digit = (k[s] >> shift) & mask;
        uint64_t peers = __ballot(valid);
        for (int b = 0; b < bits; b++) {
            const bool bit = (digit >> b) & 1u;
            const uint64_t m = __ballot(valid && bit);
            peers &= bit ? m : ~m;
        }
        const uint64_t lt = (1ull << lane) - 1ull;
        const uint32_t rank = (uint32_t)__popcll(peers & lt);
        const uint32_t count = (uint32_t)__popcll(peers);
        uint32_t o = 0;
        if (valid) o = off[digit];
        __builtin_amdgcn_wave_barrier();
        if (valid && rank == 0) off[digit] = o + count;
        __builtin_amdgcn_wave_barrier();
        if (valid) {
            const uint32_t dst = o + rank;
            if (keys_out) keys_out[dst] = k[s];
            vals_out[dst] = out[s];
            if (inv_out) inv_out[dst] = v[s];
        }
    }
}

static int radix_pass(const uint32_t *kin, const uint32_t *vin, uint32_t *kout, uint32_t *vout, int64_t n, int shift, int bits,
                      uint32_t *hist, uint32_t *totals, bool debug, hipStream_t s, const uint32_t *gather_src = nullptr,
                      uint32_t *inv_out = nullptr, const uint32_t *n_ptr = nullptr) {
    const int ipl = sort_items_per_lane(n), nchunks = sort_num_chunks(n);
    const int nblocks = div_up(nchunks, SORT_WAVES_PER_BLOCK);
    const uint32_t mask = (1u << bits) - 1u;
#define HIST(IPL) DAS3R_LAUNCH((radix_hist_kernel<IPL>), dim3(nblocks), dim3(256), 0, s, kin, (uint32_t)n, n_ptr, shift, mask, nchunks, hist)
#define SCAT(IPL)                                                                                                             \
    DAS3R_LAUNCH((radix_scatter_kernel<IPL>), dim3(nblocks), dim3(256), 0, s, kin, vin, kout, vout, (uint32_t)n, n_ptr, shift, bits, \
                 nchunks, hist, totals, gather_src, inv_out)
    if (ipl == 4) HIST(4); else if (ipl == 8) HIST(8); else HIST(16);
    KERNEL_CHECK(s, debug, "radix_hist");
    DAS3R_LAUNCH(radix_rowscan_kernel, dim3(RADIX_SIZE), dim3(256), 0, s, hist, nchunks, totals);
    KERNEL_CHECK(s, debug, "radix_rowscan");
    if (ipl == 4) SCAT(4); else if (ipl == 8) SCAT(8); else SCAT(16);
    KERNEL_CHECK(s, debug, "radix_scatter");
#undef HIST
#undef SCAT
    return DAS3R_OK;
}

int radix_sort_u32_pairs(const uint32_t *keys_in, uint32_t *keyA, uint32_t *keyB, uint32_t *valA, uint32_t *valB, int64_t n,
                         int total_bits, uint32_t *hist, uint32_t *totals, uint32_t **vals_final, hipStream_t s) {
    (void)keys_in;
    const int passes = (total_bits + 7) / 8;
    uint32_t *kin = keyA, *kout = keyB, *vin = nullptr, *vout = valB;
    int shift = 0;
    for (int p = 0; p < passes; p++) {
        const int bits = (total_bits - shift) < 8 ? (total_bits - shift) : 8;
        const bool last = p == passes - 1;
        int rc = radix_pass(kin, vin, last ? nullptr : kout, vout, n, shift, bits, hist, totals, false, s);
        if (rc) return rc;
        shift += bits;
        uint32_t *t = kin; kin = kout; kout = t;
        vin = vout;
        vout = (vout == valB) ? valA : valB;
    }
    *vals_final = vin;
    return DAS3R_OK;
}

#ifdef DAS3R_EXPERIMENTS
__global__ void __launch_bounds__(256) emit_kernel(int P, int tiles_x, int tiles_y, const uint32_t *__restrict__ sorted_idx,
                                                   const uint32_t *__restrict__ tiles_touched, const uint32_t *__restrict__ offsets,
                                                   const float4 *__restrict__ xyh, const int32_t *__restrict__ radii,
                                                   uint32_t *__restrict__ tile_keys, uint32_t *__restrict__ gids, uint32_t cap,
                                                   uint32_t *__restrict__ ghist , int tbits, int tight_rect) {
    __shared__ uint32_t h[4][RADIX_SIZE];
    if (ghist) {
#pragma unroll
        for (int q = 0; q < 4; q++) h[q][threadIdx.x] = 0;
        __syncthreads();
    }
    for (int r = blockIdx.x * blockDim.x + threadIdx.x; r < P; r += gridDim.x * blockDim.x) {
        const uint32_t g = sorted_idx[r];
        if (tiles_touched[g] == 0) continue;
        uint32_t o = offsets[r];
        const float4 p = xyh[(size_t)g * SPLAT_REC];
        int rminx, rminy, rmaxx, rmaxy;
        binned_rect(p, radii[g], tiles_x, tiles_y, tight_rect != 0, rminx, rminy, rmaxx, rmaxy);
        for (int y = rminy; y < rmaxy; y++)
            for (int x = rminx; x < rmaxx; x++) {
                if (o < cap) {
                    const uint32_t t = (uint32_t)(y * tiles_x + x);
                    tile_keys[o] = t;
                    gids[o] = g;
                    if (ghist) {
                        for (int q = 0, sh = 0, dw = tile_digit_width(tbits); sh < tbits; q++, sh += dw) {
                            const int bits = (tbits - sh) < dw ? (tbits - sh) : dw;
                            atomicAdd(&h[q][(t >> sh) & ((1u << bits) - 1u)], 1u);
                        }
                    }
                }
                o++;
            }
    }
    if (ghist) {
        __syncthreads();
        for (int q = 0, sh = 0, dw = tile_digit_width(tbits); sh < tbits; q++, sh += dw) {
            const uint32_t c = h[q][threadIdx.x];
            if (c) atomicAdd(&ghist[q * RADIX_SIZE + threadIdx.x], c);
        }
    }
}

#endif

__global__ void __launch_bounds__(256) tile_ranges_kernel(uint32_t cap, const uint32_t *__restrict__ n_ptr,
                                                          const uint32_t *__restrict__ tile_keys, uint2 *__restrict__ ranges,
                                                          uint32_t *__restrict__ err, uint32_t *__restrict__ host_late, uint32_t tag,
                                                          uint32_t rearm_words ,
                                                          uint32_t inject ,
                                                          int dbits ) {
    const uint32_t I = n_ptr ? min(*n_ptr, cap) : cap;
    const uint32_t i = blockIdx.x * blockDim.x + threadIdx.x;
    if (i == 0 && host_late) {
        host_late[0] = *err | inject;
        __hip_atomic_store(host_late + 1, tag, __ATOMIC_RELEASE, __HIP_MEMORY_SCOPE_SYSTEM);
    }
    if (i < rearm_words) err[i] = 0u;
    const uint32_t i0 = 4u * i;
    if (i0 >= I) return;
    uint32_t k[4];
    if (i0 + 4u <= I) {
        const uint4 v = *reinterpret_cast<const uint4 *>(tile_keys + i0);
        k[0] = v.x; k[1] = v.y; k[2] = v.z; k[3] = v.w;
    } else {
#pragma unroll
        for (int q = 0; q < 4; q++) k[q] = i0 + q < I ? tile_keys[i0 + q] : 0u;
    }
    uint32_t prev = i0 ? tile_keys[i0 - 1u] >> dbits : 0u;
#pragma unroll
    for (int q = 0; q < 4; q++) {
        const uint32_t at = i0 + (uint32_t)q;
        if (at < I) {
            const uint32_t t = k[q] >> dbits;
            if (at == 0u) ranges[t].x = 0u;
            else if (prev != t) {
                ranges[prev].y = at;
                ranges[t].x = at;
            }
            if (at == I - 1u) ranges[t].y = I;
            prev = t;
        }
    }
}

int launch_depth_sort(int P, char *geom, const Layout &L, int part, char *binning_ctrl, size_t binning_ctrl_bytes, bool debug, hipStream_t s) {
    uint32_t *keyA = (uint32_t *)(geom + L.g_keyA), *keyB = (uint32_t *)(geom + L.g_keyB);
    uint32_t *valA = (uint32_t *)(geom + L.g_valA), *valB = (uint32_t *)(geom + L.g_valB);
    uint32_t *hist = (uint32_t *)(geom + L.g_hist), *totals = (uint32_t *)(geom + L.g_totals);
    if (P == 0) return DAS3R_OK;
    int rc;
    if (use_onesweep()) return launch_onesweep_depth_sort(P, geom, L, part, (uint32_t *)binning_ctrl, (uint32_t)(binning_ctrl_bytes / 4), debug, s);
#ifdef DAS3R_EXPERIMENTS
    if (part == 1) return DAS3R_OK;
    if ((rc = radix_pass(keyA, nullptr, keyB, valB, P, 0, 8, hist, totals, debug, s))) return rc;
    if ((rc = radix_pass(keyB, valB, keyA, valA, P, 8, 8, hist, totals, debug, s))) return rc;
    if ((rc = radix_pass(keyA, valA, keyB, valB, P, 16, 8, hist, totals, debug, s))) return rc;
    if ((rc = radix_pass(keyB, valB, nullptr, valA, P, 24, 8, hist, totals, debug, s))) return rc;
#else
    (void)keyA; (void)keyB; (void)valA; (void)valB; (void)hist; (void)totals; (void)rc;
#endif
    return DAS3R_OK;
}

int launch_binning_scan_emit(int P, int64_t I, const int32_t *radii, char *geom, char *binning, const Layout &L, bool ctrl_zeroed,
                             uint32_t *host_out, uint32_t tag, bool debug, hipStream_t s, bool index_order) {
    if (I == 0 || P == 0) return DAS3R_OK;
    if (!ctrl_zeroed) HIP_TRY(hipMemsetAsync(binning + L.b_ghist, 0, L.b_ctrl_bytes, s));
    return launch_scan_emit(P, I, radii, geom, binning, L, host_out, tag, debug, s, index_order);
}

int launch_binning(int P, int64_t I, int W, int H, const int32_t *radii, char *geom, char *binning, char *img, const Layout &L,
                   bool fused_scan, uint32_t *host_late, uint32_t tag, bool debug, hipStream_t s, uint32_t **dead_keys, uint32_t *emit_slot,
                   uint32_t *seg_host_flag, uint32_t seg_flag_value, bool local_finish) {
    const uint32_t *n_ptr = (const uint32_t *)(geom + L.g_count);
    (void)W; (void)H;
    uint2 *ranges = (uint2 *)(img + L.pub.ranges);
    if (I == 0 || P == 0) return DAS3R_OK;
    uint32_t *keyA = (uint32_t *)(binning + L.b_keyA), *keyB = (uint32_t *)(binning + L.b_keyB);
    uint32_t *valA = (uint32_t *)(binning + L.b_valA), *valB = (uint32_t *)(binning + L.b_valB);
    uint32_t *hist = (uint32_t *)(binning + L.b_hist), *totals = (uint32_t *)(binning + L.b_totals);
    uint32_t *gid_of = (uint32_t *)(binning + L.b_gid_of), *inv = (uint32_t *)(binning + L.b_slot);
    const bool onesweep = use_onesweep();
    (void)onesweep;
#ifdef DAS3R_EXPERIMENTS
    if (!fused_scan) {
    const int emit_blocks = div_up(P, 256) < 1024 ? div_up(P, 256) : 1024;
    DAS3R_LAUNCH(emit_kernel, dim3(emit_blocks), dim3(256), 0, s, P, L.tiles_x, L.tiles_y,
                 (const uint32_t *)(geom + L.pub.sorted_idx), (const uint32_t *)(geom + L.pub.tiles_touched),
                 (const uint32_t *)(geom + L.pub.offsets), (const float4 *)(geom + L.pub.xy), radii, keyA, gid_of, (uint32_t)I,
                 onesweep ? (uint32_t *)(binning + L.b_ghist) : (uint32_t *)nullptr, L.tbits, use_tight_rect() ? 1 : 0);
    KERNEL_CHECK(s, debug, "emit");
    }
#else
    (void)radii; (void)fused_scan; (void)gid_of;
#endif
    if (onesweep) {
        uint32_t *kfinal = nullptr;
        int rc1 = launch_onesweep_partition(I, geom, binning, L, &kfinal, debug, s, emit_slot ? emit_slot + 64 : nullptr, emit_slot);
        if (rc1) return rc1;
        if (dead_keys) *dead_keys = kfinal;
        if (L.dbits > 0 && !local_finish) {
            uint32_t *other = kfinal == keyA ? keyB : keyA;
            return launch_segment_sort(I, n_ptr, kfinal, L.kshift, (uint32_t *)(binning + L.pub.point_list), (uint32_t *)(binning + L.b_slot),
                                       (const uint32_t *)(geom + L.pub.depth_key), (uint32_t)(P - 1), other, seg_host_flag, seg_flag_value, debug, s,
                                       L.dbits, ranges, (const uint32_t *)(geom + L.g_ticket) + 8, host_late, tag, (uint32_t)switches().inject_fault);
        }
        const int rearm = emit_slot ? EMIT_SLOT_WORDS : 0;
        DAS3R_LAUNCH(tile_ranges_kernel, dim3(div_up(std::max<int64_t>(div_up(I, 4), rearm), 256)), dim3(256), 0, s, (uint32_t)I, n_ptr, kfinal, ranges,
                     emit_slot ? emit_slot : (uint32_t *)(geom + L.g_ticket) + 8, host_late, tag, (uint32_t)rearm, (uint32_t)switches().inject_fault, L.dbits + L.kshift);
        KERNEL_CHECK(s, debug, "tile_ranges");
        return DAS3R_OK;
    }
#ifdef DAS3R_EXPERIMENTS
    uint32_t *kin = keyA, *vin = nullptr, *kout = keyB, *vout = valB;
    int shift = 0, rc;
    for (int p = 0; p < L.tile_passes; p++) {
        const int dw = tile_digit_width(L.tbits), bits = (L.tbits - shift) < dw ? (L.tbits - shift) : dw;
        const bool last = p == L.tile_passes - 1;
        if ((rc = radix_pass(kin, vin, kout, vout, I, shift, bits, hist, totals, debug, s, last ? gid_of : nullptr, last ? inv : nullptr, n_ptr)))
            return rc;
        shift += bits;
        uint32_t *t = kin; kin = kout; kout = t;
        vin = vout;
        vout = (vout == valB) ? valA : valB;
    }
    if (dead_keys) *dead_keys = kin;
    DAS3R_LAUNCH(tile_ranges_kernel, dim3(div_up(div_up(I, 4), 256)), dim3(256), 0, s, (uint32_t)I, n_ptr, kin, ranges,
                 (uint32_t *)(geom + L.g_ticket) + 8, host_late, tag, 0u, (uint32_t)switches().inject_fault, 0);
    KERNEL_CHECK(s, debug, "tile_ranges");
#else
    (void)keyA; (void)keyB; (void)valA; (void)valB; (void)hist; (void)totals; (void)inv;
#endif
    return DAS3R_OK;
}

}
```

### das3r_amd/roofline.py

```python

HBM_PEAK_GBS = 8000.0

BINNING_KERNELS = ("radix_hist_kernel", "radix_rowscan_kernel", "radix_scatter_kernel", "depth_hist_kernel", "onesweep_pass_kernel",
                   "scan_emit_kernel", "emit_kernel", "tile_ranges_kernel", "segment_sort_kernel")


def algorithmic_bytes(P, D, M, I, W, H):
    npix = W * H
    inp = P * (44 + 12 * (D + 1) ** 2)
    per_kernel = {
        "preprocess_kernel": inp + 4 * P,
        "binning": 12 * I,
        "render_forward_kernel": 48 * I + 12 * npix,
        "render_backward_kernel": 20 * npix + 40 * I,
        "preprocess_backward_kernel": inp + 56 * P + 12 * M * P,
    }
    b_fwd = inp + 4 * P + 60 * I + 12 * npix
    b_bwd = 20 * npix + 40 * I + inp + 56 * P + 12 * M * P
    assert sum(per_kernel.values()) == b_fwd + b_bwd
    return per_kernel, b_fwd, b_bwd


ALIASES = {"preprocess_geometry_kernel": "preprocess_kernel",
           "sh_colour_kernel": "preprocess_kernel",
           "render_forward_rows_kernel": "render_forward_kernel",
           "render_forward_lanes_kernel": "render_forward_kernel",
           "render_backward_mfma_kernel": "render_backward_kernel",
           "render_backward_scan_kernel": "render_backward_kernel",
           "render_backward_blk_kernel": "render_backward_kernel",
           "render_forward_regions_kernel": "render_forward_kernel",
           "render_forward_slices_kernel": "render_forward_kernel",
           "render_backward_regions_kernel": "render_backward_kernel"}


def group_kernel_times(report):
    out = {}
    for name, (n, ms) in report.items():
        key = "binning" if name in BINNING_KERNELS else ALIASES.get(name, name)
        c, t = out.get(key, (0, 0.0))
        out[key] = (c + n, t + ms)
    return out


WALK_VALU_PER_64_PAIRS = {"render_forward_kernel": 35, "render_backward_kernel": 50}
SIMDS, CLOCK_HZ, CYCLES_PER_VALU = 1024, 2.4e9, 2.0


def valu_roofline(kernel, live_pairs, ms):
    n = WALK_VALU_PER_64_PAIRS[kernel]
    insts = live_pairs / 64.0 * n
    ideal_ms = insts * CYCLES_PER_VALU / (SIMDS * CLOCK_HZ) * 1e3
    return {"ideal_valu_insts": int(insts), "ideal_ms": round(ideal_ms, 5), "frac": round(ideal_ms / ms, 4) if ms > 0 else None,
            "def": f"live_pairs / 64 x {n} wave instructions x 2 cycles / (1024 SIMDs x 2.4 GHz) / measured ms"}
```

### include/das3r_raster.h

```cpp
#ifndef DAS3R_RASTER_H
#define DAS3R_RASTER_H

#include <stddef.h>
#include <stdint.h>

#ifdef __cplusplus
extern "C" {
#endif

#define DAS3R_ABI_VERSION 16

typedef enum {
    DAS3R_OK = 0,
    DAS3R_ERR_INVALID_ARG = -1,
    DAS3R_ERR_HIP = -2,
    DAS3R_ERR_ALLOC = -3,
    DAS3R_ERR_OVERFLOW = -4
} das3r_status;

typedef void *das3r_stream_t;

typedef char *(*das3r_alloc_fn)(void *user, size_t bytes);

typedef struct {
    int32_t P;
    int32_t sh_degree;
    int32_t M;
    int32_t image_width;
    int32_t image_height;
    float tanfovx;
    float tanfovy;
    float scale_modifier;
    const float *bg;
    const float *viewmatrix;
    const float *projmatrix;
    const float *campos;
    int32_t prefiltered;
    int32_t debug;
    int64_t capacity_hint;
} das3r_raster_args;

typedef struct {
    const float *xyz;
    const float *rot;
    const float *scaling;
    const float *opacity_raw;
    const float *conf_flat;
    const int64_t *mask_index;
    const float *R, *t, *Lq;
} das3r_pretransform;

typedef struct {
    const float *means3D;
    const float *opacities;
    const float *shs;
    const float *colors_precomp;
    const float *scales;
    const float *rotations;
    const float *cov3D_precomp;
    const das3r_pretransform *pre;
} das3r_raster_in;

typedef struct {
    float *out_color;
    int32_t *radii;
    float *out_invdepth;
} das3r_raster_out;

typedef struct {
    char *geom;
    char *binning;
    char *img;
    int64_t num_rendered;
    int64_t capacity;
    void *check_word;
    uint32_t check_tag;
    uint32_t flags;
} das3r_raster_saved;

typedef struct {
    float *dL_dmeans2D;
    float *dL_dopacities;
    float *dL_dmeans3D;
    float *dL_dshs;
    float *dL_dcolors_precomp;
    float *dL_dscales;
    float *dL_drotations;
    float *dL_dcov3D;
    float *scratch;
    const struct das3r_chain_s *chain;
} das3r_raster_grads;

int64_t das3r_raster_forward(const das3r_raster_args *args, const das3r_raster_in *in, const das3r_raster_out *out,
                             das3r_alloc_fn alloc_geom, das3r_alloc_fn alloc_binning, das3r_alloc_fn alloc_img,
                             void *alloc_user, das3r_raster_saved *saved, das3r_stream_t stream);

int das3r_raster_backward(const das3r_raster_args *args, const das3r_raster_in *in, const das3r_raster_saved *saved,
                          const float *dL_dpix , const das3r_raster_grads *grads, das3r_stream_t stream);

size_t das3r_raster_backward_scratch_bytes(int64_t capacity);

int das3r_raster_backward_depth(const das3r_raster_args *args, const das3r_raster_in *in, const das3r_raster_saved *saved,
                                const float *dL_dpix , const float *dL_dinvdepth , const das3r_raster_grads *grads,
                                das3r_stream_t stream);
size_t das3r_raster_backward_depth_scratch_bytes(int64_t capacity);

size_t das3r_raster_focal_workspace_bytes(int32_t P);
int das3r_raster_backward_focal(const das3r_raster_args *args, const das3r_raster_in *in, const das3r_raster_saved *saved,
                                const float *dL_dpix , const float *dL_dinvdepth ,
                                const das3r_raster_grads *grads, float *sums , float *per_splat , float *workspace,
                                das3r_stream_t stream);

int das3r_raster_check(const das3r_raster_saved *saved, das3r_stream_t stream);

int das3r_mark_visible(int32_t P, const float *means3D, const float *viewmatrix, const float *projmatrix,
                       uint8_t *present, das3r_stream_t stream);

size_t das3r_knn3_workspace_bytes(int32_t P);
int das3r_knn3_mean_dist2(int32_t P, const float *points , float *out , char *workspace,
                          das3r_stream_t stream);


int das3r_pose_matrices(const float *pose, float *mats, das3r_stream_t stream);
int das3r_pose_chain(const float *pose, const float *g_mats, float *g_pose, das3r_stream_t stream);
int das3r_pose_matrices_qt(const float *q, const float *t, float *mats, das3r_stream_t stream);
int das3r_pose_chain_qt(const float *q, float *g_mats, float *g_q, float *g_t, das3r_stream_t stream);
int das3r_pose_chain_qt_rearm(const float *q, float *g_mats, float *g_q, float *g_t, float *zero_q, float *zero_t, das3r_stream_t stream);
int das3r_pretransform_forward(int32_t P, const float *xyz, const float *rot, const float *scaling, const float *opacity_raw,
                               const float *conf_flat, const int64_t *mask_index, const float *R, const float *t, const float *Lq,
                               float *means3D, float *rotations, float *scales, float *opacities, das3r_stream_t stream);
int das3r_pretransform_backward(int32_t P, const float *xyz, const float *rot, const float *scaling, const float *opacity_raw,
                                const float *conf_flat, const int64_t *mask_index, const float *R, const float *Lq,
                                const float *g_means3D, const float *g_rot, const float *g_scales, const float *g_opac, float *g_xyz,
                                float *g_rotation, float *g_scaling, float *g_opacity_raw, float *g_conf_flat, float *g_small,
                                das3r_stream_t stream);

typedef struct {
    float *param;
    const float *grad;
    float *exp_avg;
    float *exp_avg_sq;
    int64_t rows;
    int32_t row_len;
    int32_t active_len;
    float step_size;
    float bc2_sqrt;
    int32_t head_len;
    float step_size_tail;
    int32_t grad_row_len;
    int32_t state_row_len;
    float *mirror;
    int32_t mirror_row_len;
} das3r_adam_tensor;
int das3r_adam_step(int32_t n, const das3r_adam_tensor *tensors, float beta1, float beta2, float eps, das3r_stream_t stream);
int das3r_adam_step_gated(int32_t n, const das3r_adam_tensor *tensors, float beta1, float beta2, float eps, const float *gate,
                          float threshold, int32_t *state, das3r_stream_t stream);

typedef struct das3r_chain_s {
    float *g_conf_flat;
    float *g_small;
    const struct das3r_adam_slot_s *slots;
    float beta1, beta2, eps;
} das3r_chain;

typedef struct das3r_adam_slot_s {
    float *param, *exp_avg, *exp_avg_sq;
    float step_size, bc2_sqrt;
} das3r_adam_slot;
int das3r_pretransform_backward_adam(int32_t P, const float *conf_flat, const int64_t *mask_index, const float *R, const float *Lq,
                                     const float *g_means3D, const float *g_rot, const float *g_scales, const float *g_opac,
                                     float *g_conf_flat, float *g_small, const das3r_adam_slot *slots, float beta1, float beta2, float eps,
                                     das3r_stream_t stream);
int das3r_pretransform_pose_sums(int32_t P, const float *xyz, const float *rot, const float *R, const float *Lq, const float *g_means3D,
                                 const float *g_rot, float *g_small, das3r_stream_t stream);

int64_t das3r_photometric_blocks(int32_t H, int32_t W);
int das3r_photometric_forward(int32_t H, int32_t W, const float *render, const float *gt, const float *static_mask, float lambda,
                              float *partials, float *dmaps, das3r_stream_t stream);
int das3r_photometric_finish(int32_t H, int32_t W, const float *partials, float lambda, float *out8, das3r_stream_t stream);
int das3r_photometric_backward(int32_t H, int32_t W, const float *render, const float *gt, const float *static_mask, float lambda,
                               const float *dmaps, const float *grad_loss, float *d_render, float *d_static, das3r_stream_t stream);
int das3r_ssim_map_forward(int32_t H, int32_t W, const float *img1, const float *img2, float *ssim_map, float *dmaps, float *partials,
                           das3r_stream_t stream);
int das3r_ssim_map_backward(int32_t H, int32_t W, const float *img1, const float *img2, const float *dmaps, const float *grad_map,
                            float *d_img1, float *d_img2, das3r_stream_t stream);
int das3r_photometric_backward_finish(int32_t H, int32_t W, const float *render, const float *gt, const float *static_mask, float lambda,
                                      const float *dmaps, const float *grad_loss, float *d_render, float *d_static, const float *partials,
                                      float *out8, das3r_stream_t stream);

int das3r_photometric_forward_exposure(int32_t H, int32_t W, const float *render, const float *gt, const float *static_mask, float lambda,
                                       const float *exposure, float *partials, float *dmaps, das3r_stream_t stream);
int das3r_photometric_backward_finish_exposure(int32_t H, int32_t W, const float *render, const float *gt, const float *static_mask, float lambda,
                                               const float *exposure, const float *dmaps, const float *grad_loss, float *d_render,
                                               float *d_static, const float *partials, float *out8, float *epartials, das3r_stream_t stream);
int das3r_exposure_grad_finish(int32_t H, int32_t W, const float *epartials, float *grad_row, float *zero_row, das3r_stream_t stream);

int64_t das3r_depth_l1_blocks(int32_t H, int32_t W);
int das3r_depth_l1(int32_t H, int32_t W, const float *invdepth, const float *target, const float *mask, const float *static_mask, float weight,
                   const float *grad_loss, float *d_invdepth, float *partials, float *out8, das3r_stream_t stream);

#define DAS3R_PRUNE_GROUP_ROWS 1024
#define DAS3R_PRUNE_COUNT_WORDS(P) (1 + ((int64_t)(P) + DAS3R_PRUNE_GROUP_ROWS - 1) / DAS3R_PRUNE_GROUP_ROWS)
typedef struct {
    const void *src;
    void *dst;
    int64_t row_bytes;
} das3r_prune_tensor;
int das3r_prune_select(int32_t P, const float *opacity_raw, const float *conf_flat, const int64_t *mask_index, float min_opacity,
                       const float *scaling, float max_world_scale, const uint8_t *also_drop, int32_t *dst_index, int32_t *count,
                       das3r_stream_t stream);
int das3r_prune_compact(int32_t P, int32_t kept, const int32_t *dst_index, int32_t n, const das3r_prune_tensor *tensors,
                        das3r_stream_t stream);

size_t das3r_thin_workspace_bytes(int32_t P);
int das3r_thin_voxels(int32_t P, const float *xyz, const float *score , float inv_edge, uint8_t *keep, int32_t *count,
                      int32_t *info , char *workspace, das3r_stream_t stream);

#define DAS3R_AUX_MAX_CHANNELS 8
int das3r_raster_aux_forward(const das3r_raster_args *args, const das3r_raster_saved *saved, int32_t C, const float *features ,
                             float *out , das3r_stream_t stream);
size_t das3r_raster_aux_scratch_bytes(int64_t capacity, int32_t C);
int das3r_raster_aux_adjoint(const das3r_raster_args *args, const das3r_raster_saved *saved, int32_t C, const float *dL_dout ,
                             float *dL_dfeat , int32_t accumulate, float *scratch, das3r_stream_t stream);

size_t das3r_raster_aux_backward_scratch_bytes(int64_t capacity, int32_t C);
int das3r_raster_aux_backward(const das3r_raster_args *args, const das3r_raster_in *in, const das3r_raster_saved *saved, int32_t C,
                              const float *features , const float *dL_dout ,
                              const float *dL_dalpha , float *dL_dfeatures ,
                              const das3r_raster_grads *grads, das3r_stream_t stream);

int das3r_raster_distortion_forward(const das3r_raster_args *args, const das3r_raster_saved *saved, float *out ,
                                    float *totals , das3r_stream_t stream);
size_t das3r_raster_distortion_backward_scratch_bytes(int64_t capacity, int32_t P);
int das3r_raster_distortion_backward(const das3r_raster_args *args, const das3r_raster_in *in, const das3r_raster_saved *saved,
                                     const float *dL_ddist , const float *totals ,
                                     const das3r_raster_grads *grads, das3r_stream_t stream);


typedef struct {
    size_t geom_bytes, binning_bytes, img_bytes;
    size_t depth_key;
    size_t xy;
    size_t conic_opacity;
    size_t rgbd;
    size_t splat_stride;
    size_t clamped;
    size_t tiles_touched;
    size_t sorted_idx;
    size_t offsets;
    size_t point_list;
    size_t final_T;
    size_t n_contrib;
    size_t ranges;
} das3r_raster_layout;

int das3r_raster_get_layout(int32_t P, int64_t capacity, int32_t W, int32_t H, das3r_raster_layout *out);

void das3r_profile_enable(int on);
int das3r_profile_report(char *buf, size_t cap);

int das3r_debug_poison_lds(uint32_t pattern, das3r_stream_t stream);

void das3r_debug_inject_fault(uint32_t bits);

void das3r_debug_mutate(uint32_t what);

int das3r_pair_counters(int enable, uint64_t out[4]);

int das3r_raster_count_live_pairs(const das3r_raster_args *args, const das3r_raster_saved *saved, uint64_t out[2], das3r_stream_t stream);

void das3r_reload_switches(void);

void das3r_get_stats(uint64_t out[4]);

int das3r_raster_forget_shapes(void);

int das3r_raster_learning(int32_t set, uint32_t state[2]);

int das3r_has_experiments(void);

int das3r_split_colour_rule(int32_t has_sh, int32_t sh_degree, int32_t P, int32_t binning_path, int32_t no_backward, int32_t forced);
int das3r_split_colour_switch(void);

typedef struct {
    int32_t P, W, H;
    int64_t last_I, peak_I;
    int32_t radix_left, backoff;
    uint32_t gen;
    int32_t seg_extra, last_seg, fine;
    uint32_t forwards, clean, longest;
    int32_t resume_valid, resume_fine;
    uint32_t resume_forwards;
} das3r_path_policy_state;
typedef struct {
    int32_t P, W, H, ntiles, tbits, tile_passes;
    uint32_t too_long, want_bits;
    int32_t forced;
    int32_t onesweep;
    int64_t capacity_hint;
    int32_t capacity_exact;
} das3r_path_policy_inputs;
typedef struct {
    int32_t local, seg, seg_bits, seg_passes;
    int32_t speculate, decide_fine;
    uint32_t gen;
    int64_t cap;
} das3r_path_policy_plan;
void das3r_debug_path_policy_fresh(das3r_path_policy_state *state, uint32_t gen);
void das3r_debug_path_policy_plan(das3r_path_policy_state *state, const das3r_path_policy_inputs *in, das3r_path_policy_plan *plan);
int das3r_debug_path_policy_count(das3r_path_policy_state *state, const das3r_path_policy_inputs *in, const das3r_path_policy_plan *plan, int64_t I);
int das3r_debug_path_policy_skew(das3r_path_policy_state *state, uint32_t longest, uint32_t crowd16, int64_t cap, int32_t ntiles);
uint32_t das3r_debug_path_policy_hint(const das3r_path_policy_state *state);
void das3r_debug_path_policy_forget(das3r_path_policy_state *state);
void das3r_debug_path_policy_resume(das3r_path_policy_state *state, uint32_t fine, uint32_t forwards);
int das3r_debug_seg_dbits(int32_t tbits, int32_t passes);

typedef struct {
    int32_t sort_ipl, sort_classic, rect_upstream, verbose, binning, capacity_exact, fused_emit_off, no_sh_stage;
    int32_t render_fwd, render_bwd;
    int32_t render_bwd_mb, render_bwd_atomic;
    int32_t render_bwd_pix, render_bwd_occ;
    int32_t render_bwd_strips;
    int32_t tile_chunk, scan_items, deterministic, tile_lpt_off, bwd_reduce_set, bwd_reduce_shfl, ablate_set, ablate, tickets;
    int32_t bwd_pad_lds, fwd_pad_lds, bwd_buckets, fwd_no_prefetch, split_colour, tile_strip;
} das3r_switches;
typedef struct {
    int32_t kernel, mb, slices;
    int32_t pix, occ, strips, atomic_flush;
} das3r_bwd_choice;
typedef struct {
    int32_t kernel, quad_lanes, row_private, tile_lpt;
} das3r_fwd_choice;
void das3r_debug_parse_switches(const char *const *names, const char *const *values, int32_t n, int32_t experiments, das3r_switches *out);
void das3r_debug_choose_backward(const das3r_switches *sw, int64_t num_rendered, int32_t ntiles, uint32_t fwd_flags, das3r_bwd_choice *out);
void das3r_debug_choose_forward(const das3r_switches *sw, int32_t ntiles, int64_t capacity, int32_t local_lists, int32_t prefer_regions,
                                das3r_fwd_choice *out);
int das3r_debug_has_invdepth_form(int32_t backward, int32_t kernel);
const char *das3r_debug_kernel_name(int32_t backward, int32_t kernel);

typedef struct {
    int32_t has_sh, has_cov;
    int32_t M, sh_degree;
    int32_t shs_aligned16, dL_dshs_aligned16;
    int32_t no_sh_stage;
    int32_t jac_saved;
    int32_t chained, quad_rows;
    int32_t depth, aa;
} das3r_preprocess_backward_inputs;
typedef struct {
    int32_t has_sh, has_cov, stage_in, stage_out, deg0, chain, depth, jac, aa;
    int32_t base_index;
    int32_t sh_rows_staged;
} das3r_preprocess_form;
int das3r_debug_choose_preprocess_backward(const das3r_preprocess_backward_inputs *in, das3r_preprocess_form *out);
const char *das3r_debug_preprocess_backward_name(const das3r_preprocess_form *form);

int das3r_abi_version(void);
const char *das3r_last_error(void);

#ifdef __cplusplus
}
#endif
#endif
```

Before: 1207 Msplats/s.

## Add cell-based partition sort path for bucket-local binning

Adds a new binning sort path that partitions keys into cells with a strided atomic cursor (to spread contention), then a per-cell finish kernel that histograms depth digits in LDS, writes tile ranges and scatters in staged rounds. It is selected by default when the bucket-local plan is active and tile passes are at most two. The local tile sort's tie-breaking also changes to order equal depths by gaussian id. This aims to replace the multi-pass onesweep partition with fewer global passes, at the cost of repeated reads of each cell's keys per round.

```diff
diff --git a/das3r_amd/_lib.py b/das3r_amd/_lib.py
--- a/das3r_amd/_lib.py
+++ b/das3r_amd/_lib.py
@@ -71,7 +71,7 @@
 
 class PathPolicyPlan(C.Structure):
     _fields_ = [("local", C.c_int32), ("seg", C.c_int32), ("seg_bits", C.c_int32), ("seg_passes", C.c_int32), ("speculate", C.c_int32),
-                ("decide_fine", C.c_int32), ("gen", C.c_uint32), ("cap", C.c_int64)]
+                ("decide_fine", C.c_int32), ("gen", C.c_uint32), ("cells", C.c_int32), ("cap", C.c_int64)]
 
 
 class Switches(C.Structure):
diff --git a/das3r_amd/csrc/api.hip b/das3r_amd/csrc/api.hip
--- a/das3r_amd/csrc/api.hip
+++ b/das3r_amd/csrc/api.hip
@@ -165,6 +165,8 @@
     L->b_e2 = take(4 * In);
     L->b_ghist = take(4 * 4 * RADIX_SIZE);
     L->b_ticket = take(256);
+    L->cursor_stride = I >= (int64_t)(1 << 20) ? CURSOR_STRIDE : 1;
+    L->b_cursor = take(4 * (size_t)RADIX_SIZE * (size_t)L->cursor_stride);
     L->b_status = take(onesweep_status_bytes((int64_t)In, L->tile_passes + 1));
     L->b_ctrl_bytes = o - L->b_ghist;
     L->b_ckpt = take(((size_t)In / BUCKET + (size_t)(L->ntiles > 0 ? L->ntiles : 1) + 2) * 256 * 16);
@@ -219,14 +221,14 @@
     }
 };
 ForwardPlan plan_of(const das3r_path_policy_plan *p) {
-    return ForwardPlan{p->local != 0, p->seg != 0, p->seg == 2, p->seg_bits, p->seg_passes, p->speculate != 0, p->cap, p->decide_fine != 0, p->gen};
+    return ForwardPlan{p->local != 0, p->seg != 0, p->seg == 2, p->seg == 2 && p->cells != 0, p->seg_bits, p->seg_passes, p->speculate != 0, p->cap, p->decide_fine != 0, p->gen};
 }
 }
 extern "C" void das3r_debug_path_policy_fresh(das3r_path_policy_state *state, uint32_t gen) { policy_state_to(Verdict::fresh(gen), Resume(), state); }
 extern "C" void das3r_debug_path_policy_plan(das3r_path_policy_state *state, const das3r_path_policy_inputs *in, das3r_path_policy_plan *out) {
     PolicyOnState on(state);
     const ForwardPlan p = plan_forward(on.v, on.inputs(in));
-    *out = das3r_path_policy_plan{p.local, p.bucket_local ? 2 : (p.seg ? 1 : 0), p.seg_bits, p.seg_passes, p.speculate, p.decide_fine, p.gen, p.cap};
+    *out = das3r_path_policy_plan{p.local, p.bucket_local ? 2 : (p.seg ? 1 : 0), p.seg_bits, p.seg_passes, p.speculate, p.decide_fine, p.gen, p.cells, p.cap};
 }
 extern "C" int das3r_debug_path_policy_count(das3r_path_policy_state *state, const das3r_path_policy_inputs *in, const das3r_path_policy_plan *plan, int64_t I) {
     PolicyOnState on(state);
diff --git a/das3r_amd/csrc/cell_sort.hip b/das3r_amd/csrc/cell_sort.hip
--- /dev/null
+++ b/das3r_amd/csrc/cell_sort.hip
@@ -0,0 +1,307 @@
+#include "granule.h"
+
+namespace das3r {
+
+#ifndef DAS3R_CELL_SPLIT
+#define DAS3R_CELL_SPLIT 4
+#endif
+#ifndef DAS3R_CELL_ROUND
+#define DAS3R_CELL_ROUND 3072
+#endif
+#ifndef DAS3R_CELL_B1
+#define DAS3R_CELL_B1 8
+#endif
+#ifndef DAS3R_CELL_B2
+#define DAS3R_CELL_B2 4
+#endif
+constexpr int CELL_SPLIT = DAS3R_CELL_SPLIT, CELL_ROUND = DAS3R_CELL_ROUND;
+static_assert(CELL_SPLIT >= 1 && CELL_SPLIT <= 8 && (CELL_SPLIT & (CELL_SPLIT - 1)) == 0, "a power of two of workgroups per cell");
+
+template <int IPL>
+__global__ void __launch_bounds__(256) cell_partition_kernel(const uint32_t *__restrict__ keys_in, const uint32_t *__restrict__ gid_in,
+                                                             uint32_t *__restrict__ keys_out, uint32_t *__restrict__ gid_out,
+                                                             uint32_t *__restrict__ slot_out, uint32_t cap, const uint32_t *__restrict__ n_ptr,
+                                                             int shift, const uint32_t *__restrict__ ghist ,
+                                                             uint32_t *__restrict__ cursor , int cursor_stride,
+                                                             uint32_t *__restrict__ err) {
+    __shared__ uint16_t cnt[4][RADIX_SIZE];
+    __shared__ uint32_t gdelta[RADIX_SIZE];
+    __shared__ uint32_t sk[256 * IPL], sv[256 * IPL], sv2[256 * IPL];
+    __shared__ uint32_t ws[8];
+    const int tid = threadIdx.x, lane = __lane_id(), wave = tid >> 6;
+    const uint32_t n = min(*n_ptr, cap);
+    const uint32_t b = blockIdx.x;
+    if ((uint64_t)b * 256u * IPL >= n) return;
+#pragma unroll
+    for (int w = 0; w < 4; w++) cnt[w][tid] = 0;
+    __syncthreads();
+    const uint32_t base = (b * 4u + (uint32_t)wave) * 64u * (uint32_t)IPL;
+
+    uint32_t k[IPL], v[IPL];
+#pragma unroll
+    for (int s = 0; s < IPL; s++) {
+        const uint32_t i = base + s * 64 + lane;
+        k[s] = i < n ? keys_in[i] : 0u;
+        v[s] = i < n ? gid_in[i] : 0u;
+    }
+    uint32_t local[IPL];
+    {
+        volatile uint16_t *cw = cnt[wave];
+#pragma unroll
+        for (int s = 0; s < IPL; s++) {
+            const uint32_t i = base + s * 64 + lane;
+            const bool valid = i < n;
+            const uint32_t digit = (k[s] >> shift) & 255u;
+            const uint64_t vm = __ballot(valid);
+            uint32_t plo = (uint32_t)vm, phi = (uint32_t)(vm >> 32);
+#pragma unroll
+            for (int bb = 0; bb < RADIX_BITS; bb++) {
+                const uint32_t sel = 0u - ((digit >> bb) & 1u);
+                const uint64_t m = __ballot((digit >> bb) & 1u);
+                plo &= ~((uint32_t)m ^ sel);
+                phi &= ~((uint32_t)(m >> 32) ^ sel);
+            }
+            const uint32_t rank = __builtin_amdgcn_mbcnt_hi(phi, __builtin_amdgcn_mbcnt_lo(plo, 0u));
+            const uint32_t count = (uint32_t)__popc(plo) + (uint32_t)__popc(phi);
+            uint32_t before = 0;
+            if (valid) before = cw[digit];
+            __builtin_amdgcn_wave_barrier();
+            if (valid && rank == 0) cw[digit] = (uint16_t)(before + count);
+            __builtin_amdgcn_wave_barrier();
+            local[s] = before + rank;
+        }
+    }
+    __syncthreads();
+
+    const uint32_t c0 = cnt[0][tid], c1 = cnt[1][tid], c2 = cnt[2][tid], c3 = cnt[3][tid];
+    const uint32_t total = c0 + c1 + c2 + c3;
+    uint32_t reserved = 0u;
+    if (total) reserved = __hip_atomic_fetch_add(cursor + (size_t)tid * cursor_stride, total, __ATOMIC_RELAXED, __HIP_MEMORY_SCOPE_AGENT);
+    const uint32_t g = ghist[tid];
+    uint32_t digit_base, lstart;
+    {
+        const uint32_t incl = wave_incl_scan_u32(g), lincl = wave_incl_scan_u32(total);
+        if (lane == 63) {
+            ws[wave] = incl;
+            ws[4 + wave] = lincl;
+        }
+        __syncthreads();
+        uint32_t wbase = 0, lbase = 0;
+#pragma unroll
+        for (int w = 0; w < 4; w++)
+            if (w < wave) {
+                wbase += ws[w];
+                lbase += ws[4 + w];
+            }
+        lstart = lbase + lincl - total;
+        digit_base = wbase + incl - g;
+        cnt[0][tid] = (uint16_t)lstart;
+        cnt[1][tid] = (uint16_t)(lstart + c0);
+        cnt[2][tid] = (uint16_t)(lstart + c0 + c1);
+        cnt[3][tid] = (uint16_t)(lstart + c0 + c1 + c2);
+    }
+    __syncthreads();
+#pragma unroll
+    for (int s = 0; s < IPL; s++) {
+        const uint32_t i = base + s * 64 + lane;
+        if (i < n) {
+            const uint32_t slot = cnt[wave][(k[s] >> shift) & 255u] + local[s];
+            sk[slot] = k[s];
+            sv[slot] = v[s];
+            sv2[slot] = i;
+        }
+    }
+    if (reserved + total > g) atomicOr(err, ERR_COUNTS);
+    gdelta[tid] = digit_base + reserved - lstart;
+    __syncthreads();
+
+    const uint32_t block_first = b * 256u * (uint32_t)IPL;
+    const uint32_t nvalid = min(n - block_first, 256u * (uint32_t)IPL);
+#pragma unroll
+    for (int s = 0; s < IPL; s++) {
+        const uint32_t i = s * 256 + tid;
+        if (i < nvalid) {
+            const uint32_t key = sk[i];
+            const uint32_t dst = i + gdelta[(key >> shift) & 255u];
+            if (dst >= n) {
+                atomicOr(err, ERR_RANGE);
+                continue;
+            }
+            keys_out[dst] = key;
+            gid_out[dst] = sv[i];
+            slot_out[dst] = sv2[i];
+        }
+    }
+}
+
+__global__ void __launch_bounds__(256) cell_finish_kernel(const uint32_t *__restrict__ keys_in, const uint32_t *__restrict__ gid_in,
+                                                          const uint32_t *__restrict__ slot_in ,
+                                                          uint32_t *__restrict__ keys_out, uint32_t *__restrict__ gid_out,
+                                                          uint32_t *__restrict__ slot_out, uint32_t cap, const uint32_t *__restrict__ n_ptr,
+                                                          int kshift, int dbits, uint32_t ntiles, uint32_t ncells,
+                                                          const uint32_t *__restrict__ ghist_hi ,
+                                                          const uint32_t *__restrict__ cursor , int cursor_stride,
+                                                          uint2 *__restrict__ ranges, const uint32_t *__restrict__ err,
+                                                          uint32_t *__restrict__ host_late, uint32_t tag, uint32_t inject,
+                                                          uint32_t *__restrict__ host_flag, uint32_t flag_value) {
+    __shared__ uint32_t s_off[RADIX_SIZE + 1], s_cur[RADIX_SIZE], ws[4], s_cell[2];
+    __shared__ uint32_t st_k[CELL_ROUND], st_g[CELL_ROUND], st_s[CELL_ROUND];
+    const int tid = threadIdx.x;
+    const uint32_t n = min(*n_ptr, cap);
+    if (blockIdx.x == 0) {
+        const bool bad = cursor && ghist_hi && cursor[(size_t)tid * cursor_stride] != ghist_hi[tid];
+        const int any = __syncthreads_or(bad ? 1 : 0);
+        if (tid == 0 && host_late) {
+            host_late[0] = *err | inject | (any ? ERR_COUNTS : 0u);
+            __hip_atomic_store(host_late + 1, tag, __ATOMIC_RELEASE, __HIP_MEMORY_SCOPE_SYSTEM);
+        }
+    }
+    const uint32_t cell = (blockIdx.x / (8u * CELL_SPLIT)) * 8u + (blockIdx.x & 7u), part = (blockIdx.x >> 3) & (CELL_SPLIT - 1u);
+    if (cell >= ncells) return;
+    {
+        const uint32_t c = ghist_hi ? ghist_hi[tid] : (tid == 0 ? n : 0u);
+        uint32_t tot;
+        const uint32_t ex = block_exclusive_scan_256(c, ws, &tot);
+        if ((uint32_t)tid == cell) {
+            s_cell[0] = min(ex, n);
+            s_cell[1] = min(c, n - min(ex, n));
+        }
+        s_cur[tid] = 0u;
+        __syncthreads();
+    }
+    const uint32_t base = s_cell[0], cnt = s_cell[1];
+    if (cnt == 0u) return;
+    const uint32_t *kin = keys_in + base;
+
+    constexpr int B1 = DAS3R_CELL_B1;
+    for (uint32_t i0 = 0; i0 < cnt; i0 += 256u * B1) {
+        uint32_t k[B1];
+#pragma unroll
+        for (int u = 0; u < B1; u++) {
+            const uint32_t i = i0 + u * 256u + tid;
+            k[u] = i < cnt ? kin[i] : 0u;
+        }
+#pragma unroll
+        for (int u = 0; u < B1; u++)
+            if (i0 + u * 256u + tid < cnt) atomicAdd(&s_cur[(k[u] >> kshift) & 255u], 1u);
+    }
+    __syncthreads();
+    {
+        const uint32_t h = s_cur[tid];
+        uint32_t tot;
+        const uint32_t ex = block_exclusive_scan_256(h, ws, &tot);
+        s_off[tid] = ex;
+        if (tid == 255) s_off[256] = ex + h;
+        __syncthreads();
+    }
+    if (part == 0u && tid < (1 << (8 - dbits))) {
+        const uint32_t t = (cell << (8 - dbits)) + (uint32_t)tid;
+        const uint32_t lo = s_off[tid << dbits], hi = s_off[(tid + 1) << dbits];
+        if (hi > lo && t < ntiles) ranges[t] = make_uint2(base + lo, base + hi);
+    }
+
+    constexpr int B2 = DAS3R_CELL_B2;
+    const int b_end = (int)(part + 1u) * (RADIX_SIZE / CELL_SPLIT);
+    int r0 = (int)part * (RADIX_SIZE / CELL_SPLIT);
+    while (r0 < b_end) {
+        const uint32_t first = s_off[r0], lim = first + (uint32_t)CELL_ROUND;
+        int lo = r0, hi = b_end;
+        while (lo < hi) {
+            const int mid = (lo + hi + 1) >> 1;
+            if (s_off[mid] <= lim) lo = mid;
+            else hi = mid - 1;
+        }
+        const bool direct = lo == r0;
+        const int r1 = direct ? r0 + 1 : lo;
+        const uint32_t m = s_off[r1] - first;
+        if (m == 0u) {
+            r0 = r1;
+            continue;
+        }
+        __syncthreads();
+        s_cur[tid] = 0u;
+        __syncthreads();
+        for (uint32_t i0 = 0; i0 < cnt; i0 += 256u * B2) {
+            uint32_t k[B2], g[B2], sl[B2];
+#pragma unroll
+            for (int u = 0; u < B2; u++) {
+                const uint32_t i = i0 + u * 256u + tid;
+                const bool in = i < cnt;
+                k[u] = in ? kin[i] : 0u;
+                g[u] = in ? gid_in[base + i] : 0u;
+                sl[u] = (in && slot_in) ? slot_in[base + i] : base + i;
+            }
+#pragma unroll
+            for (int u = 0; u < B2; u++) {
+                const int bin = (int)((k[u] >> kshift) & 255u);
+                if (i0 + u * 256u + tid < cnt && bin >= r0 && bin < r1) {
+                    const uint32_t at = s_off[bin] - first + atomicAdd(&s_cur[bin], 1u);
+                    if (direct) {
+                        const uint32_t dst = base + first + at;
+                        if (at < m && dst < n) {
+                            keys_out[dst] = k[u];
+                            gid_out[dst] = g[u];
+                            slot_out[dst] = sl[u];
+                        }
+                    } else if (at < (uint32_t)CELL_ROUND) {
+                        st_k[at] = k[u];
+                        st_g[at] = g[u];
+                        st_s[at] = sl[u];
+                    }
+                }
+            }
+        }
+        if (direct) {
+            if (tid == 0 && host_flag) __hip_atomic_store(host_flag, flag_value, __ATOMIC_RELAXED, __HIP_MEMORY_SCOPE_SYSTEM);
+        } else {
+            __syncthreads();
+            for (uint32_t j = tid; j < m; j += 256u) {
+                const uint32_t dst = base + first + j;
+                if (dst < n) {
+                    keys_out[dst] = st_k[j];
+                    gid_out[dst] = st_g[j];
+                    slot_out[dst] = st_s[j];
+                }
+            }
+        }
+        r0 = r1;
+    }
+}
+
+int launch_cell_sort(int64_t cap, char *geom, char *binning, char *img, const Layout &L, uint32_t **keys_final, uint32_t *host_late, uint32_t tag,
+                     uint32_t *host_flag, uint32_t flag_value, bool debug, hipStream_t s) {
+    if (L.part_passes > 2 || L.kbits != 8 * L.part_passes || L.dbits < 1 || L.dbits > 7) {
+        set_error("the cells plan needs a partition key of 8 or 16 bits with depth buckets (kbits %d, dbits %d, passes %d)", L.kbits, L.dbits, L.part_passes);
+        return DAS3R_ERR_INVALID_ARG;
+    }
+    const uint32_t *n_ptr = (const uint32_t *)(geom + L.g_count);
+    uint32_t *err = (uint32_t *)(geom + L.g_ticket) + 8;
+    uint32_t *keyA = (uint32_t *)(binning + L.b_keyA), *keyB = (uint32_t *)(binning + L.b_keyB);
+    uint32_t *valA = (uint32_t *)(binning + L.b_valA), *valB = (uint32_t *)(binning + L.b_valB);
+    uint32_t *gid_of = (uint32_t *)(binning + L.b_gid_of), *slot_list = (uint32_t *)(binning + L.b_slot), *e_tmp = (uint32_t *)(binning + L.b_e2);
+    uint32_t *ghist = (uint32_t *)(binning + L.b_ghist), *cursor = (uint32_t *)(binning + L.b_cursor);
+    uint32_t *const pl_final = (uint32_t *)(binning + L.pub.point_list), *const pl_other = pl_final == valA ? valB : valA;
+    uint2 *ranges = (uint2 *)(img + L.pub.ranges);
+    const bool two = L.part_passes == 2;
+    if (two) {
+        const int ipl = sort_items_per_lane(cap);
+        const int nblocks = div_up(cap, (int64_t)256 * ipl);
+#define PART(IPL)                                                                                                                      \
+    DAS3R_LAUNCH((cell_partition_kernel<IPL>), dim3(nblocks), dim3(256), 0, s, keyA, gid_of, keyB, pl_other, e_tmp, (uint32_t)cap, n_ptr, \
+                 L.kshift + 8, ghist + 256, cursor, L.cursor_stride, err)
+        if (ipl == 4) PART(4); else if (ipl == 8) PART(8); else PART(16);
+#undef PART
+        KERNEL_CHECK(s, debug, "cell_partition");
+    }
+    const uint32_t ncells = two ? (((uint32_t)L.ntiles - 1u) >> (8 - L.dbits)) + 1u : 1u;
+    const uint32_t grid = ((ncells + 7u) & ~7u) * (uint32_t)CELL_SPLIT;
+    uint32_t *kout = two ? keyA : keyB;
+    DAS3R_LAUNCH(cell_finish_kernel, dim3(grid), dim3(256), 0, s, two ? keyB : keyA, two ? pl_other : gid_of, two ? e_tmp : (uint32_t *)nullptr, kout,
+                 pl_final, slot_list, (uint32_t)cap, n_ptr, L.kshift, L.dbits, (uint32_t)L.ntiles, ncells, two ? ghist + 256 : (uint32_t *)nullptr,
+                 two ? cursor : (uint32_t *)nullptr, L.cursor_stride, ranges, err, host_late, tag, (uint32_t)switches().inject_fault, host_flag, flag_value);
+    KERNEL_CHECK(s, debug, "cell_finish");
+    *keys_final = kout;
+    return DAS3R_OK;
+}
+
+}
diff --git a/das3r_amd/csrc/common.h b/das3r_amd/csrc/common.h
--- a/das3r_amd/csrc/common.h
+++ b/das3r_amd/csrc/common.h
@@ -132,6 +132,7 @@
     return b < 1 ? 1 : b;
 }
 
+constexpr int CURSOR_STRIDE = 32;
 constexpr int SPLAT_REC = 4;
 
 constexpr uint32_t DEPTH_SAVED_FLAG = 2u;
@@ -148,6 +149,8 @@
     size_t g_ghist, g_ticket, g_status, g_scan_status, g_ctrl_bytes;
     int64_t capacity;
     size_t b_ghist, b_ticket, b_status, b_ctrl_bytes;
+    size_t b_cursor;
+    int cursor_stride;
     int tiles_x, tiles_y, ntiles, tbits, tile_passes;
     int chunksP, chunksI;
     int dbits, kbits, kshift;
@@ -248,7 +251,10 @@
                    bool fused_scan, uint32_t *host_late, uint32_t tag, bool debug, hipStream_t s, uint32_t **dead_keys = nullptr,
                    uint32_t *emit_slot = nullptr ,
                    uint32_t *seg_host_flag = nullptr, uint32_t seg_flag_value = 0 ,
-                   bool local_finish = false );
+                   bool local_finish = false ,
+                   bool cells = false );
+int launch_cell_sort(int64_t cap, char *geom, char *binning, char *img, const Layout &L, uint32_t **keys_final, uint32_t *host_late, uint32_t tag,
+                     uint32_t *host_flag, uint32_t flag_value, bool debug, hipStream_t s);
 int launch_segment_sort(int64_t cap, const uint32_t *n_ptr, const uint32_t *keys_final, int fbits, uint32_t *point_list, uint32_t *slot_list,
                         const uint32_t *depth_key, uint32_t last_g, uint32_t *scratch_keys, uint32_t *host_flag, uint32_t flag_value, bool debug,
                         hipStream_t s, int dbits, uint2 *ranges, const uint32_t *err, uint32_t *host_late, uint32_t tag, uint32_t inject);
diff --git a/das3r_amd/csrc/forward.hip b/das3r_amd/csrc/forward.hip
--- a/das3r_amd/csrc/forward.hip
+++ b/das3r_amd/csrc/forward.hip
@@ -399,7 +399,7 @@
     if (cap > 0 && (r = claim_check_slot(&host_late))) return r;
     uint32_t *dead_keys = nullptr;
     if ((r = launch_binning(P, cap, a->image_width, a->image_height, out->radii, saved->geom, saved->binning, saved->img, L, fused_scan, host_late, late_tag,
-                            a->debug != 0, s, &dead_keys, emit_slot, mb->dev + MB_TOO_LONG, plan.gen, finish))) return r;
+                            a->debug != 0, s, &dead_keys, emit_slot, mb->dev + MB_TOO_LONG, plan.gen, finish, finish && plan.cells))) return r;
     if ((r = colour_launch())) return r;
     LocalBin lb = {(float4 *)(saved->binning + L.b_ckpt), nullptr, nullptr, nullptr, nullptr, plan.gen, (uint32_t)(P - 1), (uint32_t)cap};
     if ((r = look_at_lists(&lb))) return r;
diff --git a/das3r_amd/csrc/kernel_choice.h b/das3r_amd/csrc/kernel_choice.h
--- a/das3r_amd/csrc/kernel_choice.h
+++ b/das3r_amd/csrc/kernel_choice.h
@@ -109,7 +109,7 @@
     }
     w.rect_upstream = (e = env("DAS3R_RECT")) && e[0] == 'u';
     w.verbose = env("DAS3R_VERBOSE") != nullptr;
-    if ((e = env("DAS3R_BINNING"))) w.binning = e[0] == 'l' ? 1 : (e[0] == 'r' ? -1 : (e[0] == 's' ? (strchr(e, '3') ? 3 : 2) : (e[0] == 'b' ? 4 : 0)));
+    if ((e = env("DAS3R_BINNING"))) w.binning = e[0] == 'l' ? 1 : (e[0] == 'r' ? -1 : (e[0] == 's' ? (strchr(e, '3') ? 3 : 2) : (e[0] == 'b' ? 4 : (e[0] == 'c' ? 5 : 0))));
     w.capacity_exact = (e = env("DAS3R_CAPACITY")) && e[0] == 'e';
     w.fused_emit_off = (e = env("DAS3R_FUSED_EMIT")) && e[0] == '0';
     if ((e = env("DAS3R_SPLIT_COLOUR"))) w.split_colour = e[0] == '0' ? -1 : (e[0] == '1' ? 1 : 0);
diff --git a/das3r_amd/csrc/path_policy.h b/das3r_amd/csrc/path_policy.h
--- a/das3r_amd/csrc/path_policy.h
+++ b/das3r_amd/csrc/path_policy.h
@@ -22,8 +22,13 @@
 
 static inline bool bucket_local_rule(int forced, bool onesweep, int tbits, int tile_passes, int ntiles, int64_t last_I, int radix_left) {
     if (!onesweep || seg_dbits(tbits, tile_passes) < BUCKET_LOCAL_DBITS) return false;
-    if (forced == 4) return true;
+    if (forced == 4 || forced == 5) return true;
     return forced == 0 && radix_left == 0 && ntiles > BUCKET_LOCAL_TILES && last_I > BUCKET_LOCAL_AVG * ntiles && last_I <= LOCAL_AVG * ntiles;
+}
+
+constexpr bool CELLS_BY_SHAPE = true;
+static inline bool cells_rule(int forced, bool bucket_local, int tile_passes, bool by_shape = CELLS_BY_SHAPE) {
+    return bucket_local && tile_passes <= 2 && (forced == 5 || (forced == 0 && by_shape));
 }
 
 struct Verdict {
@@ -66,6 +71,7 @@
 struct ForwardPlan {
     bool local, seg;
     bool bucket_local;
+    bool cells;
     int seg_bits, seg_passes;
     bool speculate;
     int64_t cap;
@@ -100,7 +106,8 @@
     }
     const int forced = in.forced;
     p.bucket_local = bucket_local_rule(forced, in.onesweep, in.tbits, in.tile_passes, in.ntiles, v.last_I, v.radix_left);
-    p.local = !p.bucket_local && in.onesweep && (forced == 1 || forced == 4 || (forced == 0 && v.radix_left == 0 && v.last_I <= LOCAL_AVG * in.ntiles));
+    p.cells = cells_rule(forced, p.bucket_local, in.tile_passes);
+    p.local = !p.bucket_local && in.onesweep && (forced == 1 || forced == 4 || forced == 5 || (forced == 0 && v.radix_left == 0 && v.last_I <= LOCAL_AVG * in.ntiles));
     p.seg_passes = in.tile_passes + ((!p.bucket_local && (forced == 3 || (forced == 0 && v.seg_extra))) ? 1 : 0);
     p.seg_bits = (in.onesweep && p.seg_passes <= 3) ? seg_dbits(in.tbits, p.seg_passes) : 0;
     p.seg = p.bucket_local || (!p.local && p.seg_bits > 0 && (forced == 2 || forced == 3 || (forced == 0 && v.radix_left == 0 && v.last_I >= 0 &&
diff --git a/das3r_amd/csrc/render_common.h b/das3r_amd/csrc/render_common.h
--- a/das3r_amd/csrc/render_common.h
+++ b/das3r_amd/csrc/render_common.h
@@ -309,7 +309,7 @@
     }
     if (lb.dbits > 0 && n <= 2 * TILE_PIX) {
         uint32_t *s_word = reinterpret_cast<uint32_t *>(stage), *s_byrank = s_word + 2 * TILE_PIX + 8, *s_depth = s_byrank + 2 * TILE_PIX + 8;
-        uint32_t *s_lo = s_depth + 2 * TILE_PIX, *s_hi = s_lo + 128;
+        uint32_t *s_lo = s_depth + 2 * TILE_PIX, *s_hi = s_lo + 128, *s_idr = s_hi + 128;
         const uint32_t *kk = lb.keys + range.x;
         const int wsh = lb.fbits + 9;
         const uint32_t kmask = (1u << (lb.dbits + lb.fbits)) - 1u;
@@ -361,6 +361,7 @@
                 }
                 rank[u] = min(r, (uint32_t)(n - 1));
                 s_byrank[rank[u]] = w[u];
+                s_idr[rank[u]] = g[u];
             }
         }
         __syncthreads();
@@ -375,13 +376,13 @@
 #pragma unroll
         for (int u = 0; u < 2; u++)
             if (tied[u]) {
-                const uint32_t r = rank[u], f = w[u] >> 9, mine = s_depth[r], at = w[u] & 0x1FFu;
+                const uint32_t r = rank[u], f = w[u] >> 9, mine = s_depth[r];
                 uint32_t a = r, b = r + 1u, below = 0u;
                 while (a > 0u && (s_byrank[a - 1u] >> 9) == f) a--;
                 while (b < (uint32_t)n && (s_byrank[b] >> 9) == f) b++;
                 for (uint32_t k = a; k < b; k++) {
-                    const uint32_t dk = s_depth[k], pk = s_byrank[k] & 0x1FFu;
-                    below += (dk < mine || (dk == mine && pk < at)) ? 1u : 0u;
+                    const uint32_t dk = s_depth[k];
+                    below += (dk < mine || (dk == mine && s_idr[k] < g[u])) ? 1u : 0u;
                 }
                 rank[u] = a + below;
             }
@@ -438,22 +439,34 @@
         }
         __syncthreads();
         mark(7);
-        uint32_t g[LOCAL_MAX / TILE_PIX], slot[LOCAL_MAX / TILE_PIX];
+        uint32_t g[LOCAL_MAX / TILE_PIX], slot[LOCAL_MAX / TILE_PIX], to[LOCAL_MAX / TILE_PIX];
 #pragma unroll
         for (int u = 0; u < LOCAL_MAX / TILE_PIX; u++) {
             const int i = u * TILE_PIX + tid;
             const int from = i < n ? (int)((uint32_t)s_key[i] & (uint32_t)(LOCAL_MAX - 1)) : 0;
             g[u] = s_gid[from];
             slot[u] = s_slot[from];
+            to[u] = (uint32_t)i;
+            if (i < n) {
+                const uint32_t d = (uint32_t)(s_key[i] >> 32);
+                if ((i > 0 && (uint32_t)(s_key[i - 1] >> 32) == d) || (i + 1 < n && (uint32_t)(s_key[i + 1] >> 32) == d)) {
+                    int a = i, b = i + 1;
+                    while (a > 0 && (uint32_t)(s_key[a - 1] >> 32) == d) a--;
+                    while (b < n && (uint32_t)(s_key[b] >> 32) == d) b++;
+                    uint32_t below = 0u;
+                    for (int k = a; k < b; k++) below += s_gid[(uint32_t)s_key[k] & (uint32_t)(LOCAL_MAX - 1)] < g[u] ? 1u : 0u;
+                    to[u] = (uint32_t)a + below;
+                }
+            }
         }
         __syncthreads();
 #pragma unroll
         for (int u = 0; u < LOCAL_MAX / TILE_PIX; u++) {
             const int i = u * TILE_PIX + tid;
             if (i < n) {
-                s_gid[i] = g[u];
-                pl[i] = g[u];
-                sl[i] = slot[u];
+                s_gid[to[u]] = g[u];
+                pl[to[u]] = g[u];
+                sl[to[u]] = slot[u];
             }
         }
         __syncthreads();
diff --git a/das3r_amd/csrc/sort.hip b/das3r_amd/csrc/sort.hip
--- a/das3r_amd/csrc/sort.hip
+++ b/das3r_amd/csrc/sort.hip
@@ -276,7 +276,7 @@
 
 int launch_binning(int P, int64_t I, int W, int H, const int32_t *radii, char *geom, char *binning, char *img, const Layout &L,
                    bool fused_scan, uint32_t *host_late, uint32_t tag, bool debug, hipStream_t s, uint32_t **dead_keys, uint32_t *emit_slot,
-                   uint32_t *seg_host_flag, uint32_t seg_flag_value, bool local_finish) {
+                   uint32_t *seg_host_flag, uint32_t seg_flag_value, bool local_finish, bool cells) {
     const uint32_t *n_ptr = (const uint32_t *)(geom + L.g_count);
     (void)W; (void)H;
     uint2 *ranges = (uint2 *)(img + L.pub.ranges);
@@ -301,6 +301,11 @@
 #endif
     if (onesweep) {
         uint32_t *kfinal = nullptr;
+        if (cells && local_finish && L.dbits > 0 && !emit_slot) {
+            const int rc0 = launch_cell_sort(I, geom, binning, img, L, &kfinal, host_late, tag, seg_host_flag, seg_flag_value, debug, s);
+            if (!rc0 && dead_keys) *dead_keys = kfinal;
+            return rc0;
+        }
         int rc1 = launch_onesweep_partition(I, geom, binning, L, &kfinal, debug, s, emit_slot ? emit_slot + 64 : nullptr, emit_slot);
         if (rc1) return rc1;
         if (dead_keys) *dead_keys = kfinal;
diff --git a/das3r_amd/roofline.py b/das3r_amd/roofline.py
--- a/das3r_amd/roofline.py
+++ b/das3r_amd/roofline.py
@@ -2,7 +2,7 @@
 HBM_PEAK_GBS = 8000.0
 
 BINNING_KERNELS = ("radix_hist_kernel", "radix_rowscan_kernel", "radix_scatter_kernel", "depth_hist_kernel", "onesweep_pass_kernel",
-                   "scan_emit_kernel", "emit_kernel", "tile_ranges_kernel", "segment_sort_kernel")
+                   "scan_emit_kernel", "emit_kernel", "tile_ranges_kernel", "segment_sort_kernel", "cell_partition_kernel", "cell_finish_kernel")
 
 
 def algorithmic_bytes(P, D, M, I, W, H):
diff --git a/include/das3r_raster.h b/include/das3r_raster.h
--- a/include/das3r_raster.h
+++ b/include/das3r_raster.h
@@ -304,6 +304,7 @@
     int32_t local, seg, seg_bits, seg_passes;
     int32_t speculate, decide_fine;
     uint32_t gen;
+    int32_t cells;
     int64_t cap;
 } das3r_path_policy_plan;
 void das3r_debug_path_policy_fresh(das3r_path_policy_state *state, uint32_t gen);
```

Measured after the change: 1234 Msplats/s (median of 6 runs). +2.3%, better.
